# jolibrain/fluidnet_cxx

Measured on AMD Instinct MI355X. Metric: fluid time-step throughput, Mcells/s = cells*steps/s/1e6 (steps/s alongside), higher is better.
Workload: dtype f32; 1 GPU; plume3d_256_jacobi; method=jacobi, jacobi_iters=100, parallelism=1 GPU, launch=hip-graph replay, developed_steps=100, world_size=1, state_finite=True

## Files before the change

fluidnet_cxx_amd/csrc/fluidnet_cpp.cpp:

```cpp
#include <memory>
#include <optional>
#include <torch/extension.h>
#include <c10/hip/HIPStream.h>
#include <c10/hip/HIPGuard.h>

#include "../../include/fluidnet_hip.h"

namespace {

using at::Tensor;

struct Geom {
  bool ref_quirks = false;
  int z_offset = 0, D_global = 0;
  int k_begin = 0, k_end = 0;
};

void check_status(int rc) {
  TORCH_CHECK(rc == FNX_OK, fnx_last_error());
}

void check_field(const Tensor& t, const char* name) {
  TORCH_CHECK(t.is_cuda(), name, " must be on the GPU (libfluidnet_hip has no CPU path)");
  TORCH_CHECK(t.scalar_type() == at::kFloat, name, " must be float32");
// ... 856 lines not shown
  if (grads)
    TORCH_CHECK(upstream->is_cuda() && upstream->scalar_type() == at::kFloat && upstream->numel() == 1 && upstream->get_device() == out_p.get_device(),
                "upstream must be one float32 on the GPU");
  c10::hip::HIPGuard guard(out_p.get_device());
  const float lam[4] = {(float)lambdas[0], (float)lambdas[1], (float)lambdas[2], (float)lambdas[3]};
  Tensor t, gp, gU, ws;
  size_t bytes = 0;
  if (terms) {
    t = at::empty({5}, out_p.options());
    bytes = (is3d ? fnx_train_loss3d_ws_bytes : fnx_train_loss_ws_bytes)(&g);
    ws = at::empty({(int64_t)(bytes ? bytes : 1)}, out_p.options().dtype(at::kByte));
  }
  if (grads) { gp = at::empty_like(out_p); gU = at::empty_like(out_U); }
  check_status((is3d ? fnx_train_loss3d : fnx_train_loss)(
      &g, out_p.data_ptr<float>(), out_U.data_ptr<float>(), flags.data_ptr<float>(), has_t ? target_p->data_ptr<float>() : nullptr, lam,
      grads ? upstream->data_ptr<float>() : nullptr, terms ? t.data_ptr<float>() : nullptr, grads ? gp.data_ptr<float>() : nullptr,
      grads ? gU.data_ptr<float>() : nullptr, terms ? ws.data_ptr() : nullptr, bytes, cur_stream(out_p)));
  return {t, gp, gU};
}

static float* opt_field(const FnxGrid& g, c10::optional<Tensor>& t, bool vel, const char* name) {
  if (!t.has_value() || !t->defined()) return nullptr;
  if (vel) check_vel(*t, g, name); else check_scalar(*t, g, name);
  return t->data_ptr<float>();
}

static FnxState make_state(const FnxGrid& g, Tensor& p, Tensor& U, Tensor& flags, c10::optional<Tensor>& density,
                           c10::optional<Tensor>& UBC, c10::optional<Tensor>& UBCInvMask,
                           c10::optional<Tensor>& densityBC, c10::optional<Tensor>& densityBCInvMask) {
  FnxState st{};
  st.p = p.data_ptr<float>(); st.U = U.data_ptr<float>(); st.flags = flags.data_ptr<float>();
  st.density = opt_field(g, density, false, "density");
  st.UBC = opt_field(g, UBC, true, "UBC"); st.UBCInvMask = opt_field(g, UBCInvMask, true, "UBCInvMask");
  st.densityBC = opt_field(g, densityBC, false, "densityBC"); st.densityBCInvMask = opt_field(g, densityBCInvMask, false, "densityBCInvMask");
  return st;
}

static FnxStepParams step_params(double dt, double buoyancy_scale, const std::vector<double>& gravity_vec, double operating_density) {
  FnxStepParams prm{};
  prm.dt = (float)dt; prm.buoyancy_scale = (float)buoyancy_scale;
  for (int a = 0; a < 3; ++a) prm.gravity_vec[a] = (float)gravity_vec[a];
  prm.operating_density = (float)operating_density;
  return prm;
}

void simulate_step_(Tensor p, Tensor U, Tensor flags, c10::optional<Tensor> density, c10::optional<Tensor> UBC,
                    c10::optional<Tensor> UBCInvMask, c10::optional<Tensor> densityBC,
                    c10::optional<Tensor> densityBCInvMask, c10::optional<Tensor> net, double dt,
                    double maccormack_strength, bool sample_outside_fluid, double buoyancy_scale,
                    std::vector<double> gravity_vec, double operating_density, double p_tol, int jacobi_iter,
                    const std::string method, double normalize_threshold, c10::optional<Tensor> workspace,
                    int static_flags, const Geom* geom, const std::string& precision_mode, double viscosity,
                    double gravity_scale, bool correct_scalar, int periodic, c10::optional<Tensor> flags_stick, double pcg_tol,
                    int pcg_iter, double vorticity_confinement, bool pcg_warm) {
  check_field(U, "U");
  FnxGrid g = grid_of(flags, U.size(1) == 3, geom);
  check_vel(U, g, "U"); check_scalar(p, g, "p");
  TORCH_CHECK(viscosity >= 0, "Viscosity must be positive");
  TORCH_CHECK(method == "jacobi" || method == "convnet" || method == "pcg" || method == "hybrid",
              "Simulation method not supported. Choose convnet, jacobi, pcg or hybrid.");
  TORCH_CHECK(gravity_vec.size() == 3, "gravityVec needs x, y, z");
  FnxStepParams prm = step_params(dt, buoyancy_scale, gravity_vec, operating_density);
  prm.maccormack_strength = (float)maccormack_strength; prm.sample_outside_fluid = sample_outside_fluid;
  prm.p_tol = (float)p_tol; prm.jacobi_iter = jacobi_iter;
  prm.method = method == "convnet" ? 1 : (method == "hybrid" ? 3 : (method == "pcg" ? (pcg_warm ? 4 : 2) : 0)); prm.normalize_threshold = (float)normalize_threshold;
  prm.pcg_tol = (float)pcg_tol; prm.pcg_iter = pcg_iter;
  prm.precision_mode = precision_of(precision_mode);
  prm.viscosity = (float)viscosity; prm.gravity_scale = (float)gravity_scale; prm.correct_scalar = correct_scalar ? 1 : 0;
  prm.periodic = periodic;
  prm.vorticity_confinement = (float)vorticity_confinement;
  FnxState st = make_state(g, p, U, flags, density, UBC, UBCInvMask, densityBC, densityBCInvMask);
  st.net = (net.has_value() && net->defined()) ? net->data_ptr() : nullptr;
  st.flags_stick = opt_field(g, flags_stick, false, "flags_stick");
  c10::hip::HIPGuard guard(flags.get_device());
  const size_t bytes = fnx_workspace_bytes(&g, FNX_OP_STEP);
  Tensor ws;
  const bool given = workspace.has_value() && workspace->defined() && (size_t)workspace->numel() * workspace->element_size() >= bytes;
  if (given) ws = *workspace;
  else ws = at::empty({(int64_t)bytes}, flags.options().dtype(at::kByte));
  prm.static_flags = given ? static_flags : 0;
  check_status(fnx_simulate_step(&g, &prm, &st, ws.data_ptr(), (size_t)ws.numel() * ws.element_size(), cur_stream(U)));
  wrote(p); wrote(U); wrote(density);
}

struct PyLoopbackGroup {
  void* g = nullptr; int nranks;
  explicit PyLoopbackGroup(int n) : nranks(n) { check_status(fnx_slab_loopback_group(&g, n)); }
  ~PyLoopbackGroup() { fnx_slab_loopback_group_free(g); }
};
struct PyPeer {
  void* p = nullptr;
  std::string handle;
  PyPeer(int rank, int nranks, int64_t mailbox_bytes) {
    char h[FNX_PEER_HANDLE_BYTES];
    check_status(fnx_slab_peer_create(&p, rank, nranks, (size_t)mailbox_bytes, h));
    handle.assign(h, FNX_PEER_HANDLE_BYTES);
  }
  ~PyPeer() { fnx_slab_peer_free(p); }
};
struct PySlabComm {
  FnxSlabComm c{};
  std::shared_ptr<PyLoopbackGroup> keep;
  std::shared_ptr<PyPeer> keep_peer;
  ~PySlabComm() { fnx_slab_comm_free(&c); }
};
py::bytes slab_rccl_unique_id() {
  char id[128];
  check_status(fnx_slab_rccl_unique_id(id));
  return py::bytes(id, 128);
}
std::shared_ptr<PySlabComm> slab_comm_rccl(int rank, int nranks, const std::string& unique_id) {
  TORCH_CHECK(unique_id.size() == 128, "the RCCL unique id has 128 bytes");
  auto c = std::make_shared<PySlabComm>();
  py::gil_scoped_release nogil;
  check_status(fnx_slab_comm_rccl(&c->c, rank, nranks, unique_id.data()));
  return c;
}
std::shared_ptr<PySlabComm> slab_comm_loopback(std::shared_ptr<PyLoopbackGroup> group, int rank) {
  auto c = std::make_shared<PySlabComm>();
  check_status(fnx_slab_comm_loopback(&c->c, group->g, rank));
  c->keep = group;
  return c;
}
struct PySlab {
  FnxSlab* s = nullptr;
  FnxSlabConfig cfg{};
  std::shared_ptr<PySlabComm> comm;
  PySlab(int B, int H, int W, int D_global, int rank, int nranks, int halo, int sweeps_per_exchange, bool static_flags,
         int cfl_check_every, std::shared_ptr<PySlabComm> comm_, const std::string& schedule, const std::string& method, const std::string& direct_sends) : comm(comm_) {
    cfg.B = B; cfg.H = H; cfg.W = W; cfg.D_global = D_global; cfg.rank = rank; cfg.nranks = nranks; cfg.halo = halo;
    cfg.sweeps_per_exchange = sweeps_per_exchange; cfg.static_flags = static_flags ? 1 : 0; cfg.cfl_check_every = cfl_check_every;
    TORCH_CHECK(schedule == "deep_first" || schedule == "edge_first" || schedule == "last_pass" || schedule == "deep_beside",
                "unknown z-slab schedule '", schedule, "'");
    cfg.schedule = schedule == "deep_first" ? FNX_SLAB_DEEP_FIRST : (schedule == "edge_first" ? FNX_SLAB_EDGE_FIRST :
                   (schedule == "deep_beside" ? FNX_SLAB_DEEP_BESIDE : FNX_SLAB_LAST_PASS));
    TORCH_CHECK(method == "jacobi" || method == "convnet", "unknown z-slab method '", method, "'");
    cfg.method = method == "convnet" ? 1 : 0;
    TORCH_CHECK(direct_sends == "auto" || direct_sends == "never" || direct_sends == "always", "direct_sends: 'auto', 'never' or 'always'");
    cfg.direct_sends = direct_sends == "auto" ? 0 : (direct_sends == "never" ? 1 : 2);
    check_status(fnx_slab_create(&s, &cfg, comm ? &comm->c : nullptr));
  }
  ~PySlab() { fnx_slab_destroy(s); }
  std::vector<int> layout() const {
    int o, l, h, z;
    check_status(fnx_slab_layout(&cfg, &o, &l, &h, &z));
    return {o, l, h, z};
  }
  int64_t workspace_bytes() const { return (int64_t)fnx_slab_workspace_bytes(&cfg); }
  void stats_enable(bool on) { check_status(fnx_slab_stats_enable(s, on ? 1 : 0)); }
  py::dict stats_read() {
    FnxSlabStats t{};
    check_status(fnx_slab_stats_read(s, &t));
    py::dict d;
    d["bytes_per_neighbour"] = t.bytes_per_neighbour; d["wait_ms"] = t.wait_ms; d["exchanges"] = (int64_t)t.exchanges;
    return d;
  }
  void step(Tensor p, Tensor U, Tensor flags, Tensor density, c10::optional<Tensor> UBC, c10::optional<Tensor> UBCInvMask,
            c10::optional<Tensor> densityBC, c10::optional<Tensor> densityBCInvMask, double dt, double maccormack_strength,
            bool sample_outside_fluid, double buoyancy_scale, std::vector<double> gravity_vec, double operating_density,
            double p_tol, int jacobi_iter, Tensor workspace, c10::optional<Tensor> net, const std::string& precision_mode,
            double normalize_threshold, const std::string& method, double viscosity) {
    check_field(U, "U");
    Geom none;
    FnxGrid g = grid_of(flags, true, &none);
    check_vel(U, g, "U"); check_scalar(p, g, "p"); check_scalar(density, g, "density");
    const std::vector<int> l = layout();
    TORCH_CHECK(g.B == cfg.B && g.H == cfg.H && g.W == cfg.W && g.D == l[0] + l[1] + l[2], "the tensors are not this rank's slab (",
                cfg.B, " x ", l[0] + l[1] + l[2], " x ", cfg.H, " x ", cfg.W, " with ghost planes)");
    TORCH_CHECK(gravity_vec.size() == 3, "gravityVec needs x, y, z");
    TORCH_CHECK(workspace.is_cuda() && workspace.is_contiguous(), "workspace must be a contiguous GPU tensor");
    FnxStepParams prm = step_params(dt, buoyancy_scale, gravity_vec, operating_density);
    prm.maccormack_strength = (float)maccormack_strength; prm.sample_outside_fluid = sample_outside_fluid;
    prm.p_tol = (float)p_tol; prm.jacobi_iter = jacobi_iter; prm.method = 0;
    const bool cnn = net.has_value() && net->defined();
    if (cnn) {
      TORCH_CHECK(net->is_cuda() && net->is_contiguous(), "net: the packed weights (scalenet_pack) on the GPU");
      prm.method = 1; prm.precision_mode = precision_of(precision_mode); prm.normalize_threshold = (float)normalize_threshold;
    }
    TORCH_CHECK(method == "auto" || method == "jacobi" || method == "convnet" || method == "pcg", "unknown z-slab step method '", method, "'");
    if (method == "pcg") prm.method = 2;
    prm.viscosity = (float)viscosity;
    c10::optional<Tensor> rho(density);
    FnxState st = make_state(g, p, U, flags, rho, UBC, UBCInvMask, densityBC, densityBCInvMask);
    if (cnn) st.net = net->data_ptr();
    c10::hip::HIPGuard guard(flags.get_device());
    check_status(fnx_slab_step(s, &prm, &st, workspace.data_ptr(), (size_t)workspace.numel() * workspace.element_size(), cur_stream(U)));
  }
};

void jacobi_sweeps_(Tensor flags, Tensor div, Tensor p, bool is3D, int nsweeps, c10::optional<Tensor> workspace,
                    bool reuse_mask, const Geom* geom, bool from_zero) {
  FnxGrid g = grid_of(flags, is3D, geom);
  check_scalar(div, g, "div"); check_scalar(p, g, "p");
  c10::hip::HIPGuard guard(flags.get_device());
  const size_t bytes = fnx_workspace_bytes(&g, FNX_OP_JACOBI);
  Tensor ws;
  if (workspace.has_value() && workspace->defined() && (size_t)workspace->numel() * workspace->element_size() >= bytes) ws = *workspace;
  else { ws = at::empty({(int64_t)bytes}, flags.options().dtype(at::kByte)); reuse_mask = false; }
  check_status(fnx_jacobi_sweeps_ex(&g, flags.data_ptr<float>(), div.data_ptr<float>(), p.data_ptr<float>(), nsweeps,
                                    ws.data_ptr(), (size_t)ws.numel() * ws.element_size(), (reuse_mask ? 1 : 0) | (from_zero ? 2 : 0),
                                    cur_stream(flags)));
  wrote(p);
}

void jacobi_pass_(Tensor flags, Tensor div, c10::optional<Tensor> p_in_opt, Tensor p_out, int nsweeps, int k_begin,
                  int k_end, Tensor workspace, bool reuse_mask, int k_begin2, const Geom* geom, int layout) {
  FnxGrid g = grid_of(flags, true, geom);
  const bool zero = !(p_in_opt.has_value() && p_in_opt->defined());
  Tensor p_in = zero ? p_out : *p_in_opt;
  check_scalar(div, g, "div"); check_scalar(p_in, g, "p_in"); check_scalar(p_out, g, "p_out");
  c10::hip::HIPGuard guard(flags.get_device());
  check_status(fnx_jacobi_pass_layout(&g, flags.data_ptr<float>(), div.data_ptr<float>(), zero ? nullptr : p_in.data_ptr<float>(),
                                      p_out.data_ptr<float>(), nsweeps, k_begin, k_end, k_begin2, layout, workspace.data_ptr(),
                                      (size_t)workspace.numel() * workspace.element_size(), reuse_mask ? 1 : 0, cur_stream(flags)));
  wrote(p_out);
}

bool jacobi_quad_ok(int B, int D, int H, int W) {
  FnxGrid g{B, D, H, W, 1, 0, 0, 0};
  return fnx_jacobi_quad_ok(&g) != 0;
}

void jacobi_pass_mirror_(Tensor flags, Tensor div, Tensor p_in, Tensor p_out, int k_begin, int k_end, Tensor workspace, bool reuse_mask,
                         Tensor mirror, int k_first, int planes, int k_begin2, c10::optional<Tensor> mirror2, int k_first2, const Geom* geom,
                         int layout) {
  FnxGrid g = grid_of(flags, true, geom);
  check_scalar(div, g, "div"); check_scalar(p_in, g, "p_in"); check_scalar(p_out, g, "p_out");
  const int64_t need = (int64_t)g.B * planes * g.H * g.W;
  auto chk = [&](const Tensor& t) { TORCH_CHECK(t.is_cuda() && t.is_contiguous() && t.scalar_type() == at::kFloat && t.numel() >= need, "mirror: a contiguous fp32 GPU tensor of B * planes * H * W floats"); };
  chk(mirror);
  FnxPlaneMirror m{};
  m.out[0][0] = mirror.data_ptr<float>(); m.k_first[0] = k_first; m.planes = planes; m.sample_stride = (size_t)planes * g.H * g.W;
  if (mirror2.has_value() && mirror2->defined()) { chk(*mirror2); m.out[1][0] = mirror2->data_ptr<float>(); m.k_first[1] = k_first2; }
  c10::hip::HIPGuard guard(flags.get_device());
  check_status(fnx_jacobi_pass_mirror(&g, flags.data_ptr<float>(), div.data_ptr<float>(), p_in.data_ptr<float>(), p_out.data_ptr<float>(),
                                      k_begin, k_end, k_begin2, layout, &m, workspace.data_ptr(),
                                      (size_t)workspace.numel() * workspace.element_size(), reuse_mask ? 1 : 0, cur_stream(flags)));
  wrote(p_out); wrote(mirror); wrote(mirror2);
}

int64_t jacobi_workspace_bytes(int B, int D, int H, int W, bool is3D) {
  FnxGrid g{B, D, H, W, is3D ? 1 : 0, 0, 0, 0};
  return (int64_t)fnx_workspace_bytes(&g, FNX_OP_JACOBI);
}

static const unsigned char* bc_class_ptr(c10::optional<Tensor>& t, const Tensor& flags) {
  if (!t.has_value() || !t->defined()) return nullptr;
  TORCH_CHECK(t->scalar_type() == at::kByte && t->is_contiguous() && t->numel() == flags.numel() && t->device() == flags.device(),
              "bc_class: expected the uint8 tensor bc_classify returned for this grid");
  return t->data_ptr<unsigned char>();
}

Tensor bc_classify(Tensor flags, bool is3D, c10::optional<Tensor> UBC, c10::optional<Tensor> UBCInvMask,
                   c10::optional<Tensor> densityBC, c10::optional<Tensor> densityBCInvMask) {
  FnxGrid g = grid_of(flags, is3D, nullptr);
  Tensor dummy;
  c10::optional<Tensor> none;
  FnxState st{};
  st.UBC = opt_field(g, UBC, true, "UBC"); st.UBCInvMask = opt_field(g, UBCInvMask, true, "UBCInvMask");
  st.densityBC = opt_field(g, densityBC, false, "densityBC"); st.densityBCInvMask = opt_field(g, densityBCInvMask, false, "densityBCInvMask");
  c10::hip::HIPGuard guard(flags.get_device());
  Tensor cls = at::empty(flags.sizes(), flags.options().dtype(at::kByte));
  check_status(fnx_bc_classify(&g, &st, cls.data_ptr<unsigned char>(), cur_stream(flags)));
  return cls;
}

Tensor pre_projection_(Tensor U_adv, c10::optional<Tensor> rho_adv, Tensor p, Tensor U, Tensor flags,
                       c10::optional<Tensor> density, c10::optional<Tensor> UBC, c10::optional<Tensor> UBCInvMask,
                       c10::optional<Tensor> densityBC, c10::optional<Tensor> densityBCInvMask, double dt,
                       double buoyancy_scale, std::vector<double> gravity_vec, double operating_density,
                       bool jacobi_method, c10::optional<Tensor> bc_class, const Geom* geom) {
  check_field(U, "U");
  FnxGrid g = grid_of(flags, U.size(1) == 3, geom);
  check_vel(U, g, "U"); check_vel(U_adv, g, "U_adv"); check_scalar(p, g, "p");
  FnxStepParams prm = step_params(dt, buoyancy_scale, gravity_vec, operating_density);
  prm.method = jacobi_method ? 0 : 1;
  FnxState st = make_state(g, p, U, flags, density, UBC, UBCInvMask, densityBC, densityBCInvMask);
  const float* ra = nullptr;
  if (rho_adv.has_value() && rho_adv->defined()) { check_scalar(*rho_adv, g, "rho_adv"); ra = rho_adv->data_ptr<float>(); }
  st.bc_class = bc_class_ptr(bc_class, flags);
  c10::hip::HIPGuard guard(flags.get_device());
  Tensor div = at::empty_like(flags);
  check_status(fnx_pre_projection(&g, &prm, &st, U_adv.data_ptr<float>(), ra, div.data_ptr<float>(), cur_stream(U)));
  return div;
}

void post_projection_(Tensor p, Tensor U, Tensor flags, c10::optional<Tensor> density, c10::optional<Tensor> UBC,
                      c10::optional<Tensor> UBCInvMask, c10::optional<Tensor> densityBC,
                      c10::optional<Tensor> densityBCInvMask, c10::optional<Tensor> bc_class, const Geom* geom,
                      bool density_bc_applied) {
  check_field(U, "U");
  FnxGrid g = grid_of(flags, U.size(1) == 3, geom);
  check_vel(U, g, "U"); check_scalar(p, g, "p");
  FnxState st = make_state(g, p, U, flags, density, UBC, UBCInvMask, densityBC, densityBCInvMask);
  st.bc_class = bc_class_ptr(bc_class, flags);
  st.density_bc_applied = density_bc_applied ? 1 : 0;
  c10::hip::HIPGuard guard(flags.get_device());
  check_status(fnx_post_projection(&g, &st, cur_stream(U)));
  wrote(U); wrote(density);
}

int64_t step_workspace_bytes(int B, int D, int H, int W, bool is3D) {
  FnxGrid g{B, D, H, W, is3D ? 1 : 0, 0, 0, 0};
  return (int64_t)fnx_workspace_bytes(&g, FNX_OP_STEP);
}

}

template <class T, class R, class... A>
static auto in_dim(T which, R (*body)(T, A...)) {
  return [=](A... a) { return body(which, std::forward<A>(a)...); };
}

PYBIND11_MODULE(TORCH_EXTENSION_NAME, m) {
  using NoGil = py::call_guard<py::gil_scoped_release>;
  const auto GEOM = py::arg("geom") = py::none();
  py::class_<Geom>(m, "Geom", "per-call 3D geometry options: ref_quirks, z-slab view (z_offset, D_global), compute window [k_begin, k_end)")
      .def(py::init([](bool ref_quirks, int z_offset, int D_global, int k_begin, int k_end) {
             Geom g; g.ref_quirks = ref_quirks; g.z_offset = z_offset; g.D_global = D_global; g.k_begin = k_begin; g.k_end = k_end;
             return g;
           }),
           py::arg("ref_quirks") = false, py::arg("z_offset") = 0, py::arg("D_global") = 0, py::arg("k_begin") = 0,
           py::arg("k_end") = 0)
      .def_readwrite("ref_quirks", &Geom::ref_quirks)
      .def_readwrite("z_offset", &Geom::z_offset)
      .def_readwrite("D_global", &Geom::D_global)
      .def_readwrite("k_begin", &Geom::k_begin)
      .def_readwrite("k_end", &Geom::k_end);
  m.def("advect_scalar", &advect_scalar, "Advect Scalar", py::arg("dt"), py::arg("src"), py::arg("U"), py::arg("flags"),
        py::arg("method"), py::arg("boundary_width"), py::arg("sample_outside_fluid"), py::arg("maccormack_strength"),
        py::arg("out") = py::none(), GEOM, py::arg("plan") = "auto", NoGil());
  m.def("advect_scalars", &advect_scalars, "Advect C passive scalars through one pair of line traces", py::arg("dt"), py::arg("src"),
        py::arg("U"), py::arg("flags"), py::arg("method"), py::arg("boundary_width"), py::arg("sample_outside_fluid"),
        py::arg("maccormack_strength"), py::arg("workspace") = py::none(), GEOM, py::arg("out") = py::none(), NoGil());
  m.def("advect_scalars_workspace_bytes", [](int B, int D, int H, int W, bool is3D, int channels) {
          FnxGrid g{}; g.B = B; g.D = D; g.H = H; g.W = W; g.is3D = is3D ? 1 : 0;
          return fnx_advect_scalars_workspace_bytes(&g, channels);
        }, py::arg("B"), py::arg("D"), py::arg("H"), py::arg("W"), py::arg("is3D"), py::arg("channels"));
  m.def("advect_step", &advect_step, py::arg("dt"), py::arg("density"), py::arg("U"), py::arg("flags"),
        py::arg("sample_outside_fluid"), py::arg("maccormack_strength"), py::arg("out_density") = py::none(),
        py::arg("out_U") = py::none(), GEOM, py::arg("plan") = "auto", NoGil());
  m.def("advect_vel", &advect_vel, "Advect Velocity", py::arg("dt"), py::arg("orig"), py::arg("U"), py::arg("flags"),
        py::arg("method"), py::arg("boundary_width"), py::arg("maccormack_strength"), py::arg("out") = py::none(), GEOM,
        py::arg("plan") = "auto", NoGil());
  m.def("solve_linear_system", &solve_linear_system, "Solve Linear System using Jacobi's method", py::arg("flags"),
        py::arg("div"), py::arg("is3D"), py::arg("p_tol"), py::arg("max_iter"), py::arg("verbose"), GEOM, NoGil());
  m.def("solve_linear_system_pcg", &solve_linear_system_pcg, "Converged pressure solve: multigrid-preconditioned CG (fnx_pcg); "
        "returns (p, residual, iterations per sample or None when p_tol <= 0).  p0: a starting guess (fnx_pcg_from; max_iter may then be 0)",
        py::arg("flags"), py::arg("div"), py::arg("is3D"), py::arg("p_tol") = 1e-5,
        py::arg("max_iter") = 50, py::arg("verbose") = false, GEOM, py::arg("p0") = py::none(), NoGil());
  m.def("poisson_apply", &poisson_apply, "A p, the operator of the pressure solve (fnx_poisson_apply)", py::arg("flags"), py::arg("p"),
        py::arg("is3D"), GEOM, NoGil());
  m.def("pcg_precondition", &pcg_precondition, "z = M^-1 r, one V-cycle of the PCG preconditioner (fnx_pcg_precondition)", py::arg("flags"),
        py::arg("r"), py::arg("is3D"), GEOM, NoGil());
  m.def("velocity_divergence", &velocity_divergence, py::arg("U"), py::arg("flags"), GEOM, NoGil());
  m.def("velocity_update_", &velocity_update_, py::arg("pressure"), py::arg("U"), py::arg("flags"), GEOM, NoGil());
  m.def("add_buoyancy_", &add_buoyancy_, py::arg("U"), py::arg("flags"), py::arg("density"), py::arg("gravity"),
        py::arg("rho_star"), py::arg("dt"), GEOM, NoGil());
  m.def("correct_scalar_", &correct_scalar_, py::arg("dt"), py::arg("src"), py::arg("div"), py::arg("flags"), NoGil());
  m.def("add_gravity_", &add_gravity_, py::arg("U"), py::arg("flags"), py::arg("gravity"), py::arg("dt"), GEOM, NoGil());
  m.def("add_viscosity_", &add_viscosity_, NoGil());
  m.def("add_vorticity_confinement", &add_vorticity_confinement, py::arg("U"), py::arg("flags"), py::arg("strength"), GEOM, NoGil());
  m.def("add_vorticity_confinement_", &add_vorticity_confinement_, py::arg("U"), py::arg("flags"), py::arg("strength"), GEOM, NoGil());
  m.def("render_volume", &render_volume, "density + flags -> (B,2,R,Cc) radiance / transmittance image (fnx_render_volume)", py::arg("density"),
        py::arg("flags"), py::arg("view_dir"), py::arg("light_dir"), py::arg("k_view"), py::arg("k_light"), py::arg("ambient") = 0.25,
        py::arg("albedo_smoke") = 1.0, py::arg("albedo_obstacle") = 0.5, py::arg("bnd") = 1, NoGil());
  m.def("set_wall_bcs_", &set_wall_bcs_, py::arg("U"), py::arg("flags"), GEOM, NoGil());
  m.def("set_wall_bcs_stick_", &set_wall_bcs_stick_, NoGil());
  m.def("add_viscosity_out", &add_viscosity_out, "addViscosity of U into `out` (not U), returned (fnx_add_viscosity)", py::arg("dt"), py::arg("U"),
        py::arg("flags"), py::arg("viscosity"), py::arg("out"), NoGil());
  m.def("set_wall_bcs_stick_out", &set_wall_bcs_stick_out, "setWallBcsStick of U into `out` (not U), returned (fnx_set_wall_bcs_stick)",
        py::arg("U"), py::arg("flags"), py::arg("flags_stick"), py::arg("out"), NoGil());
  m.def("set_const_vals_", &set_const_vals_, NoGil());
  m.def("flags_to_occupancy", &flags_to_occupancy, NoGil());
  m.def("max_abs", &max_abs, NoGil());
  m.def("empty_domain_", &empty_domain_, py::arg("flags"), py::arg("boundary_width"), GEOM, NoGil());
  m.def("velocity_divergence_backward", &velocity_divergence_backward, py::arg("grad_div"), py::arg("flags"), py::arg("is3D"), GEOM, NoGil());
  m.def("velocity_update_backward", &velocity_update_backward, py::arg("grad_U_out"), py::arg("flags"), GEOM, NoGil());
  m.def("create_cylinder_", &create_cylinder_, NoGil());
  m.def("create_box2d_", &create_box2d_, NoGil());
  m.def("get_centered", &get_centered, NoGil());
  m.def("scalenet_pack", &scalenet_pack, NoGil());
  m.def("multiscale_forward", &multiscale_forward, py::arg("packed"), py::arg("x"), py::arg("precision_mode") = "fp32",
        py::arg("trim") = std::vector<int64_t>(), NoGil());
  m.def("fluidnet_forward", in_dim((const BankApi*)nullptr, &whole_forward), py::arg("packed"), py::arg("input"),
        py::arg("normalize_threshold"), py::arg("precision_mode") = "fp32", NoGil());
  m.def("banknet_pack", in_dim(&BANK2D, &bank_pack), py::arg("blob"), NoGil());
  m.def("banknet_forward", in_dim(&BANK2D, &bank_forward), py::arg("packed"), py::arg("x"), py::arg("precision_mode") = "fp32", NoGil());
  m.def("fluidnet_bank_forward", in_dim(&BANK2D, &whole_forward), py::arg("packed"), py::arg("input"), py::arg("normalize_threshold"),
        py::arg("precision_mode") = "fp32", NoGil());
  m.def("banknet3d_pack", in_dim(&BANK3D, &bank_pack), py::arg("blob"), NoGil());
  m.def("banknet3d_forward", in_dim(&BANK3D, &bank_forward), py::arg("packed"), py::arg("x"), py::arg("precision_mode") = "fp32", NoGil());
  m.def("fluidnet_bank3d_forward", in_dim(&BANK3D, &whole_forward), py::arg("packed"), py::arg("input"), py::arg("normalize_threshold"),
        py::arg("precision_mode") = "fp32", NoGil());
  m.def("banknet_pack_t", &banknet_pack_t, py::arg("blob"), NoGil());
  m.def("banknet_tape_layout", &banknet_tape_layout, py::arg("B"), py::arg("H"), py::arg("W"));
  m.def("banknet_forward_train", &banknet_forward_train, py::arg("packed"), py::arg("x"), py::arg("precision_mode") = "fp32", NoGil());
  m.def("banknet_backward", &banknet_backward, py::arg("packed_t"), py::arg("x"), py::arg("grad_p"), py::arg("tape"),
        py::arg("precision_mode") = "fp32", NoGil());
  m.def("fluidnet_bank_forward_train", &fluidnet_bank_forward_train, py::arg("packed"), py::arg("input"), py::arg("normalize_threshold"),
        py::arg("precision_mode") = "fp32", NoGil());
  m.def("fluidnet_bank_backward", &fluidnet_bank_backward, py::arg("packed_t"), py::arg("flags"), py::arg("scale"), py::arg("grad_p"),
        py::arg("grad_U"), py::arg("tape"), py::arg("precision_mode") = "fp32", NoGil());
  m.def("simulate_step_", &simulate_step_, py::arg("p"), py::arg("U"), py::arg("flags"), py::arg("density"), py::arg("UBC"),
        py::arg("UBCInvMask"), py::arg("densityBC"), py::arg("densityBCInvMask"), py::arg("net"), py::arg("dt"),
        py::arg("maccormack_strength"), py::arg("sample_outside_fluid"), py::arg("buoyancy_scale"), py::arg("gravity_vec"),
        py::arg("operating_density"), py::arg("p_tol"), py::arg("jacobi_iter"), py::arg("method"),
        py::arg("normalize_threshold"), py::arg("workspace") = py::none(), py::arg("static_flags") = 0, GEOM,
        py::arg("precision_mode") = "fp32", py::arg("viscosity") = 0.0, py::arg("gravity_scale") = 0.0,
        py::arg("correct_scalar") = false, py::arg("periodic") = 0, py::arg("flags_stick") = py::none(), py::arg("pcg_tol") = 1e-5,
        py::arg("pcg_iter") = 50, py::arg("vorticity_confinement") = 0.0, py::arg("pcg_warm") = false, NoGil());
  m.def("step_workspace_bytes", &step_workspace_bytes);
  m.def("jacobi_sweeps_", &jacobi_sweeps_, py::arg("flags"), py::arg("div"), py::arg("p"), py::arg("is3D"), py::arg("nsweeps"),
        py::arg("workspace") = py::none(), py::arg("reuse_mask") = false, GEOM, py::arg("from_zero") = false, NoGil());
  m.def("jacobi_workspace_bytes", &jacobi_workspace_bytes);
  m.def("jacobi_pass_", &jacobi_pass_, py::arg("flags"), py::arg("div"), py::arg("p_in"), py::arg("p_out"), py::arg("nsweeps"),
        py::arg("k_begin"), py::arg("k_end"), py::arg("workspace"), py::arg("reuse_mask"), py::arg("k_begin2") = -1, GEOM,
        py::arg("layout") = 0, NoGil());
  m.def("jacobi_pass_mirror_", &jacobi_pass_mirror_, py::arg("flags"), py::arg("div"), py::arg("p_in"), py::arg("p_out"), py::arg("k_begin"),
        py::arg("k_end"), py::arg("workspace"), py::arg("reuse_mask"), py::arg("mirror"), py::arg("k_first"), py::arg("planes"),
        py::arg("k_begin2") = -1, py::arg("mirror2") = py::none(), py::arg("k_first2") = 0, GEOM, py::arg("layout") = 0, NoGil(),
        "two sweeps on planes [k_begin, k_end) (+ a second range) whose output planes [k_first, k_first + planes) also go to `mirror` (fnx_jacobi_pass_mirror)");
  m.def("jacobi_pass_mirror_ok", [](int B, int D, int H, int W, int planes_per_range, bool two_ranges, int layout) {
    FnxGrid g{}; g.B = B; g.D = D; g.H = H; g.W = W; g.is3D = 1;
    return fnx_jacobi_pass_mirror_ok(&g, planes_per_range, two_ranges ? 1 : 0, layout) != 0;
  });
  m.def("jacobi_quad_ok", &jacobi_quad_ok);
  m.def("pre_projection_", &pre_projection_, py::arg("U_adv"), py::arg("rho_adv"), py::arg("p"), py::arg("U"), py::arg("flags"),
        py::arg("density"), py::arg("UBC"), py::arg("UBCInvMask"), py::arg("densityBC"), py::arg("densityBCInvMask"),
        py::arg("dt"), py::arg("buoyancy_scale"), py::arg("gravity_vec"), py::arg("operating_density"),
        py::arg("jacobi_method"), py::arg("bc_class") = py::none(), GEOM, NoGil());
  m.def("post_projection_", &post_projection_, py::arg("p"), py::arg("U"), py::arg("flags"), py::arg("density"), py::arg("UBC"),
        py::arg("UBCInvMask"), py::arg("densityBC"), py::arg("densityBCInvMask"), py::arg("bc_class") = py::none(), GEOM,
        py::arg("density_bc_applied") = false, NoGil());
  m.def("bc_classify", &bc_classify, "uint8 class map of static BC arrays (FnxState.bc_class)", NoGil());
  py::class_<PyLoopbackGroup, std::shared_ptr<PyLoopbackGroup>>(m, "SlabLoopbackGroup", "in-process communicator group: n slabs driven by n host threads")
      .def(py::init<int>(), py::arg("nranks"))
      .def("set_timeout", [](PyLoopbackGroup& g, double seconds) { check_status(fnx_slab_loopback_group_set_timeout(g.g, seconds)); }, py::arg("seconds"),
           "how long a rank waits for a peer before its call fails (the group stays usable); default 120 s")
      .def("reset", [](PyLoopbackGroup& g) { check_status(fnx_slab_loopback_group_reset(g.g)); },
           "clear an abort (no rank may be inside a call of the group)");
  py::class_<PySlabComm, std::shared_ptr<PySlabComm>>(m, "SlabComm", "ghost-plane communicator of the native z-slab driver (FnxSlabComm)")
      .def("failed", [](PySlabComm& c) { return c.keep_peer ? fnx_slab_peer_failed(c.keep_peer->p) != FNX_OK : false; },
           "peer-store: an exchange of this rank timed out / the group was aborted (ask after synchronising; other transports report through their calls)")
      .def("allreduce_sum_", [](PySlabComm& c, Tensor x) {
             TORCH_CHECK(x.is_cuda() && x.is_contiguous() && x.scalar_type() == at::kFloat, "allreduce: a contiguous fp32 GPU tensor");
             c10::hip::HIPGuard guard(x.get_device());
             py::gil_scoped_release nogil;
             check_status(c.c.allreduce_sum(c.c.ctx, x.data_ptr<float>(), (int)x.numel(), cur_stream(x)));
           }, py::arg("x"))
      .def("allreduce_max_", [](PySlabComm& c, Tensor x) {
             TORCH_CHECK(x.is_cuda() && x.is_contiguous() && x.scalar_type() == at::kFloat, "allreduce: a contiguous fp32 GPU tensor");
             c10::hip::HIPGuard guard(x.get_device());
             py::gil_scoped_release nogil;
             check_status(c.c.allreduce_max(c.c.ctx, x.data_ptr<float>(), (int)x.numel(), cur_stream(x)));
           }, py::arg("x"));
  m.def("slab_rccl_unique_id", &slab_rccl_unique_id);
  m.def("slab_comm_rccl", &slab_comm_rccl, py::arg("rank"), py::arg("nranks"), py::arg("unique_id"));
  m.def("slab_comm_loopback", &slab_comm_loopback, py::arg("group"), py::arg("rank"));
  py::class_<PyPeer, std::shared_ptr<PyPeer>>(m, "SlabPeer", "a rank's peer-store region: flags + mailbox its z-neighbours map (fnx_slab_peer_create)")
      .def(py::init<int, int, int64_t>(), py::arg("rank"), py::arg("nranks"), py::arg("mailbox_bytes"))
      .def_property_readonly("handle", [](PyPeer& p) { return py::bytes(p.handle); }, "the bytes both neighbours need (FNX_PEER_HANDLE_BYTES)")
      .def("set_timeout", [](PyPeer& p, double seconds) { check_status(fnx_slab_peer_set_timeout(p.p, seconds)); }, py::arg("seconds"))
      .def("failed", [](PyPeer& p) { return fnx_slab_peer_failed(p.p) != FNX_OK; },
           "a device-side wait of this rank's exchanges has timed out, or the group was aborted (ask after synchronising the stream)");
  m.def("slab_comm_peer", [](std::shared_ptr<PyPeer> peer, py::object handle_lo, py::object handle_hi) {
    std::string lo = handle_lo.is_none() ? std::string() : handle_lo.cast<std::string>();
    std::string hi = handle_hi.is_none() ? std::string() : handle_hi.cast<std::string>();
    TORCH_CHECK((lo.empty() || lo.size() == FNX_PEER_HANDLE_BYTES) && (hi.empty() || hi.size() == FNX_PEER_HANDLE_BYTES), "a peer handle has ",
                FNX_PEER_HANDLE_BYTES, " bytes");
    auto c = std::make_shared<PySlabComm>();
    check_status(fnx_slab_comm_peer(&c->c, peer->p, lo.empty() ? nullptr : lo.data(), hi.empty() ? nullptr : hi.data()));
    c->keep_peer = peer;
    return c;
  }, py::arg("peer"), py::arg("handle_lo"), py::arg("handle_hi"), "peer-store communicator: device stores into the neighbours' mapped mailboxes + flags");
  m.def("slab_comm_link_model", [](double latency_us, double gbps) {
    auto c = std::make_shared<PySlabComm>();
    check_status(fnx_slab_comm_link_model(&c->c, latency_us, gbps));
    return c;
  }, py::arg("latency_us"), py::arg("gbytes_per_s"), "rehearsal communicator: one process runs a middle rank's step against an assumed link");
  m.def("slab_comm_probe", [](std::shared_ptr<PySlabComm> comm, int64_t bytes, int reps, Tensor scratch) {
    TORCH_CHECK(scratch.is_cuda() && scratch.is_contiguous() && (int64_t)scratch.numel() * scratch.element_size() >= 4 * bytes,
                "slab_comm_probe: scratch must be a contiguous GPU tensor of at least 4 * bytes");
    c10::hip::HIPGuard guard(scratch.get_device());
    float ms = 0.f;
    { py::gil_scoped_release nogil;
      check_status(fnx_slab_comm_probe(&comm->c, scratch.data_ptr(), (size_t)bytes, reps, &ms, cur_stream(scratch))); }
    return (double)ms;
  }, py::arg("comm"), py::arg("bytes"), py::arg("reps"), py::arg("scratch"),
        "average ms of one ghost exchange of `bytes` bytes with each neighbour (every rank must call it)");
  py::class_<PySlab>(m, "SlabDriver", "native z-slab driver of the 3D Jacobi step (fnx_slab_create / fnx_slab_step)")
      .def(py::init<int, int, int, int, int, int, int, int, bool, int, std::shared_ptr<PySlabComm>, const std::string&, const std::string&, const std::string&>(), py::arg("B"), py::arg("H"),
           py::arg("W"), py::arg("D_global"), py::arg("rank"), py::arg("nranks"), py::arg("halo"), py::arg("sweeps_per_exchange"),
           py::arg("static_flags") = false, py::arg("cfl_check_every") = 0, py::arg("comm") = nullptr, py::arg("schedule") = "deep_first",
           py::arg("method") = "jacobi", py::arg("direct_sends") = "auto")
      .def("stats_enable", &PySlab::stats_enable, py::arg("on"))
      .def("stats_read", &PySlab::stats_read, "dict(bytes_per_neighbour, wait_ms, exchanges) since stats_enable(True); synchronises")
      .def("layout", &PySlab::layout, "(owned planes, ghost planes below, above, global plane of local plane 0)")
      .def("workspace_bytes", &PySlab::workspace_bytes)
      .def("step", &PySlab::step, py::arg("p"), py::arg("U"), py::arg("flags"), py::arg("density"), py::arg("UBC"), py::arg("UBCInvMask"),
           py::arg("densityBC"), py::arg("densityBCInvMask"), py::arg("dt"), py::arg("maccormack_strength"),
           py::arg("sample_outside_fluid"), py::arg("buoyancy_scale"), py::arg("gravity_vec"), py::arg("operating_density"),
           py::arg("p_tol"), py::arg("jacobi_iter"), py::arg("workspace"), py::arg("net") = py::none(), py::arg("precision_mode") = "fp32",
           py::arg("normalize_threshold") = 1e-5, py::arg("method") = "auto", py::arg("viscosity") = 0.0, NoGil());
  m.def("device_name", []() { const char* n = fnx_device_name(); return std::string(n ? n : ""); });
  m.def("trilinear_upsample_backward", &trilinear_upsample_backward, py::arg("grad_dst"), py::arg("size"), NoGil());
  m.def("multiscale_tape_layout", [](int64_t B, int64_t H, int64_t W) { return multiscale_tape_layout(false, B, 1, H, W); }, py::arg("B"),
        py::arg("H"), py::arg("W"));
  m.def("multiscale3d_tape_layout", in_dim(true, &multiscale_tape_layout), py::arg("B"), py::arg("D"), py::arg("H"), py::arg("W"));
  m.def("scene_obstacles",
        [](Tensor ids, int64_t H, int64_t W, int64_t seed, int n_min, int n_max, double centre_min, double centre_max, double size_min,
           double size_max, int64_t depth) {
          return scene_obstacles(false, ids, depth, H, W, seed, n_min, n_max, centre_min, centre_max, size_min, size_max);
        },
        py::arg("scene_ids"), py::arg("H"), py::arg("W"), py::arg("seed"), py::arg("n_min"), py::arg("n_max"), py::arg("centre_min"),
        py::arg("centre_max"), py::arg("size_min"), py::arg("size_max"), py::arg("depth") = 1, NoGil());
  m.def("scene_obstacles3d", in_dim(true, &scene_obstacles), py::arg("scene_ids"), py::arg("D"), py::arg("H"), py::arg("W"), py::arg("seed"),
        py::arg("n_min"), py::arg("n_max"), py::arg("centre_min"), py::arg("centre_max"), py::arg("size_min"), py::arg("size_max"), NoGil());
  m.def("scene_turbulence",
        [](Tensor ids, int64_t H, int64_t W, int64_t seed, int octaves, double wavelength, double amplitude, double density_scale,
           bool with_density, int64_t depth) {
          return scene_turbulence(false, ids, depth, H, W, seed, octaves, wavelength, amplitude, density_scale, with_density);
        },
        py::arg("scene_ids"), py::arg("H"), py::arg("W"), py::arg("seed"), py::arg("octaves"), py::arg("wavelength"), py::arg("amplitude"),
        py::arg("density_scale"), py::arg("with_density") = true, py::arg("depth") = 1, NoGil());
  m.def("scene_turbulence3d", in_dim(true, &scene_turbulence), py::arg("scene_ids"), py::arg("D"), py::arg("H"), py::arg("W"), py::arg("seed"),
        py::arg("octaves"), py::arg("wavelength"), py::arg("amplitude"), py::arg("density_scale"), py::arg("with_density") = true, NoGil());
  for (const bool is3d : {false, true}) {
    const std::string d = is3d ? "3d" : "";
    m.def(("scalenet" + d + "_pack_t").c_str(), in_dim(is3d, &scalenet_pack_t), py::arg("blob"), NoGil());
    m.def(("multiscale" + d + "_forward_train").c_str(), in_dim(is3d, &multiscale_forward_train), py::arg("packed"), py::arg("x"),
          py::arg("precision_mode") = "fp32", NoGil());
    m.def(("multiscale" + d + "_backward").c_str(), in_dim(is3d, &multiscale_backward), py::arg("packed_t"), py::arg("grad_p"), py::arg("tape"),
          py::arg("precision_mode") = "fp32", NoGil());
    m.def(("multiscale" + d + "_backward_plain").c_str(), in_dim(is3d, &multiscale_backward_plain), py::arg("packed_t"), py::arg("grad_p"),
          py::arg("tape"), py::arg("precision_mode") = "fp32", NoGil());
    m.def(("fluidnet" + d + "_forward_train").c_str(), in_dim(is3d, &fluidnet_forward_train), py::arg("packed"), py::arg("input"),
          py::arg("normalize_threshold"), py::arg("precision_mode") = "fp32", NoGil());
    m.def(("fluidnet" + d + "_backward").c_str(), in_dim(is3d, &fluidnet_backward), py::arg("packed_t"), py::arg("flags"), py::arg("scale"),
          py::arg("grad_p"), py::arg("grad_U"), py::arg("tape"), py::arg("precision_mode") = "fp32", NoGil());
    m.def(is3d ? "train_loss3d" : "train_loss", in_dim(is3d, &train_loss), py::arg("out_p"), py::arg("out_U"), py::arg("flags"),
          py::arg("target_p"), py::arg("lambdas"), py::arg("upstream") = py::none(), py::arg("terms") = true, NoGil());
  }
  m.def("abi_version", &fnx_abi_version);
  m.def("profile_enable", [](bool on, bool runs) { fnx_profile_enable(on ? (runs ? 2 : 1) : 0); }, py::arg("on"), py::arg("runs") = false);
  m.def("roctx_enable", [](bool on) { check_status(fnx_roctx_enable(on ? 1 : 0)); });
  m.def("profile_read_work", [](int tag) { double w = 0; fnx_profile_read_work(tag, &w); return w; });
  m.def("profile_read", [](int tag) { double ms = 0; int n = 0; fnx_profile_read(tag, &ms, &n); return std::make_pair(ms, n); });
}
```

fluidnet_cxx_amd/csrc/fnx_api.hip:

```cpp
#include <stdarg.h>
#include <stdio.h>
#include <string.h>

#include "../../include/fluidnet_hip.h"
#include "fnx_cnn.h"
#include "fnx_kernels.h"
#include <algorithm>
#include <atomic>
#include <dlfcn.h>

namespace {

thread_local char g_err[512] = "";

int fail(int code, const char* fmt, ...) {
  va_list ap;
  va_start(ap, fmt);
  vsnprintf(g_err, sizeof(g_err), fmt, ap);
  va_end(ap);
  return code;
}

#define HIP_OK(expr)                                                                      \
  do {                                                                                    \
    hipError_t e_ = (expr);                                                               \
    if (e_ != hipSuccess) return fail(FNX_EHIP, "HIP error: %s (%s)", hipGetErrorString(e_), #expr); \
  } while (0)

int check_grid(const FnxGrid* g) {
  if (!g) return fail(FNX_EINVAL, "grid descriptor is NULL");
  if (g->B < 1 || g->D < 1 || g->H < 3 || g->W < 3) return fail(FNX_EINVAL, "Dimension mismatch: B=%d D=%d H=%d W=%d", g->B, g->D, g->H, g->W);
  if (!g->is3D && g->D != 1) return fail(FNX_EINVAL, "2D velocity field but zdepth > 1");
  if (g->is3D && g->D < 3) return fail(FNX_EINVAL, "3D domain needs D >= 3");
  if ((long long)g->D * g->H * g->W >= (1ll << 31)) return fail(FNX_EINVAL, "more than 2^31 cells per sample");
  if ((long long)g->B * g->D > 65535) return fail(FNX_EINVAL, "B*D > 65535 not supported");
  if (!g->is3D && (g->W > 65535 || g->H > 65535)) return fail(FNX_EINVAL, "2D grids wider or taller than 65535 are not supported");
  if (g->k_end != 0 || g->k_begin != 0) {
    if (!g->is3D || g->k_begin < 0 || g->k_end > g->D || g->k_end <= g->k_begin)
      return fail(FNX_EINVAL, "bad compute window [%d, %d) for D=%d", g->k_begin, g->k_end, g->D);
  }
  if (g->D_global != 0 && (!g->is3D || g->z_offset < 0 || g->z_offset + g->D > g->D_global))
    return fail(FNX_EINVAL, "bad z-slab: z_offset=%d D=%d D_global=%d", g->z_offset, g->D, g->D_global);
  return FNX_OK;
}

inline GridDims dims(const FnxGrid* g) {
  GridDims d = make_dims(g->B, g->D, g->H, g->W, g->z_offset, g->D_global);
  if (g->is3D && g->k_end > g->k_begin) { d.K0 = g->k_begin; d.KN = g->k_end - g->k_begin; }
  return d;
}
inline bool quirks(const FnxGrid* g) { return g->is3D && g->ref_quirks; }
inline size_t ncell(const FnxGrid* g) { return (size_t)g->B * g->D * g->H * g->W; }
inline size_t al(size_t x) { return (x + 255) & ~(size_t)255; }

struct Carver {
  char* base; size_t off;
  explicit Carver(void* p) : base((char*)p), off(0) {}
  void* take(size_t bytes) { void* r = base ? base + off : nullptr; off += al(bytes); return r; }
};

size_t ws_advect(const FnxGrid* g, int what) { return fnx::advect_workspace(dims(g), g->is3D, what, nullptr).bytes; }
size_t ws_mask(const FnxGrid* g) { return g->is3D ? fnx::jacobi3d_mask_layout(dims(g), nullptr).bytes : 0; }
struct JacobiWs { float* tmp; double* partials; float* res; fnx::JacobiMaskLayout mask; };
size_t carve_jacobi(const FnxGrid* g, void* ws, JacobiWs* out) {
  Carver c(ws);
  out->tmp = (float*)c.take(ncell(g) * 4);
  out->partials = (double*)c.take(fnx::residual_scratch_bytes(g->B));
  out->res = (float*)c.take(4);
  out->mask = fnx::jacobi3d_mask_layout(dims(g), g->is3D ? c.take(ws_mask(g)) : nullptr);
  return c.off;
}
size_t ws_jacobi(const FnxGrid* g) { JacobiWs W; return carve_jacobi(g, nullptr, &W); }
size_t ws_pcg_kept(const FnxGrid* g) { return al(fnx::pcg_kept_bytes(dims(g), g->is3D)); }
size_t ws_pcg(const FnxGrid* g) { return ws_pcg_kept(g) + al(fnx::pcg_scratch_bytes(dims(g), g->is3D)); }
inline bool is_view(const FnxGrid* g) { return g->k_begin != 0 || g->k_end != 0 || g->z_offset != 0 || g->D_global != 0; }
fnx::StepLayout carve_step(const FnxGrid* g, void* ws) {
  const GridDims d = dims(g);
  const size_t advect = ws_advect(g, fnx::ADVECT_BOTH);
  const size_t jacobi = ws_jacobi(g);
  const size_t net = fnx::fluidnet_ws_bytes(d, g->is3D);
  const size_t pcg = al(fnx::pcg_scratch_bytes(d, g->is3D));
  const size_t periodic = fnx::periodic_save_bytes(d);
  const size_t tail_need = std::max({advect, jacobi, net, pcg, periodic});
  return fnx::step_layout(ncell(g), g->is3D ? 3 : 2, g->is3D != 0, ws_mask(g), ws_pcg_kept(g), tail_need, ws);
}
size_t ws_step(const FnxGrid* g) { return carve_step(g, nullptr).bytes; }

}

namespace fnx {
int set_error(int code, const char* fmt, ...) {
  va_list ap;
  va_start(ap, fmt);
  vsnprintf(g_err, sizeof(g_err), fmt, ap);
  va_end(ap);
  return code;
}
}

namespace fnx {
namespace {
constexpr int PROF_MAX = 16384;
struct Prof {
  bool on = false;
  bool runs = false;
  int n = 0;
  hipEvent_t ev[PROF_MAX][2];
  int tag[PROF_MAX];
  int count[PROF_MAX];
  hipStream_t stream[PROF_MAX];
  int created = 0;
  int open_idx[FNX_PROF_NTAGS];
  double work[FNX_PROF_NTAGS];
} g_prof;
}

namespace {
struct Roctx { int (*push)(const char*) = nullptr; int (*pop)() = nullptr; std::atomic<bool> on{false}; } g_roctx;
const char* const kProfNames[FNX_PROF_NTAGS] = {"fnx:jacobi", "fnx:conv_mfma", "fnx:advect", "fnx:stage", "fnx:conv_direct", "fnx:conv_mfma16", "fnx:conv_bf16"};
}

bool prof_begin(int tag, hipStream_t s) {
  const bool pushed = g_roctx.on.load(std::memory_order_acquire);
  if (pushed) g_roctx.push(kProfNames[tag]);
  if (!g_prof.on || g_prof.n >= PROF_MAX) { if (g_prof.on) g_prof.open_idx[tag] = -1; return pushed; }
  if (g_prof.runs && g_prof.n > 0 && g_prof.tag[g_prof.n - 1] == tag && g_prof.stream[g_prof.n - 1] == s) {
    g_prof.open_idx[tag] = g_prof.n - 1;
    ++g_prof.count[g_prof.n - 1];
    return pushed;
  }
  const int i = g_prof.n++;
  if (i >= g_prof.created) {
    hipEventCreate(&g_prof.ev[i][0]); hipEventCreate(&g_prof.ev[i][1]);
    g_prof.created = i + 1;
  }
  g_prof.tag[i] = tag;
  g_prof.count[i] = 1;
  g_prof.stream[i] = s;
  g_prof.open_idx[tag] = i;
  hipEventRecord(g_prof.ev[i][0], s);
  return pushed;
}

void prof_add_work(int tag, double amount) {
  if (g_prof.on && g_prof.open_idx[tag] >= 0) g_prof.work[tag] += amount;
}

void prof_end(int tag, hipStream_t s, bool pushed) {
  if (pushed) g_roctx.pop();
  if (!g_prof.on) return;
  const int i = g_prof.open_idx[tag];
  if (i >= 0) hipEventRecord(g_prof.ev[i][1], s);
}
}

extern "C" {

int fnx_profile_enable(int on) {
  fnx::g_prof.on = on != 0;
  fnx::g_prof.runs = on == 2;
  if (on) { fnx::g_prof.n = 0; for (int t = 0; t < FNX_PROF_NTAGS; ++t) { fnx::g_prof.open_idx[t] = -1; fnx::g_prof.work[t] = 0.0; } }
  return FNX_OK;
}

int fnx_roctx_enable(int on) {
  if (!on) { fnx::g_roctx.on.store(false, std::memory_order_release); return FNX_OK; }
  if (!fnx::g_roctx.push) {
    void* h = nullptr;
    for (const char* name : {"librocprofiler-sdk-roctx.so.1", "librocprofiler-sdk-roctx.so", "libroctx64.so.4", "libroctx64.so"}) {
      h = dlopen(name, RTLD_NOW | RTLD_GLOBAL);
      if (h) break;
    }
    if (!h) return fail(FNX_EINVAL, "roctx_enable: no roctx library found (librocprofiler-sdk-roctx.so / libroctx64.so)");
    fnx::g_roctx.push = (int (*)(const char*))dlsym(h, "roctxRangePushA");
    fnx::g_roctx.pop = (int (*)())dlsym(h, "roctxRangePop");
    if (!fnx::g_roctx.push || !fnx::g_roctx.pop) { fnx::g_roctx.push = nullptr; return fail(FNX_EINVAL, "roctx_enable: roctxRangePushA / roctxRangePop not found"); }
  }
  fnx::g_roctx.on.store(true, std::memory_order_release);
  return FNX_OK;
}

int fnx_profile_read_work(int tag, double* work) {
  if (tag < 0 || tag >= FNX_PROF_NTAGS || !work) return fail(FNX_EINVAL, "profile_read_work: bad tag");
  *work = fnx::g_prof.work[tag];
  return FNX_OK;
}

int fnx_profile_read(int tag, double* total_ms, int* launches) {
  double tot = 0.0; int cnt = 0;
  for (int i = 0; i < fnx::g_prof.n; ++i) {
    if (fnx::g_prof.tag[i] != tag) continue;
    if (hipEventSynchronize(fnx::g_prof.ev[i][1]) != hipSuccess) continue;
    float ms = 0.f;
    if (hipEventElapsedTime(&ms, fnx::g_prof.ev[i][0], fnx::g_prof.ev[i][1]) == hipSuccess) { tot += ms; cnt += fnx::g_prof.count[i]; }
  }
  if (total_ms) *total_ms = tot;
  if (launches) *launches = cnt;
  return FNX_OK;
}

const char* fnx_last_error(void) { return g_err; }
int fnx_abi_version(void) { return FNX_ABI_VERSION; }

const char* fnx_device_name(void) {
  static thread_local char name[256];
  int dev = 0;
  if (hipGetDevice(&dev) != hipSuccess) { fail(FNX_EHIP, "no HIP device"); return nullptr; }
  hipDeviceProp_t prop;
  if (hipGetDeviceProperties(&prop, dev) != hipSuccess) { fail(FNX_EHIP, "no HIP device"); return nullptr; }
  snprintf(name, sizeof(name), "%s (%s)", prop.name, prop.gcnArchName);
  return name;
}

size_t fnx_workspace_bytes(const FnxGrid* g, int op) {
  if (check_grid(g) != FNX_OK) return 0;
  switch (op) {
    case FNX_OP_ADVECT_SCALAR: return ws_advect(g, fnx::ADVECT_RHO);
    case FNX_OP_ADVECT_VEL: return ws_advect(g, fnx::ADVECT_VEL);
    case FNX_OP_JACOBI: return ws_jacobi(g);
    case FNX_OP_STEP: return ws_step(g);
    case FNX_OP_FLUIDNET: return fnx::fluidnet_ws_bytes(dims(g), g->is3D);
    case FNX_OP_ADVECT_STEP: return ws_advect(g, fnx::ADVECT_BOTH);
  }
  fail(FNX_EINVAL, "unknown op %d", op);
  return 0;
}

static int advect_run(const char* name, const FnxGrid* g, int what, int method, int plan, const fnx::AdvectArgs& a, void* ws,
                      size_t ws_bytes, void* stream) {
  const fnx::AdvectPlan p = fnx::advect_plan(dims(g), g->is3D, quirks(g), what, a.orig == a.U, method, plan);
  fnx::AdvectWs w{};
  if (p.maccormack) {
    w = fnx::advect_workspace(p.g, g->is3D, what, ws);
    if (!ws || w.bytes > ws_bytes) return fail(FNX_EWORKSPACE, "%s: workspace too small (%zu < %zu)", name, ws_bytes, w.bytes);
  }
  hipStream_t s = (hipStream_t)stream;
  fnx::ProfScope ps(FNX_PROF_ADVECT, s);
  fnx::launch_advect(p, a, w, s);
  HIP_OK(hipGetLastError());
  return FNX_OK;
}

int fnx_advect_scalar(const FnxGrid* g, float dt, const float* src, const float* U, const float* flags, float* dst,
                      int method, int bnd, int sample_outside, float strength, void* ws, size_t ws_bytes,
                      void* stream) {
  return fnx_advect_scalar_plan(g, dt, src, U, flags, dst, method, bnd, sample_outside, strength, FNX_ADVECT_PLAN_AUTO, ws, ws_bytes, stream);
}

int fnx_advect_scalar_plan(const FnxGrid* g, float dt, const float* src, const float* U, const float* flags, float* dst,
                           int method, int bnd, int sample_outside, float strength, int plan, void* ws, size_t ws_bytes,
                           void* stream) {
  if (int rc = check_grid(g)) return rc;
  if (plan < FNX_ADVECT_PLAN_AUTO || plan > FNX_ADVECT_PLAN_TILES_SPLIT) return fail(FNX_EINVAL, "advect_scalar: unknown plan %d", plan);
  if (!src || !U || !flags || !dst) return fail(FNX_EINVAL, "advect_scalar: NULL tensor");
  if (dst == src) return fail(FNX_EINVAL, "advect_scalar: dst must not alias src");
  if (method != FNX_ADVECT_EULER && method != FNX_ADVECT_MACCORMACK) return fail(FNX_EMETHOD, "Advection method not supported");
  if (bnd != 1) return fail(FNX_EINVAL, "advect_scalar: only boundary_width == 1 is supported (the reference's MAC sampling strips exactly one border cell)");
  const fnx::AdvectArgs a{dt, strength * 0.5f, sample_outside != 0, src, U, U, flags, dst, nullptr};
  return advect_run("advect_scalar", g, fnx::ADVECT_RHO, method, plan, a, ws, ws_bytes, stream);
}

int fnx_advect_vel(const FnxGrid* g, float dt, const float* orig, const float* U, const float* flags, float* dst,
                   int method, int bnd, float strength, void* ws, size_t ws_bytes, void* stream) {
  return fnx_advect_vel_plan(g, dt, orig, U, flags, dst, method, bnd, strength, FNX_ADVECT_PLAN_AUTO, ws, ws_bytes, stream);
}

int fnx_advect_vel_plan(const FnxGrid* g, float dt, const float* orig, const float* U, const float* flags, float* dst,
                        int method, int bnd, float strength, int plan, void* ws, size_t ws_bytes, void* stream) {
  if (int rc = check_grid(g)) return rc;
  if (plan < FNX_ADVECT_PLAN_AUTO || plan > FNX_ADVECT_PLAN_TILES_SPLIT) return fail(FNX_EINVAL, "advect_vel: unknown plan %d", plan);
  if (!orig || !U || !flags || !dst) return fail(FNX_EINVAL, "advect_vel: NULL tensor");
  if (dst == orig || dst == U) return fail(FNX_EINVAL, "advect_vel: dst must not alias orig or U");
  if (method != FNX_ADVECT_EULER && method != FNX_ADVECT_MACCORMACK) return fail(FNX_EMETHOD, "Advection method not supported");
  if (bnd != 1) return fail(FNX_EINVAL, "advect_vel: only boundary_width == 1 is supported");
  const fnx::AdvectArgs a{dt, strength * 0.5f, false, nullptr, orig, U, flags, nullptr, dst};
  return advect_run("advect_vel", g, fnx::ADVECT_VEL, method, plan, a, ws, ws_bytes, stream);
}

int fnx_advect_step(const FnxGrid* g, float dt, const float* density, const float* U, const float* flags,
                    float* density_dst, float* U_dst, int sample_outside, float strength, void* ws, size_t ws_bytes,
                    void* stream) {
  return fnx_advect_step_plan(g, dt, density, U, flags, density_dst, U_dst, sample_outside, strength, FNX_ADVECT_PLAN_AUTO, ws, ws_bytes, stream);
}

int fnx_advect_step_plan(const FnxGrid* g, float dt, const float* density, const float* U, const float* flags,
                         float* density_dst, float* U_dst, int sample_outside, float strength, int plan, void* ws,
                         size_t ws_bytes, void* stream) {
  if (int rc = check_grid(g)) return rc;
  if (plan < FNX_ADVECT_PLAN_AUTO || plan > FNX_ADVECT_PLAN_TILES_SPLIT) return fail(FNX_EINVAL, "advect_step: unknown plan %d", plan);
  if (!density || !U || !flags || !density_dst || !U_dst) return fail(FNX_EINVAL, "advect_step: NULL tensor");
  if (density_dst == density || U_dst == U) return fail(FNX_EINVAL, "advect_step: dst must not alias the inputs");
  const fnx::AdvectArgs a{dt, strength * 0.5f, sample_outside != 0, density, U, U, flags, density_dst, U_dst};
  return advect_run("advect_step", g, fnx::ADVECT_BOTH, FNX_ADVECT_MACCORMACK, plan, a, ws, ws_bytes, stream);
}

static int check_scalars_grid(const FnxGrid* g, int channels) {
  if (int rc = check_grid(g)) return rc;
  if (channels < 1) return fail(FNX_EINVAL, "advect_scalars: channels < 1 (%d)", channels);
  if (is_view(g)) return fail(FNX_EINVAL, "advect_scalars: no compute window or z-slab view (single-domain only)");
  if ((g->H + 3) / 4 > 65535) return fail(FNX_EINVAL, "advect_scalars: H/4 > 65535 not supported");
  if (g->is3D && (long long)g->B * channels * fnx::advect_scalars_box_chunks(dims(g)) > 65535)
    return fail(FNX_EINVAL, "advect_scalars: B*channels*ceil(D/16) > 65535 not supported");
  return FNX_OK;
}

size_t fnx_advect_scalars_workspace_bytes(const FnxGrid* g, int channels) {
  if (check_scalars_grid(g, channels) != FNX_OK) return 0;
  return fnx::advect_scalars_workspace(dims(g), g->is3D != 0, channels, nullptr).bytes;
}

int fnx_advect_scalars(const FnxGrid* g, float dt, int channels, const float* src, const float* U, const float* flags, float* dst,
                       int method, int bnd, int sample_outside, float strength, void* ws, size_t ws_bytes, void* stream) {
  if (int rc = check_scalars_grid(g, channels)) return rc;
  if (!src || !U || !flags || !dst) return fail(FNX_EINVAL, "advect_scalars: NULL tensor");
  if (dst == src) return fail(FNX_EINVAL, "advect_scalars: dst must not alias src");
  if (method != FNX_ADVECT_EULER && method != FNX_ADVECT_MACCORMACK) return fail(FNX_EMETHOD, "Advection method not supported");
  if (bnd != 1) return fail(FNX_EINVAL, "advect_scalars: only boundary_width == 1 is supported (the reference's MAC sampling strips exactly one border cell)");
  const bool mac = method == FNX_ADVECT_MACCORMACK;
  fnx::AdvectScalarsWs w{};
  if (mac) {
    w = fnx::advect_scalars_workspace(dims(g), g->is3D != 0, channels, ws);
    if (!ws || w.bytes > ws_bytes) return fail(FNX_EWORKSPACE, "advect_scalars: workspace too small (%zu < %zu)", ws ? ws_bytes : (size_t)0, w.bytes);
  }
  hipStream_t s = (hipStream_t)stream;
  fnx::ProfScope ps(FNX_PROF_ADVECT, s);
  fnx::launch_advect_scalars(dims(g), g->is3D != 0, quirks(g), mac, sample_outside != 0, dt, strength * 0.5f, channels, src, U, flags, dst,
                             w, s);
  HIP_OK(hipGetLastError());
  return FNX_OK;
}

int fnx_velocity_divergence(const FnxGrid* g, const float* U, const float* flags, float* div, void* stream) {
  if (int rc = check_grid(g)) return rc;
  if (!U || !flags || !div) return fail(FNX_EINVAL, "velocity_divergence: NULL tensor");
  fnx::launch_divergence(dims(g), g->is3D, U, flags, div, (hipStream_t)stream);
  HIP_OK(hipGetLastError());
  return FNX_OK;
}

static int jacobi_begin(const char* name, const FnxGrid* g, const float* flags, void* ws, size_t ws_bytes, bool reuse_mask,
                        hipStream_t s, JacobiWs* W, unsigned char* kept_mask = nullptr) {
  const size_t need = carve_jacobi(g, ws, W);
  if (!ws || need > ws_bytes) return fail(FNX_EWORKSPACE, "%s: workspace too small (%zu < %zu)", name, ws_bytes, need);
  if (g->is3D && kept_mask) W->mask = fnx::jacobi3d_mask_layout(dims(g), kept_mask);
  if (g->is3D && !reuse_mask) fnx::launch_jacobi3d_mask(dims(g), quirks(g), flags, W->mask, s);
  return FNX_OK;
}

static int check_plane_ranges(const char* name, const FnxGrid* g, int kb, int ke, int kb2, bool whole_ok) {
  if (kb < 0 || ke > g->D || ((ke != 0 || !whole_ok) && ke <= kb)) return fail(FNX_EINVAL, "%s: bad plane range", name);
  const int n = ke - kb;
  if (kb2 >= 0 && (ke == 0 || kb2 + n > g->D || (kb2 < ke && kb < kb2 + n)))
    return fail(FNX_EINVAL, "%s: bad or overlapping second plane range", name);
  return FNX_OK;
}

static const float* run_jacobi_launches(const FnxGrid* g, const fnx::JacobiSchedule& sch, const float* flags, const float* div,
                                        const fnx::JacobiMaskLayout& mask, const float* in, float* const buf[2], int first,
                                        hipStream_t s) {
  const GridDims d = dims(g);
  for (int l = 0; l < sch.n; ++l) {
    const fnx::JacobiLaunch L = sch.at(l);
    float* out = buf[(first + l) & 1];
    fnx::ProfScope ps(FNX_PROF_JACOBI, s);
    if (!g->is3D) fnx::launch_jacobi(d, flags, div, in, out, L.sweeps, in == nullptr, s);
    else if (L.sweeps == 2) fnx::launch_jacobi3d_x2(d, mask, div, in, out, s, 0, 0, in == nullptr, -1, L.lay);
    else fnx::launch_jacobi3d(d, mask, div, in, out, in == nullptr, s);
    in = out;
  }
  return in;
}

static int jacobi_solve(const FnxGrid* g, const float* flags, const float* div, float* p, float* residual, float p_tol,
                        int max_iter, int* iters_done, void* ws, size_t ws_bytes, unsigned char* kept_mask, bool reuse_mask,
                        void* stream, int verbose) {
  if (int rc = check_grid(g)) return rc;
  if (!flags || !div || !p) return fail(FNX_EINVAL, "solve_linear_system: NULL tensor");
  if (max_iter < 1) return fail(FNX_EINVAL, "At least 1 iteration is needed (maxIter < 1)");
  hipStream_t s = (hipStream_t)stream;
  const GridDims d = dims(g);
  JacobiWs W;
  if (int rc = jacobi_begin("solve_linear_system", g, flags, ws, ws_bytes, reuse_mask && kept_mask, s, &W, kept_mask)) return rc;
  float* const buf[2] = {p, W.tmp};
  const int cus = cu_count();
  const fnx::JacobiSchedule one = fnx::jacobi_schedule(d, g->is3D, 1, cus);
  const size_t per = (size_t)g->D * g->H * g->W;
  auto residual_of = [&](const float* a, const float* b, float* out) { fnx::launch_residual(g->B, per, 0, per, a, b, W.partials, nullptr, out, s); };
  const bool per_sweep = p_tol > 0.f || verbose;
  if (!per_sweep) {
    const fnx::JacobiSchedule sch = fnx::jacobi_schedule(d, g->is3D, residual ? max_iter - 1 : max_iter, cus);
    if (sch.n > fnx::JACOBI_MAX_LAUNCHES) return fail(FNX_EINVAL, "solve_linear_system: max_iter too large for one call (%d)", max_iter);
    const float* in = run_jacobi_launches(g, sch, flags, div, W.mask, nullptr, buf, fnx::jacobi_solve_first_buffer(sch, residual != nullptr), s);
    if (residual) {
      run_jacobi_launches(g, one, flags, div, W.mask, in, buf, 0, s);
      residual_of(p, in, residual);
    }
    if (iters_done) *iters_done = max_iter;
  } else {
    const float* in = nullptr;
    int sweeps = 0;
    float r = 0.f;
    for (;;) {
      const float* out = run_jacobi_launches(g, one, flags, div, W.mask, in, buf, sweeps & 1, s);
      residual_of(out, in, W.res);
      HIP_OK(hipMemcpyAsync(&r, W.res, 4, hipMemcpyDeviceToHost, s));
      HIP_OK(hipStreamSynchronize(s));
      in = out;
      ++sweeps;
      if (verbose) printf("Jacobi iteration %d: residual %g\n", sweeps, (double)r);
      if (r < p_tol) {
        if (verbose) printf("Jacobi max residual fell below p_tol (%g) (terminating)\n", (double)p_tol);
        break;
      }
      if (sweeps >= max_iter) {
        if (verbose) printf("Jacobi max iteration count (%d) reached (terminating)\n", max_iter);
        break;
      }
    }
    if (verbose) fflush(stdout);
    if (in != p) HIP_OK(hipMemcpyAsync(p, in, ncell(g) * 4, hipMemcpyDeviceToDevice, s));
    if (residual) HIP_OK(hipMemcpyAsync(residual, W.res, 4, hipMemcpyDeviceToDevice, s));
    if (iters_done) *iters_done = sweeps;
  }
  HIP_OK(hipGetLastError());
  return FNX_OK;
}

int fnx_jacobi(const FnxGrid* g, const float* flags, const float* div, float* p, float* residual, float p_tol,
               int max_iter, int* iters_done, void* ws, size_t ws_bytes, void* stream) {
  return jacobi_solve(g, flags, div, p, residual, p_tol, max_iter, iters_done, ws, ws_bytes, nullptr, false, stream, 0);
}

int fnx_jacobi_verbose(const FnxGrid* g, const float* flags, const float* div, float* p, float* residual, float p_tol,
                       int max_iter, int* iters_done, void* ws, size_t ws_bytes, void* stream) {
  return jacobi_solve(g, flags, div, p, residual, p_tol, max_iter, iters_done, ws, ws_bytes, nullptr, false, stream, 1);
}

int fnx_jacobi_sweeps(const FnxGrid* g, const float* flags, const float* div, float* p, int nsweeps, void* ws,
                      size_t ws_bytes, void* stream) {
  return fnx_jacobi_sweeps_ex(g, flags, div, p, nsweeps, ws, ws_bytes, 0, stream);
}

int fnx_jacobi_sweeps_ex(const FnxGrid* g, const float* flags, const float* div, float* p, int nsweeps, void* ws,
                         size_t ws_bytes, int reuse_mask, void* stream) {
  if (int rc = check_grid(g)) return rc;
  if (!flags || !div || !p) return fail(FNX_EINVAL, "jacobi_sweeps: NULL tensor");
  if (nsweeps < 1) return fail(FNX_EINVAL, "At least 1 iteration is needed (maxIter < 1)");
  hipStream_t s = (hipStream_t)stream;
  JacobiWs W;
  if (int rc = jacobi_begin("jacobi_sweeps", g, flags, ws, ws_bytes, (reuse_mask & 1) != 0, s, &W)) return rc;
  const bool from_zero = (reuse_mask & 2) != 0;
  float* const buf[2] = {p, W.tmp};
  const fnx::JacobiSchedule sch = fnx::jacobi_schedule(dims(g), g->is3D, nsweeps, cu_count());
  const float* in = run_jacobi_launches(g, sch, flags, div, W.mask, from_zero ? nullptr : p, buf, 1, s);
  if (in != p) HIP_OK(hipMemcpyAsync(p, in, ncell(g) * 4, hipMemcpyDeviceToDevice, s));
  HIP_OK(hipGetLastError());
  return FNX_OK;
}

int fnx_jacobi_pass2(const FnxGrid* g, const float* flags, const float* div, const float* p_in, float* p_out,
                     int nsweeps, int k_begin, int k_end, int k_begin2, void* ws, size_t ws_bytes, int reuse_mask,
                     void* stream) {
  return fnx_jacobi_pass_layout(g, flags, div, p_in, p_out, nsweeps, k_begin, k_end, k_begin2, 0, ws, ws_bytes, reuse_mask, stream);
}

int fnx_jacobi_quad_ok(const FnxGrid* g) {
  if (check_grid(g) != FNX_OK || !g->is3D) return 0;
  return fnx::jacobi3d_quad_ok(dims(g)) ? 1 : 0;
}

int fnx_jacobi_pass_layout(const FnxGrid* g, const float* flags, const float* div, const float* p_in, float* p_out,
                           int nsweeps, int k_begin, int k_end, int k_begin2, int layout, void* ws, size_t ws_bytes,
                           int reuse_mask, void* stream) {
  if (int rc = check_grid(g)) return rc;
  if (layout < 0 || layout > 3) return fail(FNX_EINVAL, "jacobi_pass: layout must be 0..3");
  if (layout != 0 && (nsweeps != 2 || !g->is3D || !fnx::jacobi3d_quad_ok(dims(g))))
    return fail(FNX_EINVAL, "jacobi_pass: the row-quad layout needs a two-sweep pass on a grid fnx_jacobi_quad_ok accepts");
  if (!flags || !div || !p_out || p_in == p_out) return fail(FNX_EINVAL, "jacobi_pass: NULL or aliased tensor");
  if (!g->is3D) return fail(FNX_EINVAL, "jacobi_pass: 3D only (2D uses fnx_jacobi_sweeps)");
  const bool from_zero = p_in == nullptr;
  if (nsweeps < 1 || nsweeps > 2) return fail(FNX_EINVAL, "jacobi_pass: nsweeps must be 1 or 2");
  if (int rc = check_plane_ranges("jacobi_pass", g, k_begin, k_end, k_begin2, true)) return rc;
  hipStream_t s = (hipStream_t)stream;
  const GridDims d = dims(g);
  JacobiWs W;
  if (int rc = jacobi_begin("jacobi_pass", g, flags, ws, ws_bytes, reuse_mask != 0, s, &W)) return rc;
  fnx::ProfScope ps(FNX_PROF_JACOBI, s);
  if (nsweeps == 2) fnx::launch_jacobi3d_x2(d, W.mask, div, p_in, p_out, s, k_begin, k_end, from_zero, k_begin2, layout);
  else {
    fnx::launch_jacobi3d(d, W.mask, div, p_in, p_out, from_zero, s, k_begin, k_end);
    if (k_begin2 >= 0) fnx::launch_jacobi3d(d, W.mask, div, p_in, p_out, from_zero, s, k_begin2, k_begin2 + (k_end - k_begin));
  }
  HIP_OK(hipGetLastError());
  return FNX_OK;
}

int fnx_jacobi_pass_mirror_ok(const FnxGrid* g, int planes, int two_ranges, int layout) {
  if (check_grid(g) != FNX_OK || !g->is3D || planes < 1) return 0;
  return fnx::jacobi3d_mirror_ok(dims(g), planes, two_ranges != 0, false, layout, cu_count()) ? 1 : 0;
}

int fnx_jacobi_pass_mirror(const FnxGrid* g, const float* flags, const float* div, const float* p_in, float* p_out, int k_begin,
                           int k_end, int k_begin2, int layout, const FnxPlaneMirror* mirror, void* ws, size_t ws_bytes,
                           int reuse_mask, void* stream) {
  if (int rc = check_grid(g)) return rc;
  if (!g->is3D || !flags || !div || !p_in || !p_out || p_in == p_out || !mirror) return fail(FNX_EINVAL, "jacobi_pass_mirror: NULL or aliased argument");
  if (int rc = check_plane_ranges("jacobi_pass_mirror", g, k_begin, k_end, k_begin2, false)) return rc;
  const GridDims d = dims(g);
  if ((layout == 3 && !fnx::jacobi3d_quad_ok(d)) || !fnx::jacobi3d_mirror_ok(d, k_end - k_begin, k_begin2 >= 0, false, layout, cu_count()))
    return fail(FNX_EINVAL, "jacobi_pass_mirror: this launch cannot mirror its output (fnx_jacobi_pass_mirror_ok)");
  if (mirror->planes < 1 || !mirror->out[0][0] || (mirror->slot_select[0] && !mirror->out[0][1]) ||
      (k_begin2 >= 0 && (!mirror->out[1][0] || (mirror->slot_select[1] && !mirror->out[1][1]))))
    return fail(FNX_EINVAL, "jacobi_pass_mirror: bad mirror");
  hipStream_t s = (hipStream_t)stream;
  JacobiWs W;
  if (int rc = jacobi_begin("jacobi_pass_mirror", g, flags, ws, ws_bytes, reuse_mask != 0, s, &W)) return rc;
  fnx::ProfScope ps(FNX_PROF_JACOBI, s);
  fnx::JacobiMirror m{};
  for (int r = 0; r < 2; ++r) { m.out[r][0] = mirror->out[r][0]; m.out[r][1] = mirror->out[r][1]; m.sel[r] = mirror->slot_select[r]; }
  m.k[0] = mirror->k_first[0]; m.k[1] = mirror->k_first[1]; m.n = mirror->planes;
  m.bstride = mirror->sample_stride; m.clock = mirror->start_clock;
  fnx::launch_jacobi3d_x2(d, W.mask, div, p_in, p_out, s, k_begin, k_end, false, k_begin2, layout, &m);
  HIP_OK(hipGetLastError());
  return FNX_OK;
}

int fnx_jacobi_pass(const FnxGrid* g, const float* flags, const float* div, const float* p_in, float* p_out,
                    int nsweeps, int k_begin, int k_end, void* ws, size_t ws_bytes, int reuse_mask, void* stream) {
  return fnx_jacobi_pass2(g, flags, div, p_in, p_out, nsweeps, k_begin, k_end, -1, ws, ws_bytes, reuse_mask, stream);
}

int fnx_residual(const FnxGrid* g, const float* a, const float* b, float* sumsq, float* residual, void* ws, size_t ws_bytes, void* stream) {
  if (int rc = check_grid(g)) return rc;
  if (!a || (!sumsq && !residual)) return fail(FNX_EINVAL, "residual: NULL tensor");
  if (!ws || ws_bytes < fnx::residual_scratch_bytes(g->B)) return fail(FNX_EWORKSPACE, "residual: workspace too small (%zu < %zu)", ws_bytes, fnx::residual_scratch_bytes(g->B));
  const GridDims d = dims(g);
  const size_t per = (size_t)g->D * g->H * g->W;
  fnx::launch_residual(g->B, per, (size_t)d.K0 * d.HW, (size_t)d.KN * d.HW, a, b, (double*)ws, sumsq, residual, (hipStream_t)stream);
  HIP_OK(hipGetLastError());
  return FNX_OK;
}

size_t fnx_pcg_workspace_bytes(const FnxGrid* g) {
  if (check_grid(g) != FNX_OK) return 0;
  return ws_pcg(g);
}

namespace {
int check_pcg_grid(const FnxGrid* g, const char* who) {
  if (int rc = check_grid(g)) return rc;
  if (is_view(g))
    return fail(FNX_EINVAL, "%s: no compute window or z-slab view (the solve is single-domain)", who);
  return FNX_OK;
}

int pcg_entry(const FnxGrid* g, const float* flags, const float* div, const float* p0, float* p, float* residual, float p_tol, int max_iter,
              int min_iter, int* iters_done, void* ws, size_t ws_bytes, void* stream, bool verbose) {
  if (int rc = check_pcg_grid(g, "pcg")) return rc;
  if (!flags || !div || !p) return fail(FNX_EINVAL, "pcg: NULL tensor");
  if (div == p) return fail(FNX_EINVAL, "pcg: p must not alias div");
  if (min_iter > 0 && max_iter < 1) return fail(FNX_EINVAL, "At least 1 iteration is needed (maxIter < 1)");
  if (max_iter < 0) return fail(FNX_EINVAL, "pcg_from: max_iter must not be negative (maxIter < 0)");
  if (!ws || ws_bytes < ws_pcg(g)) return fail(FNX_EWORKSPACE, "pcg: workspace too small (%zu < %zu)", ws_bytes, ws_pcg(g));
  hipStream_t s = (hipStream_t)stream;
  const GridDims d = dims(g);
  char* kept = (char*)ws;
  fnx::launch_pcg_build(d, g->is3D, quirks(g), flags, kept, s);
  HIP_OK(hipGetLastError());
  if (int rc = fnx::pcg_solve(d, g->is3D, kept, kept + ws_pcg_kept(g), div, p0, p, residual, p_tol, max_iter, iters_done, verbose, s)) return rc;
  HIP_OK(hipGetLastError());
  return FNX_OK;
}
}

int fnx_pcg(const FnxGrid* g, const float* flags, const float* div, float* p, float* residual, float p_tol, int max_iter,
            int* iters_done, void* ws, size_t ws_bytes, void* stream) {
  return pcg_entry(g, flags, div, nullptr, p, residual, p_tol, max_iter, 1, iters_done, ws, ws_bytes, stream, false);
}

int fnx_pcg_verbose(const FnxGrid* g, const float* flags, const float* div, float* p, float* residual, float p_tol, int max_iter,
                    int* iters_done, void* ws, size_t ws_bytes, void* stream) {
  return pcg_entry(g, flags, div, nullptr, p, residual, p_tol, max_iter, 1, iters_done, ws, ws_bytes, stream, true);
}

int fnx_pcg_from(const FnxGrid* g, const float* flags, const float* div, const float* p0, float* p, float* residual, float p_tol,
                 int max_iter, int* iters_done, void* ws, size_t ws_bytes, void* stream) {
  return pcg_entry(g, flags, div, p0, p, residual, p_tol, max_iter, 0, iters_done, ws, ws_bytes, stream, false);
}

int fnx_pcg_from_verbose(const FnxGrid* g, const float* flags, const float* div, const float* p0, float* p, float* residual, float p_tol,
                         int max_iter, int* iters_done, void* ws, size_t ws_bytes, void* stream) {
  return pcg_entry(g, flags, div, p0, p, residual, p_tol, max_iter, 0, iters_done, ws, ws_bytes, stream, true);
}

int fnx_poisson_apply(const FnxGrid* g, const float* flags, const float* p, float* Ap, void* stream) {
  if (int rc = check_pcg_grid(g, "poisson_apply")) return rc;
  if (!flags || !p || !Ap) return fail(FNX_EINVAL, "poisson_apply: NULL tensor");
  if (p == Ap) return fail(FNX_EINVAL, "poisson_apply: Ap must not alias p");
  fnx::launch_poisson_apply(dims(g), g->is3D, quirks(g), flags, p, Ap, (hipStream_t)stream);
  HIP_OK(hipGetLastError());
  return FNX_OK;
}

int fnx_pcg_precondition(const FnxGrid* g, const float* flags, const float* r, float* z, void* ws, size_t ws_bytes, void* stream) {
  if (int rc = check_pcg_grid(g, "pcg_precondition")) return rc;
  if (!flags || !r || !z) return fail(FNX_EINVAL, "pcg_precondition: NULL tensor");
  if (r == z) return fail(FNX_EINVAL, "pcg_precondition: z must not alias r");
  if (!ws || ws_bytes < ws_pcg(g)) return fail(FNX_EWORKSPACE, "pcg_precondition: workspace too small (%zu < %zu)", ws_bytes, ws_pcg(g));
  hipStream_t s = (hipStream_t)stream;
  const GridDims d = dims(g);
  char* kept = (char*)ws;
  fnx::launch_pcg_build(d, g->is3D, quirks(g), flags, kept, s);
  fnx::launch_pcg_precondition(d, g->is3D, kept, kept + ws_pcg_kept(g), r, z, s);
  HIP_OK(hipGetLastError());
  return FNX_OK;
}

int fnx_velocity_update(const FnxGrid* g, const float* p, float* U, const float* flags, void* stream) {
  if (int rc = check_grid(g)) return rc;
  if (!p || !U || !flags) return fail(FNX_EINVAL, "velocity_update: NULL tensor");
  fnx::launch_velocity_update(dims(g), g->is3D, p, U, flags, (hipStream_t)stream);
  HIP_OK(hipGetLastError());
  return FNX_OK;
}

int fnx_add_gravity(const FnxGrid* g, float* U, const float* flags, const float gravity[3], float dt, void* stream) {
  if (int rc = check_grid(g)) return rc;
  if (!U || !flags || !gravity) return fail(FNX_EINVAL, "add_gravity: NULL tensor");
  fnx::launch_add_gravity(dims(g), g->is3D, U, flags, gravity[0] * dt, gravity[1] * dt, gravity[2] * dt,
                          (hipStream_t)stream);
  HIP_OK(hipGetLastError());
  return FNX_OK;
}

int fnx_correct_scalar(const FnxGrid* g, float dt, float* src, const float* div, const float* flags, void* stream) {
  if (int rc = check_grid(g)) return rc;
  if (!src || !div || !flags) return fail(FNX_EINVAL, "correct_scalar: NULL tensor");
  fnx::launch_correct_scalar(dims(g), g->is3D, dt * 0.5f, src, div, flags, (hipStream_t)stream);
  HIP_OK(hipGetLastError());
  return FNX_OK;
}

int fnx_add_viscosity(const FnxGrid* g, float dt, const float* U_in, float* U_out, const float* flags, float viscosity,
                      void* stream) {
  if (int rc = check_grid(g)) return rc;
  if (!U_in || !U_out || !flags) return fail(FNX_EINVAL, "add_viscosity: NULL tensor");
  if (quirks(g))
    return fail(FNX_EINVAL, "add_viscosity: no 3D form with ref_quirks (the reference's 3D branch cannot run, viscosity.py never defines "
                            "mask_fluid_k: there is nothing to reproduce)");
  if (g->is3D && is_view(g)) return fail(FNX_EINVAL, "add_viscosity: no compute window or z-slab view (whole grids only)");
  if (U_in == U_out) return fail(FNX_EINVAL, "add_viscosity: U_out must not alias U_in");
  if (!(viscosity >= 0.f)) return fail(FNX_EINVAL, "add_viscosity: viscosity must be positive");
  const float coef = (float)((double)dt * (double)viscosity);
  if (g->is3D) fnx::launch_add_viscosity3d(dims(g), U_in, U_out, flags, coef, (hipStream_t)stream);
  else fnx::launch_add_viscosity(dims(g), U_in, U_out, flags, coef, (hipStream_t)stream);
  HIP_OK(hipGetLastError());
  return FNX_OK;
}

int fnx_add_vorticity_confinement(const FnxGrid* g, const float* U_in, float* U_out, const float* flags, float amp, void* stream) {
  if (!U_in || !U_out || !flags) return fail(FNX_EINVAL, "add_vorticity_confinement: NULL tensor");
  if (U_in == U_out) return fail(FNX_EINVAL, "add_vorticity_confinement: U_out must not alias U_in (a cell reads U_in three cells around it)");
  if (int rc = check_grid(g)) return rc;
  if (is_view(g))
    return fail(FNX_EINVAL, "add_vorticity_confinement: no compute window or z-slab view (whole grids only)");
  if (!(amp == amp)) return fail(FNX_EINVAL, "add_vorticity_confinement: the amplitude is NaN");
  hipStream_t s = (hipStream_t)stream;
  if (amp == 0.f) HIP_OK(hipMemcpyAsync(U_out, U_in, ncell(g) * 4 * (g->is3D ? 3 : 2), hipMemcpyDeviceToDevice, s));
  else fnx::launch_vorticity_confinement(dims(g), g->is3D, U_in, flags, U_out, amp, s);
  HIP_OK(hipGetLastError());
  return FNX_OK;
}

namespace {
int check_render(const FnxGrid* g, const FnxRenderParams* prm) {
  if (!prm) return fail(FNX_EINVAL, "render_volume: NULL parameters");
  if (int rc = check_grid(g)) return rc;
  if (is_view(g))
    return fail(FNX_EINVAL, "render_volume: no compute window or z-slab view (whole grids only)");
  if (prm->view_dir < 0 || prm->view_dir > 5 || prm->light_dir < 0 || prm->light_dir > 5)
    return fail(FNX_EINVAL, "render_volume: direction outside 0..5 (view_dir=%d light_dir=%d)", prm->view_dir, prm->light_dir);
  if (prm->bnd < 0) return fail(FNX_EINVAL, "render_volume: bnd < 0 (%d)", prm->bnd);
  const float k[2] = {prm->k_view, prm->k_light};
  for (float v : k)
    if (!(v >= 0.f) || !(v - v == 0.f))
      return fail(FNX_EINVAL, "render_volume: absorption must be finite and not negative (k_view=%g k_light=%g)", prm->k_view, prm->k_light);
  return FNX_OK;
}
}

size_t fnx_render_volume_ws_bytes(const FnxGrid* g, const FnxRenderParams* prm) {
  if (check_render(g, prm) != FNX_OK) return 0;
  return prm->view_dir == prm->light_dir ? 0 : al(ncell(g) * 4);
}

int fnx_render_volume(const FnxGrid* g, const float* density, const float* flags, const FnxRenderParams* prm, float* image,
                      void* ws, size_t ws_bytes, void* stream) {
  if (!density || !flags || !image) return fail(FNX_EINVAL, "render_volume: NULL tensor");
  if (int rc = check_render(g, prm)) return rc;
  const size_t need = prm->view_dir == prm->light_dir ? 0 : al(ncell(g) * 4);
  if (need && (!ws || ws_bytes < need)) return fail(FNX_EINVAL, "render_volume: workspace too small (%zu < %zu)", ws ? ws_bytes : (size_t)0, need);
  const fnx::RenderConsts c = {prm->k_view, prm->k_light, prm->ambient, prm->one_minus_ambient, prm->albedo_smoke, prm->albedo_obstacle,
                               prm->bnd};
  fnx::launch_render_volume(dims(g), prm->view_dir, prm->light_dir, c, density, flags, (float*)ws, image, (hipStream_t)stream);
  HIP_OK(hipGetLastError());
  return FNX_OK;
}

int fnx_add_buoyancy(const FnxGrid* g, float* U, const float* flags, const float* density, const float gravity[3],
                     float rho_star, float dt, void* stream) {
  if (int rc = check_grid(g)) return rc;
  if (!U || !flags || !density || !gravity) return fail(FNX_EINVAL, "add_buoyancy: NULL tensor");
  const float sx = gravity[0] * dt, sy = gravity[1] * dt, sz = gravity[2] * dt;
  fnx::launch_add_buoyancy(dims(g), g->is3D, quirks(g), U, flags, density, sx, sy, sz, rho_star, (hipStream_t)stream);
  HIP_OK(hipGetLastError());
  return FNX_OK;
}

int fnx_set_wall_bcs(const FnxGrid* g, float* U, const float* flags, void* stream) {
  if (int rc = check_grid(g)) return rc;
  if (!U || !flags) return fail(FNX_EINVAL, "set_wall_bcs: NULL tensor");
  fnx::launch_set_wall_bcs(dims(g), g->is3D, U, flags, (hipStream_t)stream);
  HIP_OK(hipGetLastError());
  return FNX_OK;
}

int fnx_set_wall_bcs_stick(const FnxGrid* g, const float* U_in, float* U_out, const float* flags, const float* flags_stick,
                           void* stream) {
  if (int rc = check_grid(g)) return rc;
  if (!U_in || !U_out || !flags || !flags_stick) return fail(FNX_EINVAL, "set_wall_bcs_stick: NULL tensor");
  if (quirks(g))
    return fail(FNX_EINVAL, "set_wall_bcs_stick: no 3D form with ref_quirks (the reference's 3D branch cannot run, "
                            "set_wall_bcs_stick.py:85-86: there is nothing to reproduce)");
  if (U_in == U_out) return fail(FNX_EINVAL, "set_wall_bcs_stick: U_out must not alias U_in");
  if (g->is3D) fnx::launch_set_wall_bcs_stick3d(dims(g), U_in, U_out, flags, flags_stick, (hipStream_t)stream);
  else fnx::launch_set_wall_bcs_stick(dims(g), U_in, U_out, flags, flags_stick, (hipStream_t)stream);
  HIP_OK(hipGetLastError());
  return FNX_OK;
}

int fnx_set_const_vals(const FnxGrid* g, float* U, const float* UBC, const float* UBCInvMask, float* density,
                       const float* densityBC, const float* densityBCInvMask, void* stream) {
  if (int rc = check_grid(g)) return rc;
  hipStream_t s = (hipStream_t)stream;
  if (U && UBC && UBCInvMask) fnx::launch_set_const_vals(ncell(g) * (g->is3D ? 3 : 2), U, UBC, UBCInvMask, s);
  if (density && densityBC && densityBCInvMask) fnx::launch_set_const_vals(ncell(g), density, densityBC, densityBCInvMask, s);
  HIP_OK(hipGetLastError());
  return FNX_OK;
}

int fnx_flags_to_occupancy(const FnxGrid* g, const float* flags, float* occupancy, void* stream) {
  if (int rc = check_grid(g)) return rc;
  if (!flags || !occupancy) return fail(FNX_EINVAL, "flags_to_occupancy: NULL tensor");
  fnx::launch_flags_to_occupancy(ncell(g), flags, occupancy, (hipStream_t)stream);
  HIP_OK(hipGetLastError());
  return FNX_OK;
}

int fnx_max_abs(const FnxGrid* g, const float* x, int channels, float* out_max, void* stream) {
  if (int rc = check_grid(g)) return rc;
  if (!x || !out_max || channels < 1) return fail(FNX_EINVAL, "max_abs: NULL tensor or channels < 1");
  if (((size_t)x & 15) != 0) return fail(FNX_EINVAL, "max_abs: the field must be 16-byte aligned");
  hipStream_t s = (hipStream_t)stream;
  HIP_OK(hipMemsetAsync(out_max, 0, 4, s));
  fnx::launch_max_abs(ncell(g) * (size_t)channels, x, out_max, s);
  HIP_OK(hipGetLastError());
  return FNX_OK;
}

int fnx_empty_domain(const FnxGrid* g, float* flags, int boundary_width, void* stream) {
  if (int rc = check_grid(g)) return rc;
  if (!flags) return fail(FNX_EINVAL, "empty_domain: NULL tensor");
  if (boundary_width < 1) return fail(FNX_EINVAL, "Boundary width must be greater than zero!");
  fnx::launch_empty_domain(dims(g), g->is3D, flags, boundary_width, (hipStream_t)stream);
  HIP_OK(hipGetLastError());
  return FNX_OK;
}

int fnx_create_cylinder(const FnxGrid* g, float* flags, double center_x, double center_y, double radius, void* stream) {
  if (int rc = check_grid(g)) return rc;
  if (!flags) return fail(FNX_EINVAL, "create_cylinder: NULL tensor");
  const float r2 = (float)(radius * radius);
  fnx::launch_create_cylinder(dims(g), flags, (float)center_x, (float)center_y, r2, (hipStream_t)stream);
  HIP_OK(hipGetLastError());
  return FNX_OK;
}

int fnx_create_box2d(const FnxGrid* g, float* flags, float x0, float x1, float y0, float y1, void* stream) {
  if (int rc = check_grid(g)) return rc;
  if (!flags) return fail(FNX_EINVAL, "create_box2d: NULL tensor");
  fnx::launch_create_box2d(dims(g), flags, x0, x1, y0, y1, (hipStream_t)stream);
  HIP_OK(hipGetLastError());
  return FNX_OK;
}

int fnx_get_centered(const FnxGrid* g, const float* U, float* centered, void* stream) {
  if (!g) return fail(FNX_EINVAL, "grid descriptor is NULL");
  if (g->B < 1 || g->D < 1 || g->H < 1 || g->W < 1) return fail(FNX_EINVAL, "Dimension mismatch: B=%d D=%d H=%d W=%d", g->B, g->D, g->H, g->W);
  if (!g->is3D && g->D != 1) return fail(FNX_EINVAL, "2D velocity field but zdepth > 1");
  if ((long long)g->D * g->H * g->W >= (1ll << 31)) return fail(FNX_EINVAL, "more than 2^31 cells per sample");
  if ((long long)g->B * g->D > 65535 || (g->H + 3) / 4 > 65535) return fail(FNX_EINVAL, "B*D or H/4 > 65535 not supported");
  if (!U || !centered) return fail(FNX_EINVAL, "get_centered: NULL tensor");
  if ((const float*)centered == U) return fail(FNX_EINVAL, "get_centered: the output must not alias U");
  fnx::launch_get_centered(make_dims(g->B, g->D, g->H, g->W), g->is3D, U, centered, (hipStream_t)stream);
  HIP_OK(hipGetLastError());
  return FNX_OK;
}

int fnx_velocity_divergence_backward(const FnxGrid* g, const float* grad_div, const float* flags, float* grad_U, void* stream) {
  if (int rc = check_grid(g)) return rc;
  if (!grad_div || !flags || !grad_U) return fail(FNX_EINVAL, "velocity_divergence_backward: NULL tensor");
  fnx::launch_divergence_bwd(make_dims(g->B, g->D, g->H, g->W, g->z_offset, g->D_global), g->is3D, grad_div, flags, grad_U, (hipStream_t)stream);
  HIP_OK(hipGetLastError());
  return FNX_OK;
}

int fnx_velocity_update_backward(const FnxGrid* g, const float* grad_U_out, const float* flags, float* grad_U, float* grad_p,
                                 void* stream) {
  if (int rc = check_grid(g)) return rc;
  if (!grad_U_out || !flags || !grad_U || !grad_p) return fail(FNX_EINVAL, "velocity_update_backward: NULL tensor");
  if (grad_U == grad_U_out) return fail(FNX_EINVAL, "velocity_update_backward: grad_U must not alias grad_U_out (a cell reads its +1 neighbours)");
  fnx::launch_velocity_update_bwd(make_dims(g->B, g->D, g->H, g->W, g->z_offset, g->D_global), g->is3D, grad_U_out, flags, grad_U, grad_p, (hipStream_t)stream);
  HIP_OK(hipGetLastError());
  return FNX_OK;
}

static int pre_projection(const FnxGrid* g, const fnx::StagePlan& sp, const FnxState* st, const float* U_adv, const float* rho_adv,
                          float* div, void* stream) {
  if (U_adv == st->U || (rho_adv && rho_adv == st->density)) return fail(FNX_EINVAL, "pre_projection: the advected fields must not alias the state");
  if (sp.confine && is_view(g))
    return fail(FNX_EINVAL, "pre_projection: vorticity confinement takes no compute window or z-slab view (single domain only)");
  hipStream_t s = (hipStream_t)stream;
  fnx::ProfScope ps(FNX_PROF_STAGE, s);
  const GridDims d = dims(g);
  const fnx::BcPtrs bc = fnx::bc_ptrs(st);
  const fnx::StageIO io{U_adv, rho_adv, st->flags, bc, st->U, st->density, sp.periodic ? nullptr : div};
  const fnx::StageOps all{quirks(g), true, sp.buoy, {sp.s[0], sp.s[1], sp.s[2]}, sp.rho_star, sp.grav, {sp.g[0], sp.g[1], sp.g[2]},
                          sp.wall, sp.second_bcs, d.K0 + d.KN};
  if (!sp.confine) {
    GridDims ds = d;
    if (g->is3D && div && ds.K0 + ds.KN < ds.D) ds.KN += 1;
    fnx::launch_pre_projection(ds, g->is3D, io, all, s);
    if (sp.periodic) fnx::launch_periodic_pre(ds, g->is3D, U_adv, bc.UBC, bc.UBCInvMask, st->U, sp.px, sp.py, s, false);
  } else {
    fnx::StageIO io1 = io;
    io1.div = nullptr;
    fnx::StageOps upto_gravity = all;
    upto_gravity.wall = false; upto_gravity.second_bcs = false; upto_gravity.div_k_end = 0;
    fnx::launch_pre_projection(d, g->is3D, io1, upto_gravity, s);
    float* U_scr = const_cast<float*>(U_adv);
    fnx::launch_vorticity_confinement(d, g->is3D, st->U, st->flags, U_scr, sp.amp, s);
    fnx::StageIO io3 = io;
    io3.rho_adv = nullptr; io3.rho = nullptr; io3.bc.rhoBC = nullptr; io3.bc.rhoBCInvMask = nullptr;
    fnx::StageOps from_walls = all;
    from_walls.first_bcs = false; from_walls.buoy = false; from_walls.grav = false;
    fnx::launch_pre_projection(d, g->is3D, io3, from_walls, s);
    if (sp.periodic) fnx::launch_periodic_pre(d, g->is3D, U_scr, bc.UBC, bc.UBCInvMask, st->U, sp.px, sp.py, s, true);
  }
  if (sp.periodic && div) fnx::launch_divergence(d, g->is3D, st->U, st->flags, div, s);
  if (sp.confine && rho_adv && bc.rhoBC && sp.second_bcs) fnx::launch_set_const_vals(ncell(g), st->density, bc.rhoBC, bc.rhoBCInvMask, s);
  HIP_OK(hipGetLastError());
  return FNX_OK;
}

int fnx_pre_projection(const FnxGrid* g, const FnxStepParams* prm, const FnxState* st, const float* U_adv,
                       const float* rho_adv, float* div, void* stream) {
  if (int rc = check_grid(g)) return rc;
  if (!prm || !st || !st->U || !st->flags || !U_adv) return fail(FNX_EINVAL, "pre_projection: NULL state");
  if (rho_adv && !st->density) return fail(FNX_EINVAL, "pre_projection: rho_adv given but state has no density");
  return pre_projection(g, fnx::stage_plan(prm, rho_adv != nullptr, st->flags_stick != nullptr), st, U_adv, rho_adv, div, stream);
}

int fnx_post_projection(const FnxGrid* g, const FnxState* st, void* stream) {
  if (int rc = check_grid(g)) return rc;
  if (!st || !st->U || !st->flags || !st->p) return fail(FNX_EINVAL, "post_projection: NULL state");
  fnx::ProfScope ps(FNX_PROF_STAGE, (hipStream_t)stream);
  fnx::launch_post_projection(dims(g), g->is3D, st->p, st->U, st->density, st->flags, fnx::bc_ptrs(st), (hipStream_t)stream,
                              st->density_bc_applied != 0);
  HIP_OK(hipGetLastError());
  return FNX_OK;
}

int fnx_bc_classify(const FnxGrid* g, const FnxState* st, unsigned char* bc_class, void* stream) {
  if (int rc = check_grid(g)) return rc;
  if (!st || !bc_class) return fail(FNX_EINVAL, "bc_classify: NULL argument");
  fnx::launch_bc_classify(dims(g), g->is3D, fnx::bc_ptrs(st), bc_class, (hipStream_t)stream);
  HIP_OK(hipGetLastError());
  return FNX_OK;
}

int fnx_simulate_step(const FnxGrid* g, const FnxStepParams* prm, const FnxState* st, void* ws, size_t ws_bytes,
                      void* stream) {
  using fnx::StepAdvect; using fnx::StepClassMap; using fnx::StepProjection; using fnx::StepTail;
  if (int rc = check_grid(g)) return rc;
  if (!prm || !st || !st->p || !st->U || !st->flags) return fail(FNX_EINVAL, "simulate_step: NULL state");
  if (prm->method < 0 || prm->method > 4) return fail(FNX_EINVAL, "Simulation method not supported. Choose convnet, jacobi, pcg or hybrid.");
  const bool pcg = prm->method >= 2;
  if (pcg && prm->pcg_iter < 1) return fail(FNX_EINVAL, "At least 1 iteration of the solver is needed (pcg_iter < 1)");
  if (pcg && is_view(g))
    return fail(FNX_EINVAL, "simulate_step: the PCG solve takes no compute window or z-slab view (single domain only)");
  if (prm->vorticity_confinement > 0.f && is_view(g))
    return fail(FNX_EINVAL, "simulate_step: vorticity confinement takes no compute window or z-slab view (single domain only)");
  if (prm->method == 1 && !st->net) return fail(FNX_EINVAL, "simulate_step: convnet method needs packed weights");
  if (prm->method == 3 && !st->net) return fail(FNX_EINVAL, "simulate_step: hybrid method needs packed weights");
  if (prm->method == 3 && fnx::net_mode(prm->precision_mode) < 0) return fail(FNX_EINVAL, "simulate_step: unknown precision_mode %d", prm->precision_mode);
  const fnx::StepLayout L = carve_step(g, ws);
  if (!ws || ws_bytes < L.bytes) return fail(FNX_EWORKSPACE, "simulate_step: workspace too small (%zu < %zu)", ws_bytes, L.bytes);
  const bool has_rho = st->density != nullptr;
  const fnx::StepPlan plan = fnx::step_plan(prm, has_rho, st->flags_stick != nullptr, st->UBC || st->densityBC);
  if (prm->viscosity < 0.f) return fail(FNX_EINVAL, "Viscosity must be positive");
  if (prm->vorticity_confinement != prm->vorticity_confinement) return fail(FNX_EINVAL, "simulate_step: vorticity_confinement is NaN");
  if (plan.viscous && g->is3D) return fail(FNX_EINVAL, "simulate_step: viscosity is 2D only (reference viscosity.py:5)");
  if (plan.projection == StepProjection::NET_STICK && g->is3D) return fail(FNX_EINVAL, "simulate_step: flags_stick is 2D only (set_wall_bcs_stick.py:85-86)");
  hipStream_t s = (hipStream_t)stream;
  const GridDims d = dims(g);
  const size_t nc = g->is3D ? 3 : 2;

  if (plan.viscous) {
    if (int rc = fnx_add_viscosity(g, prm->dt, st->U, L.orig, st->flags, prm->viscosity, stream)) return rc;
  }
  if (plan.advect == StepAdvect::PAIR) {
    if (int rc = fnx_advect_step(g, prm->dt, st->density, st->U, st->flags, L.rho2, L.U2, prm->sample_outside_fluid,
                                 prm->maccormack_strength, L.tail, L.tail_bytes, stream)) return rc;
  } else {
    if (plan.advect == StepAdvect::RHO_THEN_VEL) {
      if (int rc = fnx_advect_scalar(g, prm->dt, st->density, st->U, st->flags, L.rho2, FNX_ADVECT_MACCORMACK, 1,
                                     prm->sample_outside_fluid, prm->maccormack_strength, L.tail, L.tail_bytes, stream)) return rc;
    }
    if (int rc = fnx_advect_vel(g, prm->dt, plan.viscous ? L.orig : st->U, st->U, st->flags, L.U2, FNX_ADVECT_MACCORMACK, 1,
                                prm->maccormack_strength, L.tail, L.tail_bytes, stream)) return rc;
  }
  if (plan.correct_scalar) {
    fnx::launch_divergence(d, g->is3D, st->U, st->flags, L.div, s);
    if (int rc = fnx_correct_scalar(g, prm->dt, L.rho2, L.div, st->flags, stream)) return rc;
  }
  FnxState stc = *st;
  if (plan.class_map == StepClassMap::BUILD) { if (int rc = fnx_bc_classify(g, st, L.cls, stream)) return rc; }
  stc.bc_class = plan.class_map == StepClassMap::NONE ? nullptr : L.cls;
  stc.density_bc_applied = 1;
  st = &stc;
  if (int rc = pre_projection(g, plan.stage, st, L.U2, has_rho ? L.rho2 : nullptr, plan.solve ? L.div : nullptr, stream)) return rc;

  auto stick_then_bcs = [&]() -> int {
    if (int rc = fnx_set_wall_bcs_stick(g, st->U, L.U2, st->flags, st->flags_stick, stream)) return rc;
    HIP_OK(hipMemcpyAsync(st->U, L.U2, ncell(g) * 4 * nc, hipMemcpyDeviceToDevice, s));
    return fnx_set_const_vals(g, st->U, st->UBC, st->UBCInvMask, st->density, st->densityBC, st->densityBCInvMask, stream);
  };
  switch (plan.projection) {
    case StepProjection::JACOBI:
      if (int rc = jacobi_solve(g, st->flags, L.div, st->p, nullptr, prm->p_tol, prm->jacobi_iter, nullptr, L.tail, L.tail_bytes, L.mask,
                                plan.reuse_mask, stream, 0)) return rc;
      break;
    case StepProjection::PCG_COLD: case StepProjection::PCG_FROM_NET: case StepProjection::PCG_FROM_P: {
      if (plan.pcg_rebuild) fnx::launch_pcg_build(d, g->is3D, quirks(g), st->flags, L.pcg_kept, s);
      if (plan.projection == StepProjection::PCG_FROM_NET) {
        if (int rc = fnx::fluidnet_pressure(g, st->net, st->flags, prm->normalize_threshold, fnx::net_mode(prm->precision_mode), st->p, st->U,
                                            L.tail, stream)) return rc;
      }
      const float* p0 = plan.projection == StepProjection::PCG_COLD ? nullptr : st->p;
      if (int rc = fnx::pcg_solve(d, g->is3D, L.pcg_kept, L.tail, L.div, p0, st->p, nullptr, prm->pcg_tol, prm->pcg_iter, nullptr, false, s)) return rc;
      break;
    }
    case StepProjection::NET_STICK:
      if (int rc = stick_then_bcs()) return rc;
      [[fallthrough]];
    case StepProjection::NET_FUSED: {
      const int mode = fnx::net_mode(prm->precision_mode);
      if (mode < 0) return fail(FNX_EINVAL, "simulate_step: unknown precision_mode %d", prm->precision_mode);
      if (int rc = fnx::fluidnet_core(g, st->net, st->flags, prm->normalize_threshold, mode, st->p, st->U, L.tail, stream,
                                      plan.projection == StepProjection::NET_FUSED ? st : nullptr)) return rc;
      break;
    }
  }
  switch (plan.tail) {
    case StepTail::POST:
      if (int rc = fnx_post_projection(g, st, stream)) return rc;
      break;
    case StepTail::POST_PERIODIC: {
      const fnx::BcPtrs bc = fnx::bc_ptrs(st);
      fnx::launch_periodic_post(d, g->is3D, st->U, (float*)L.tail, nullptr, nullptr, plan.stage.px, plan.stage.py, 0, s);
      if (int rc = fnx_post_projection(g, st, stream)) return rc;
      fnx::launch_periodic_post(d, g->is3D, st->U, (float*)L.tail, bc.UBC, bc.UBCInvMask, plan.stage.px, plan.stage.py, 1, s);
      break;
    }
    case StepTail::STICK_BCS:
      if (int rc = stick_then_bcs()) return rc;
      break;
    case StepTail::NONE:
      break;
  }
  HIP_OK(hipGetLastError());
  return FNX_OK;
}

}
```

fluidnet_cxx_amd/csrc/fnx_kernels.h:

```cpp
#pragma once
#include <hip/hip_runtime.h>
#include "fnx_device.h"
#include "fnx_jacobi_plan.h"
#include "fnx_step_plan.h"

namespace fnx {

int set_error(int code, const char* fmt, ...);

bool prof_begin(int tag, hipStream_t s);
void prof_end(int tag, hipStream_t s, bool pushed);
void prof_add_work(int tag, double amount);
struct ProfScope {
  int tag; hipStream_t s; bool pushed;
  ProfScope(int t, hipStream_t st) : tag(t), s(st), pushed(prof_begin(t, st)) {}
  ~ProfScope() { prof_end(tag, s, pushed); }
};

enum { ADVECT_RHO = 1, ADVECT_VEL = 2, ADVECT_BOTH = 3 };
enum class AdvectPath { CELLS, TILES_2D, TILES_3D };
struct AdvectPlan {
  GridDims g, gfwd;
  bool is3d, quirks;
  int what;
  bool maccormack;
  AdvectPath fwd, bwd;
  bool bwd_fused;
  bool cells_pair;
};
AdvectPlan advect_plan(const GridDims& g, bool is3d, bool quirks, int what, bool orig_is_U, int method, int request);
struct AdvectWs { float* rho_fwd; int* cell; float2* box; float* U_fwd; unsigned long long* fix; size_t bytes; };
AdvectWs advect_workspace(const GridDims& g, bool is3d, int what, void* base);
struct AdvectArgs {
  float dt, half_s; bool sample_outside;
  const float *rho, *orig, *U, *flags;
  float *rho_dst, *U_dst;
};
void launch_advect(const AdvectPlan& p, const AdvectArgs& a, const AdvectWs& ws, hipStream_t s);

struct AdvectScalarsWs { float* fwd; int* cell; float2* box; size_t bytes; };
AdvectScalarsWs advect_scalars_workspace(const GridDims& g, bool is3d, int channels, void* base);
inline int advect_scalars_box_chunks(const GridDims& g) { return (g.D + 15) / 16; }
void launch_advect_scalars(const GridDims& g, bool is3d, bool quirks, bool maccormack, bool sample_outside, float dt, float half_s,
                           int channels, const float* src, const float* U, const float* flags, float* dst, const AdvectScalarsWs& w,
                           hipStream_t s);

void launch_divergence(const GridDims& g, bool is3d, const float* U, const float* flags, float* div, hipStream_t s);
void launch_velocity_update(const GridDims& g, bool is3d, const float* p, float* U, const float* flags, hipStream_t s);
void launch_add_gravity(const GridDims& g, bool is3d, float* U, const float* flags, float fx, float fy, float fz,
                        hipStream_t s);
void launch_correct_scalar(const GridDims& g, bool is3d, float half_dt, float* src, const float* div, const float* flags,
                           hipStream_t s);
void launch_add_viscosity(const GridDims& g, const float* Uin, float* Uout, const float* flags, float coef,
                          hipStream_t s);
void launch_add_buoyancy(const GridDims& g, bool is3d, bool quirks, float* U, const float* flags, const float* rho,
                         float sx, float sy, float sz, float rho_star, hipStream_t s);
void launch_set_wall_bcs(const GridDims& g, bool is3d, float* U, const float* flags, hipStream_t s);
void launch_set_wall_bcs_stick(const GridDims& g, const float* Uin, float* Uout, const float* flags, const float* stick,
                               hipStream_t s);
void launch_set_const_vals(size_t n, float* x, const float* bc, const float* inv_mask, hipStream_t s);
void launch_flags_to_occupancy(size_t n, const float* flags, float* occ, hipStream_t s);
void launch_max_abs(size_t n, const float* x, float* out, hipStream_t s);
void launch_empty_domain(const GridDims& g, bool is3d, float* flags, int bnd, hipStream_t s);
void launch_create_cylinder(const GridDims& g, float* flags, float cx, float cy, float r2, hipStream_t s);
void launch_create_box2d(const GridDims& g, float* flags, float x0, float x1, float y0, float y1, hipStream_t s);
void launch_get_centered(const GridDims& g, bool is3d, const float* U, float* out, hipStream_t s);
void launch_divergence_bwd(const GridDims& g, bool is3d, const float* gdiv, const float* flags, float* gU, hipStream_t s);
void launch_velocity_update_bwd(const GridDims& g, bool is3d, const float* gout, const float* flags, float* gU, float* gp,
                                hipStream_t s);

void launch_add_viscosity3d(const GridDims& g, const float* Uin, float* Uout, const float* flags, float coef, hipStream_t s);
void launch_set_wall_bcs_stick3d(const GridDims& g, const float* Uin, float* Uout, const float* flags, const float* stick,
                                 hipStream_t s);

struct BcPtrs { const float *UBC, *UBCInvMask, *rhoBC, *rhoBCInvMask; const unsigned char* cls; };
inline BcPtrs bc_ptrs(const FnxState* st) {
  const bool ubc = st->UBC && st->UBCInvMask, rbc = st->densityBC && st->densityBCInvMask;
  return BcPtrs{ubc ? st->UBC : nullptr, ubc ? st->UBCInvMask : nullptr, rbc ? st->densityBC : nullptr, rbc ? st->densityBCInvMask : nullptr,
                st->bc_class};
}
struct StageIO {
  const float *U_adv, *rho_adv, *flags;
  BcPtrs bc;
  float *U, *rho, *div;
};
struct StageOps {
  bool quirks;
  bool first_bcs;
  bool buoy; float s[3];
  float rho_star;
  bool grav; float g[3];
  bool wall;
  bool second_bcs;
  int div_k_end;
};
void launch_pre_projection(const GridDims& g, bool is3d, const StageIO& io, const StageOps& ops, hipStream_t s);
void launch_periodic_pre(const GridDims& g, bool is3d, const float* U_adv, const float* UBC, const float* UBCInvMask, float* U,
                         bool px, bool py, hipStream_t s, bool staged = false);
size_t periodic_save_bytes(const GridDims& g);
void launch_periodic_post(const GridDims& g, bool is3d, float* U, float* save, const float* UBC, const float* UBCInvMask,
                          bool px, bool py, int mode, hipStream_t s);
void launch_post_projection(const GridDims& g, bool is3d, const float* p, float* U, float* rho, const float* flags, const BcPtrs& bc,
                            hipStream_t s, bool rho_bc_applied = false, const float* scale = nullptr, float* p_scaled = nullptr);
void launch_bc_classify(const GridDims& g, bool is3d, const BcPtrs& bc, unsigned char* cls, hipStream_t s);

void launch_vorticity_confinement(const GridDims& g, bool is3d, const float* U_in, const float* flags, float* U_out, float amp,
                                  hipStream_t s);

struct RenderConsts { float k_view, k_light, ambient, one_minus_ambient, albedo_smoke, albedo_obstacle; int bnd; };
void launch_render_volume(const GridDims& g, int view_dir, int light_dir, const RenderConsts& c, const float* density, const float* flags,
                          float* Lws, float* image, hipStream_t s);

void launch_jacobi(const GridDims& g, const float* flags, const float* div, const float* p_in, float* p_out, int nsweeps,
                   bool from_zero, hipStream_t s);
void launch_jacobi3d_mask(const GridDims& g, bool quirks, const float* flags, const JacobiMaskLayout& mask, hipStream_t s);
void launch_jacobi3d(const GridDims& g, const JacobiMaskLayout& mask, const float* div, const float* p_in, float* p_out,
                     bool from_zero, hipStream_t s, int kb = 0, int ke = 0);
struct JacobiMirror { float* out[2][2]; const unsigned* sel[2]; int k[2]; int n; unsigned long long bstride; unsigned long long* clock; };
void launch_jacobi3d_x2(const GridDims& g, const JacobiMaskLayout& mask, const float* div, const float* p_in, float* p_out,
                        hipStream_t s, int kb = 0, int ke = 0, bool from_zero = false, int kb2 = -1, int lay = 0,
                        const JacobiMirror* mirror = nullptr);
size_t residual_scratch_bytes(int B);
void launch_residual(int B, size_t per_sample, size_t first, size_t count, const float* a, const float* b, double* partials,
                     float* sumsq, float* res, hipStream_t s);
void launch_residual_root(int B, const float* sumsq, float* res, hipStream_t s);

size_t pcg_kept_bytes(const GridDims& g, bool is3d);
size_t pcg_scratch_bytes(const GridDims& g, bool is3d);
void launch_pcg_build(const GridDims& g, bool is3d, bool quirks, const float* flags, void* kept, hipStream_t s);
void launch_poisson_apply(const GridDims& g, bool is3d, bool quirks, const float* flags, const float* x, float* y, hipStream_t s);
void launch_pcg_precondition(const GridDims& g, bool is3d, const void* kept, void* scratch, const float* r, float* z, hipStream_t s);
int pcg_solve(const GridDims& g, bool is3d, const void* kept, void* scratch, const float* div, const float* p0, float* p, float* residual,
              float tol, int max_iter, int* iters_done, bool verbose, hipStream_t s);

}
```

fluidnet_cxx_amd/csrc/fnx_step.hip:

```cpp
#include "fnx_device.h"
#include "fnx_kernels.h"

namespace {

constexpr int BX = 64, BY = 4;

struct StepPtrs {
  const float* U_adv; const float* rho_adv;
  const float* flags;
  const float* UBC; const float* UBCInvMask;
  const float* rhoBC; const float* rhoBCInvMask;
  float* U; float* rho; float* div;
  const unsigned char* cls;
  int grav; float gx, gy, gz;
  int bc2;
};

__device__ __forceinline__ bool gravity_applies(float fc, float fm) {
  return (fc == FNX_FLUID || fc == FNX_EMPTY) && (fm == FNX_FLUID || (fm == FNX_EMPTY && fc == FNX_FLUID));
}

template <bool QUIRKS, bool WALL, bool BC1 = true>
__device__ __forceinline__ float stage_eval3d(int a, float v, bool ubc, float um, float uc, float fc, float fm, bool border, bool buoy,
                                              float r0, float r1, bool rbc, float rm0, float rc0, float rm1, float rc1, float s_a,
                                              float rho_star, bool grav, float g_a, bool bc2, int kg, int k) {
  if (ubc && BC1) { const float t = v * um; v = t + uc; }
  if (buoy && !border && fc == FNX_FLUID && fm == FNX_FLUID) {
    float q0 = r0, q1 = r1;
    if (rbc) { float t = q0 * rm0; q0 = t + rc0; t = q1 * rm1; q1 = t + rc1; }
    if (a == 2 && QUIRKS) v = v + s_a * (0.5f * (q0 + (kg <= 1 ? 0.f : q1)));
    else v = v + s_a * ((0.5f * (q0 + q1)) - rho_star);
  }
  if (grav && !border && gravity_applies(fc, fm)) v = v + g_a;
  if (WALL && (fc == FNX_FLUID || fc == FNX_OBST)) {
    if (!(a == 2 && (kg == 0 || k == 0))) {
      if (fm == FNX_OBST || (fc == FNX_OBST && fm == FNX_FLUID)) v = 0.f;
    }
  }
  if (ubc && bc2) { const float t = v * um; v = t + uc; }
  return v;
}

template <bool QUIRKS, bool WALL, bool DIV, bool BC1 = true>
__global__ __launch_bounds__(BX* BY) void stage3d_kernel(GridDims g, StepPtrs P, int buoy, float sx, float sy, float sz,
                                                         float rho_star, int kdiv) {
  const int i = blockIdx.x * BX + threadIdx.x, j = blockIdx.y * BY + threadIdx.y;
  const int bk = blockIdx.z;
  const int b = bk / g.KN, k = g.K0 + (bk - b * g.KN);
  if (i >= g.W || j >= g.H) return;
  const size_t o = (size_t)k * g.HW + j * g.W + i, os = (size_t)b * g.DHW + o;
  const int off[3] = { i > 0 ? 1 : 0, j > 0 ? g.W : 0, k > 0 ? g.HW : 0 };
  const bool want_div = DIV && k < kdiv;
  const int offp[3] = { i + 1 < g.W ? 1 : 0, j + 1 < g.H ? g.W : 0, k + 1 < g.D ? g.HW : 0 };
  const bool has_rho = P.rho_adv != nullptr, ubc = P.UBC != nullptr, rbc = P.rhoBC != nullptr;
  bool ident = false;
  if (P.cls) {
    bool mine = P.cls[os] == 3;
#pragma unroll
    for (int a = 0; a < 3; ++a) mine = mine & ((P.cls[os - off[a]] & 2) != 0);
    if (want_div) {
#pragma unroll
      for (int a = 0; a < 3; ++a) mine = mine & (P.cls[os + offp[a]] == 3);
    }
    ident = __builtin_amdgcn_ballot_w64(!mine) == 0;
  }
  const float fc = P.flags[os];
  float fm[3], u[3], r1[3] = { 0.f, 0.f, 0.f }, r0 = 0.f;
#pragma unroll
  for (int a = 0; a < 3; ++a) { fm[a] = P.flags[os - off[a]]; u[a] = P.U_adv[((size_t)b * 3 + a) * g.DHW + o]; }
  if (has_rho) {
    r0 = P.rho_adv[os];
#pragma unroll
    for (int a = 0; a < 3; ++a) r1[a] = P.rho_adv[os - off[a]];
  }
  float fp[3] = { 0.f, 0.f, 0.f }, up[3] = { 0.f, 0.f, 0.f }, rp[3] = { 0.f, 0.f, 0.f };
  if (want_div) {
#pragma unroll
    for (int a = 0; a < 3; ++a) { fp[a] = P.flags[os + offp[a]]; up[a] = P.U_adv[((size_t)b * 3 + a) * g.DHW + o + offp[a]]; }
    if (has_rho) {
#pragma unroll
      for (int a = 0; a < 3; ++a) rp[a] = P.rho_adv[os + offp[a]];
    }
  }
  float um[3] = { 1.f, 1.f, 1.f }, uc[3] = { 0.f, 0.f, 0.f }, rm0 = 1.f, rc0 = 0.f, rm1[3] = { 1.f, 1.f, 1.f }, rc1[3] = { 0.f, 0.f, 0.f };
  float ump[3] = { 1.f, 1.f, 1.f }, ucp[3] = { 0.f, 0.f, 0.f }, rmp[3] = { 1.f, 1.f, 1.f }, rcp[3] = { 0.f, 0.f, 0.f };
  if (!ident) {
    if (ubc) {
#pragma unroll
      for (int a = 0; a < 3; ++a) { um[a] = P.UBCInvMask[((size_t)b * 3 + a) * g.DHW + o]; uc[a] = P.UBC[((size_t)b * 3 + a) * g.DHW + o]; }
      if (want_div) {
#pragma unroll
        for (int a = 0; a < 3; ++a) { ump[a] = P.UBCInvMask[((size_t)b * 3 + a) * g.DHW + o + offp[a]]; ucp[a] = P.UBC[((size_t)b * 3 + a) * g.DHW + o + offp[a]]; }
      }
    }
    if (rbc && has_rho) {
      rm0 = P.rhoBCInvMask[os]; rc0 = P.rhoBC[os];
#pragma unroll
      for (int a = 0; a < 3; ++a) { rm1[a] = P.rhoBCInvMask[os - off[a]]; rc1[a] = P.rhoBC[os - off[a]]; }
      if (want_div) {
#pragma unroll
        for (int a = 0; a < 3; ++a) { rmp[a] = P.rhoBCInvMask[os + offp[a]]; rcp[a] = P.rhoBC[os + offp[a]]; }
      }
    }
  }
  const bool border = is_border<true>(g, i, j, k);
  const float sa[3] = { sx, sy, sz };
  const float ga[3] = { P.gx, P.gy, P.gz };
  const bool by = buoy && has_rho, gr = P.grav && has_rho, rb = rbc && has_rho;
  float un[3];
#pragma unroll
  for (int a = 0; a < 3; ++a)
    un[a] = stage_eval3d<QUIRKS, WALL, BC1>(a, u[a], ubc, um[a], uc[a], fc, fm[a], border, by, r0, r1[a], rb, rm0, rc0, rm1[a], rc1[a], sa[a],
                                       rho_star, gr, ga[a], P.bc2 != 0, k + g.zoff, k);
  float rnew = r0;
  if (has_rho && rbc) {
    float t = rnew * rm0; rnew = t + rc0;
    if (P.bc2) { t = rnew * rm0; rnew = t + rc0; }
  }
#pragma unroll
  for (int a = 0; a < 3; ++a) P.U[((size_t)b * 3 + a) * g.DHW + o] = un[a];
  if (has_rho) P.rho[os] = rnew;
  if (want_div) {
    float d = 0.f;
    if (!border) {
      float vp[3];
#pragma unroll
      for (int a = 0; a < 3; ++a) {
        const bool bp = is_border<true>(g, i + (a == 0), j + (a == 1), k + (a == 2));
        vp[a] = stage_eval3d<QUIRKS, WALL, BC1>(a, up[a], ubc, ump[a], ucp[a], fp[a], fc, bp, by, rp[a], r0, rb, rmp[a], rcp[a], rm0, rc0, sa[a],
                                           rho_star, gr, ga[a], P.bc2 != 0, k + (a == 2) + g.zoff, k + (a == 2));
      }
      d = ((un[0] - vp[0]) + un[1]) - vp[1];
      d = d + (un[2] - vp[2]);
    }
    if (fc == FNX_OBST) d = 0.f;
    P.div[os] = d;
  }
}

template <bool WALL, bool BC1 = true>
__device__ __forceinline__ float stage_eval2d(int a, float u, bool ubc, float um, float uc, float fc, float fm, bool border,
                                              bool buoy, float r0, float r1, bool rbc, float rm0, float rc0, float rm1,
                                              float rc1, float s_a, float rho_star, bool grav, float g_a, bool bc2) {
  if (ubc && BC1) { const float t = u * um; u = t + uc; }
  if (buoy && !border && fc == FNX_FLUID && fm == FNX_FLUID) {
    if (rbc) { float t = r0 * rm0; r0 = t + rc0; t = r1 * rm1; r1 = t + rc1; }
    u = u + s_a * ((0.5f * (r0 + r1)) - rho_star);
  }
  if (grav && !border && gravity_applies(fc, fm)) u = u + g_a;
  if (WALL && (fc == FNX_FLUID || fc == FNX_OBST)) {
    if (fm == FNX_OBST || (fc == FNX_OBST && fm == FNX_FLUID)) u = 0.f;
  }
  if (ubc && bc2) { const float t = u * um; u = t + uc; }
  (void)a;
  return u;
}

template <bool WALL, bool BC1 = true>
__global__ __launch_bounds__(BX* BY) void stage2d_div_kernel(GridDims g, StepPtrs P, int buoy_, float sx, float sy,
                                                             float rho_star) {
  const int i = blockIdx.x * BX + threadIdx.x, j = blockIdx.y * BY + threadIdx.y;
  const int b = blockIdx.z;
  if (i >= g.W || j >= g.H) return;
  const size_t o = (size_t)j * g.W + i, os = (size_t)b * g.DHW + o;
  const bool has_rho = P.rho_adv != nullptr, ubc = P.UBC != nullptr, rbc = P.rhoBC != nullptr && has_rho;
  const bool buoy = buoy_ != 0 && has_rho;
  const bool grav = P.grav != 0 && has_rho, bc2 = P.bc2 != 0;
  const int xm = i > 0 ? 1 : 0, ym = j > 0 ? g.W : 0, xp = i < g.W - 1 ? 1 : 0, yp = j < g.H - 1 ? g.W : 0;
  bool ident = false;
  if (P.cls) {
    const bool mine = (P.cls[os] == 3) & ((P.cls[os - xm] & 2) != 0) & ((P.cls[os - ym] & 2) != 0) & (P.cls[os + xp] == 3) &
                      (P.cls[os + yp] == 3);
    ident = __builtin_amdgcn_ballot_w64(!mine) == 0;
  }
  const float F00 = P.flags[os], Fm0 = P.flags[os - xm], F0m = P.flags[os - ym], Fp0 = P.flags[os + xp], F0p = P.flags[os + yp];
  const size_t o0 = ((size_t)b * 2 + 0) * g.DHW + o, o1 = ((size_t)b * 2 + 1) * g.DHW + o;
  const float u0 = P.U_adv[o0], u1 = P.U_adv[o1], u0p = P.U_adv[o0 + xp], u1p = P.U_adv[o1 + yp];
  float R00 = 0.f, Rm0 = 0.f, R0m = 0.f, Rp0 = 0.f, R0p = 0.f;
  if (has_rho) { R00 = P.rho_adv[os]; Rm0 = P.rho_adv[os - xm]; R0m = P.rho_adv[os - ym]; Rp0 = P.rho_adv[os + xp]; R0p = P.rho_adv[os + yp]; }
  float m0 = 1.f, c0 = 0.f, m1 = 1.f, c1 = 0.f, m0p = 1.f, c0p = 0.f, m1p = 1.f, c1p = 0.f;
  float rm00 = 1.f, rc00 = 0.f, rmm0 = 1.f, rcm0 = 0.f, rm0m = 1.f, rc0m = 0.f, rmp0 = 1.f, rcp0 = 0.f, rm0p = 1.f, rc0p = 0.f;
  if (!ident) {
    if (ubc) {
      m0 = P.UBCInvMask[o0]; c0 = P.UBC[o0]; m1 = P.UBCInvMask[o1]; c1 = P.UBC[o1];
      m0p = P.UBCInvMask[o0 + xp]; c0p = P.UBC[o0 + xp]; m1p = P.UBCInvMask[o1 + yp]; c1p = P.UBC[o1 + yp];
    }
    if (rbc) {
      rm00 = P.rhoBCInvMask[os]; rc00 = P.rhoBC[os]; rmm0 = P.rhoBCInvMask[os - xm]; rcm0 = P.rhoBC[os - xm];
      rm0m = P.rhoBCInvMask[os - ym]; rc0m = P.rhoBC[os - ym]; rmp0 = P.rhoBCInvMask[os + xp]; rcp0 = P.rhoBC[os + xp];
      rm0p = P.rhoBCInvMask[os + yp]; rc0p = P.rhoBC[os + yp];
    }
  }
  const bool border = is_border<false>(g, i, j, 0);
  const float v0 = stage_eval2d<WALL, BC1>(0, u0, ubc, m0, c0, F00, Fm0, border, buoy, R00, Rm0, rbc, rm00, rc00, rmm0, rcm0, sx, rho_star, grav, P.gx, bc2);
  const float v1 = stage_eval2d<WALL, BC1>(1, u1, ubc, m1, c1, F00, F0m, border, buoy, R00, R0m, rbc, rm00, rc00, rm0m, rc0m, sy, rho_star, grav, P.gy, bc2);
  float rnew = R00;
  if (rbc) { float t = rnew * rm00; rnew = t + rc00; if (bc2) { t = rnew * rm00; rnew = t + rc00; } }
  float d = 0.f;
  if (P.div) {
    if (!border) {
      const float v0p = stage_eval2d<WALL, BC1>(0, u0p, ubc, m0p, c0p, Fp0, F00, is_border<false>(g, i + 1, j, 0), buoy, Rp0, R00, rbc,
                                           rmp0, rcp0, rm00, rc00, sx, rho_star, grav, P.gx, bc2);
      const float v1p = stage_eval2d<WALL, BC1>(1, u1p, ubc, m1p, c1p, F0p, F00, is_border<false>(g, i, j + 1, 0), buoy, R0p, R00, rbc,
                                           rm0p, rc0p, rm00, rc00, sy, rho_star, grav, P.gy, bc2);
      d = ((v0 - v0p) + v1) - v1p;
    }
    if (F00 == FNX_OBST) d = 0.f;
  }
  P.U[o0] = v0;
  P.U[o1] = v1;
  if (has_rho) P.rho[os] = rnew;
  if (P.div) P.div[os] = d;
}

template <bool IS3D, bool SCALE>
__global__ __launch_bounds__(BX* BY) void post_projection_kernel(GridDims g, const float* __restrict__ p,
                                                                 float* __restrict__ U, float* __restrict__ rho,
                                                                 const float* __restrict__ flags,
                                                                 const float* __restrict__ UBC,
                                                                 const float* __restrict__ UBCInvMask,
                                                                 const float* __restrict__ rhoBC,
                                                                 const float* __restrict__ rhoBCInvMask,
                                                                 const unsigned char* __restrict__ cls, int rho_done,
                                                                 const float* __restrict__ scale, float* __restrict__ p_scaled) {
  const int i = blockIdx.x * BX + threadIdx.x, j = blockIdx.y * BY + threadIdx.y;
  const int bk = blockIdx.z;
  const int b = IS3D ? bk / g.KN : bk, k = IS3D ? g.K0 + (bk - b * g.KN) : 0;
  if (i >= g.W || j >= g.H) return;
  constexpr int NC = IS3D ? 3 : 2;
  const size_t o = (size_t)k * g.HW + j * g.W + i, os = (size_t)b * g.DHW + o;
  const float fc = flags[os], P = p[os];
  const unsigned cl = cls ? cls[os] : 0u;
  const bool border = is_border<IS3D>(g, i, j, k);
  const float sc = SCALE ? scale[b] : 1.f;
  float fm[NC], Pm[NC], u[NC], bm[NC], bc[NC];
  size_t ou[NC];
  const bool need_u = UBC != nullptr && !(cl & 1);
  const bool load_u = __builtin_amdgcn_ballot_w64(need_u) != 0;
  const bool do_rho = rho != nullptr && rhoBC != nullptr && !(rho_done && (cl & 2));
  const bool need_r = do_rho && !(cl & 2);
  const bool load_rho = __builtin_amdgcn_ballot_w64(do_rho) != 0, load_r = __builtin_amdgcn_ballot_w64(need_r) != 0;
#pragma unroll
  for (int a = 0; a < NC; ++a) {
    ou[a] = ((size_t)b * NC + a) * g.DHW + o;
    const int off = a == 0 ? 1 : (a == 1 ? g.W : g.HW);
    const int idx = a == 0 ? i : (a == 1 ? j : k);
    const int offs = idx > 0 ? off : 0;
    fm[a] = flags[os - offs];
    Pm[a] = p[os - offs];
    u[a] = U[ou[a]];
    bm[a] = 1.f; bc[a] = 0.f;
  }
  if (load_u) {
#pragma unroll
    for (int a = 0; a < NC; ++a) { bm[a] = UBCInvMask[ou[a]]; bc[a] = UBC[ou[a]]; }
  }
  float r0 = 0.f, rm = 1.f, rc = 0.f;
  if (load_rho) r0 = rho[os];
  if (load_r) { rm = rhoBCInvMask[os]; rc = rhoBC[os]; }
  if (SCALE) p_scaled[os] = P * sc;
#pragma unroll
  for (int a = 0; a < NC; ++a) {
    float v = u[a];
    if (SCALE) v = v / sc;
    {
      const float m_ff = (fc == FNX_FLUID && fm[a] == FNX_FLUID) ? 1.f : 0.f;
      float w;
      if (!IS3D) {
        const float m_fe = (fc == FNX_FLUID && fm[a] == FNX_EMPTY) ? 1.f : 0.f;
        const float m_ef = (fc == FNX_EMPTY && fm[a] == FNX_FLUID) ? 1.f : 0.f;
        const float m_nf = (fc == FNX_EMPTY && fm[a] == FNX_EMPTY) ? 1.f : 0.f;
        w = ((m_ff * (v - (P - Pm[a])) + m_fe * (v - P)) + m_ef * (v + Pm[a])) + m_nf * 0.f;
      } else {
        w = m_ff * (v - (P - Pm[a]));
      }
      v = border ? v : w;
    }
    if (SCALE) v = v * sc;
    {
      const bool zface = a == 2 && (k + g.zoff == 0 || k == 0);
      const bool wall = (fc == FNX_FLUID || fc == FNX_OBST) && !zface && (fm[a] == FNX_OBST || (fc == FNX_OBST && fm[a] == FNX_FLUID));
      v = wall ? 0.f : v;
    }
    if (UBC) {
      const float m = need_u ? bm[a] : 1.f, c = need_u ? bc[a] : 0.f;
      const float t = v * m; v = t + c;
    }
    U[ou[a]] = v;
  }
  if (do_rho) {
    const float m = need_r ? rm : 1.f, c = need_r ? rc : 0.f;
    const float t = r0 * m; rho[os] = t + c;
  }
}

__global__ __launch_bounds__(256) void bc_classify_kernel(size_t n, size_t dhw, int nc, const float* __restrict__ UBC,
                                                          const float* __restrict__ UBCInvMask,
                                                          const float* __restrict__ rhoBC,
                                                          const float* __restrict__ rhoBCInvMask,
                                                          unsigned char* __restrict__ cls) {
  for (size_t q = (size_t)blockIdx.x * 256 + threadIdx.x; q < n; q += (size_t)gridDim.x * 256) {
    const size_t b = q / dhw, o = q - b * dhw;
    unsigned c = 0;
    if (UBC && UBCInvMask) {
      bool id = true;
      for (int a = 0; a < nc; ++a) {
        const size_t ou = (b * nc + a) * dhw + o;
        id = id & (UBCInvMask[ou] == 1.f) & (__float_as_uint(UBC[ou]) == 0u);
      }
      c |= id ? 1u : 0u;
    }
    if (rhoBC && rhoBCInvMask) c |= ((rhoBCInvMask[q] == 1.f) & (__float_as_uint(rhoBC[q]) == 0u)) ? 2u : 0u;
    cls[q] = (unsigned char)c;
  }
}

__global__ __launch_bounds__(256) void periodic_pre_kernel(GridDims g, int nc, const float* __restrict__ U_adv,
                                                           const float* __restrict__ UBC, const float* __restrict__ UBCInvMask,
                                                           float* __restrict__ U, int px, int py, int staged) {
  const int t = blockIdx.x * 256 + threadIdx.x;
  const int bk = blockIdx.y, b = bk / g.KN, k = g.K0 + (bk - b * g.KN);
  if (t >= g.H + g.W) return;
  const bool xp = t < g.H;
  if (xp ? !px : !py) return;
  const int a = xp ? 1 : 0;
  const size_t base = ((size_t)b * nc + a) * g.DHW + (size_t)k * g.HW;
  const size_t src = base + (xp ? (size_t)t * g.W + (g.W - 1) : (size_t)(g.H - 1) * g.W + (t - g.H));
  const size_t dst = base + (xp ? (size_t)t * g.W + 1 : (size_t)g.W + (t - g.H));
  float v = U_adv[src];
  if (UBC) {
    float q;
    if (!staged) { q = v * UBCInvMask[src]; v = q + UBC[src]; }
    q = v * UBCInvMask[dst]; v = q + UBC[dst];
  }
  U[dst] = v;
}

__global__ __launch_bounds__(256) void periodic_post_kernel(GridDims g, int nc, float* __restrict__ U, float* __restrict__ save,
                                                            const float* __restrict__ UBC, const float* __restrict__ UBCInvMask,
                                                            int px, int py, int mode) {
  const int t = blockIdx.x * 256 + threadIdx.x;
  const int bk = blockIdx.y, b = bk / g.KN, k = g.K0 + (bk - b * g.KN);
  if (t >= g.H + g.W) return;
  const bool xp = t < g.H;
  if (xp ? !px : !py) return;
  const int a = xp ? 1 : 0;
  const size_t base = ((size_t)b * nc + a) * g.DHW + (size_t)k * g.HW;
  const size_t src = base + (xp ? (size_t)t * g.W + (g.W - 1) : (size_t)(g.H - 1) * g.W + (t - g.H));
  const size_t dst = base + (xp ? (size_t)t * g.W + 1 : (size_t)g.W + (t - g.H));
  float* sv = save + (size_t)bk * (g.H + g.W) + t;
  if (mode == 0) { *sv = U[src]; return; }
  float v = *sv;
  if (UBC) { const float q = v * UBCInvMask[dst]; v = q + UBC[dst]; }
  U[dst] = v;
}

inline dim3 cell_grid(const GridDims& g) { return dim3((g.W + BX - 1) / BX, (g.H + BY - 1) / BY, g.B * g.KN); }

}

namespace fnx {

namespace {
using Stage2d = void (*)(GridDims, StepPtrs, int, float, float, float);
using Stage3d = void (*)(GridDims, StepPtrs, int, float, float, float, float, int);
struct StageKernel { Stage2d k2; Stage3d k3; };
template <bool Q, bool BC1> Stage3d stage3d_of(bool wall, bool div) {
  return wall ? (div ? stage3d_kernel<Q, true, true, BC1> : stage3d_kernel<Q, true, false, BC1>)
              : (div ? stage3d_kernel<Q, false, true, BC1> : stage3d_kernel<Q, false, false, BC1>);
}
StageKernel stage_kernel(bool is3d, const StageOps& o, bool div) {
  if (!is3d) {
    return {o.first_bcs ? (o.wall ? stage2d_div_kernel<true, true> : stage2d_div_kernel<false, true>)
                        : (o.wall ? stage2d_div_kernel<true, false> : stage2d_div_kernel<false, false>), nullptr};
  }
  return {nullptr, !o.first_bcs ? stage3d_of<false, false>(o.wall, div) : o.quirks ? stage3d_of<true, true>(o.wall, div) : stage3d_of<false, true>(o.wall, div)};
}
}

void launch_pre_projection(const GridDims& g, bool is3d, const StageIO& io, const StageOps& o, hipStream_t s) {
  const StepPtrs P{io.U_adv, io.rho_adv, io.flags, io.bc.UBC, io.bc.UBCInvMask, io.bc.rhoBC, io.bc.rhoBCInvMask, io.U, io.rho, io.div, io.bc.cls,
                   o.grav ? 1 : 0, o.g[0], o.g[1], o.g[2], o.second_bcs ? 1 : 0};
  const dim3 grid = cell_grid(g), block(BX, BY);
  const StageKernel k = stage_kernel(is3d, o, io.div != nullptr);
  auto launch = [&](auto kernel, auto... rest) { kernel<<<grid, block, 0, s>>>(g, P, o.buoy ? 1 : 0, o.s[0], o.s[1], rest...); };
  if (is3d) launch(k.k3, o.s[2], o.rho_star, io.div ? o.div_k_end : 0);
  else launch(k.k2, o.rho_star);
}

void launch_post_projection(const GridDims& g, bool is3d, const float* p, float* U, float* rho, const float* flags, const BcPtrs& bc,
                            hipStream_t s, bool rho_bc_applied, const float* scale, float* p_scaled) {
  const dim3 grid = cell_grid(g), block(BX, BY);
  const int rd = (bc.cls && rho_bc_applied) ? 1 : 0;
  const bool scaled = scale && p_scaled;
  auto k = scaled ? (is3d ? post_projection_kernel<true, true> : post_projection_kernel<false, true>)
                  : (is3d ? post_projection_kernel<true, false> : post_projection_kernel<false, false>);
  k<<<grid, block, 0, s>>>(g, p, U, rho, flags, bc.UBC, bc.UBCInvMask, bc.rhoBC, bc.rhoBCInvMask, bc.cls, rd, scaled ? scale : nullptr,
                           scaled ? p_scaled : nullptr);
}

void launch_periodic_pre(const GridDims& g, bool is3d, const float* U_adv, const float* UBC, const float* UBCInvMask, float* U,
                         bool px, bool py, hipStream_t s, bool staged) {
  const dim3 grid((g.H + g.W + 255) / 256, g.B * g.KN);
  periodic_pre_kernel<<<grid, 256, 0, s>>>(g, is3d ? 3 : 2, U_adv, UBC, UBCInvMask, U, px, py, staged ? 1 : 0);
}

size_t periodic_save_bytes(const GridDims& g) { return (size_t)g.B * g.KN * (g.H + g.W) * sizeof(float); }

void launch_periodic_post(const GridDims& g, bool is3d, float* U, float* save, const float* UBC, const float* UBCInvMask,
                          bool px, bool py, int mode, hipStream_t s) {
  const dim3 grid((g.H + g.W + 255) / 256, g.B * g.KN);
  periodic_post_kernel<<<grid, 256, 0, s>>>(g, is3d ? 3 : 2, U, save, UBC, UBCInvMask, px, py, mode);
}

void launch_bc_classify(const GridDims& g, bool is3d, const BcPtrs& bc, unsigned char* cls, hipStream_t s) {
  const size_t n = (size_t)g.B * g.DHW;
  size_t blocks = (n + 255) / 256;
  if (blocks > 8192) blocks = 8192;
  bc_classify_kernel<<<(unsigned)blocks, 256, 0, s>>>(n, (size_t)g.DHW, is3d ? 3 : 2, bc.UBC, bc.UBCInvMask, bc.rhoBC, bc.rhoBCInvMask, cls);
}

}
```

fluidnet_cxx_amd/csrc/fnx_step_plan.h:

```cpp
#pragma once
#include <stddef.h>

#include "../../include/fluidnet_hip.h"

namespace fnx {

struct StepLayout {
  float *rho2, *U2, *div;
  unsigned char *mask, *cls;
  void* pcg_kept;
  float* orig;
  void* tail;
  size_t tail_bytes, bytes;
};
inline StepLayout step_layout(size_t cells, size_t nc, bool is3d, size_t mask_bytes, size_t pcg_kept_bytes, size_t tail_need, void* base) {
  size_t off = 0;
  auto take = [&](size_t bytes) { void* r = base ? (char*)base + off : nullptr; off += (bytes + 255) & ~(size_t)255; return r; };
  StepLayout L{};
  L.rho2 = (float*)take(cells * 4);
  L.U2 = (float*)take(cells * 4 * nc);
  L.div = (float*)take(cells * 4);
  if (is3d) L.mask = (unsigned char*)take(mask_bytes);
  L.cls = (unsigned char*)take(cells);
  L.pcg_kept = take(pcg_kept_bytes);
  if (!is3d) L.orig = (float*)take(cells * 4 * nc);
  L.tail = take(0);
  L.tail_bytes = tail_need;
  L.bytes = off + tail_need;
  return L;
}

struct StagePlan {
  bool buoy; float s[3];
  float rho_star;
  bool grav; float g[3];
  bool wall;
  bool periodic, px, py;
  bool second_bcs;
  bool confine; float amp;
};
inline StagePlan stage_plan(const FnxStepParams* prm, bool has_rho, bool has_stick) {
  StagePlan p{};
  p.buoy = has_rho && prm->buoyancy_scale > 0.f;
  p.rho_star = prm->operating_density;
  if (p.buoy) {
    const float ns = -prm->buoyancy_scale;
    const float gx = prm->gravity_vec[0] * ns, gy = prm->gravity_vec[1] * ns, gz = prm->gravity_vec[2] * ns;
    p.s[0] = gx * prm->dt; p.s[1] = gy * prm->dt; p.s[2] = gz * prm->dt;
  }
  p.grav = has_rho && prm->gravity_scale > 0.f;
  if (p.grav) {
    const float ns = -prm->gravity_scale;
    for (int a = 0; a < 3; ++a) p.g[a] = (prm->gravity_vec[a] * ns) * prm->dt;
  }
  p.wall = prm->method != 1;
  p.periodic = p.wall && (prm->periodic & 1);
  p.px = (prm->periodic & 2) != 0;
  p.py = (prm->periodic & 4) != 0;
  p.second_bcs = !(prm->method == 1 && has_stick);
  p.confine = prm->vorticity_confinement > 0.f;
  p.amp = prm->vorticity_confinement;
  return p;
}

enum class StepAdvect { PAIR, RHO_THEN_VEL, VEL_ONLY };
enum class StepClassMap { NONE, BUILD, REUSE };
enum class StepProjection { JACOBI, PCG_COLD, PCG_FROM_NET, PCG_FROM_P, NET_FUSED, NET_STICK };
enum class StepTail { POST, POST_PERIODIC, STICK_BCS, NONE };
struct StepPlan {
  bool viscous;
  StepAdvect advect;
  bool correct_scalar;
  StepClassMap class_map;
  StagePlan stage;
  StepProjection projection;
  bool solve;
  bool pcg_rebuild;
  bool reuse_mask;
  StepTail tail;
};
inline StepPlan step_plan(const FnxStepParams* prm, bool has_rho, bool has_stick, bool has_bc) {
  StepPlan p{};
  p.viscous = prm->viscosity > 0.f;
  p.advect = !has_rho ? StepAdvect::VEL_ONLY : p.viscous ? StepAdvect::RHO_THEN_VEL : StepAdvect::PAIR;
  p.correct_scalar = has_rho && prm->correct_scalar;
  p.class_map = !((prm->static_flags & 2) && has_bc) ? StepClassMap::NONE : (prm->static_flags & 4) ? StepClassMap::REUSE : StepClassMap::BUILD;
  p.stage = stage_plan(prm, has_rho, has_stick);
  switch (prm->method) {
    case 0: p.projection = StepProjection::JACOBI; break;
    case 1: p.projection = has_stick ? StepProjection::NET_STICK : StepProjection::NET_FUSED; break;
    case 2: p.projection = StepProjection::PCG_COLD; break;
    case 3: p.projection = StepProjection::PCG_FROM_NET; break;
    default: p.projection = StepProjection::PCG_FROM_P; break;
  }
  p.solve = prm->method != 1;
  p.pcg_rebuild = (prm->static_flags & 9) != 9;
  p.reuse_mask = (prm->static_flags & 1) != 0;
  p.tail = p.projection == StepProjection::NET_FUSED ? StepTail::NONE
         : p.projection == StepProjection::NET_STICK ? StepTail::STICK_BCS
         : p.stage.periodic ? StepTail::POST_PERIODIC : StepTail::POST;
  return p;
}

}
```

include/fluidnet_hip.h:

```cpp
#ifndef FLUIDNET_HIP_H
#define FLUIDNET_HIP_H

#include <stddef.h>
#include <stdint.h>

#ifdef __cplusplus
extern "C" {
#endif

#define FNX_ABI_VERSION 32

enum {
  FNX_OK = 0,
  FNX_EINVAL = 1,
  FNX_EMETHOD = 2,
  FNX_EWORKSPACE = 3,
  FNX_EHIP = 4,
  FNX_ECFL = 5,
  FNX_ECOMM = 6
};

enum { FNX_TYPE_NONE = 0, FNX_TYPE_FLUID = 1, FNX_TYPE_OBSTACLE = 2, FNX_TYPE_EMPTY = 4,
       FNX_TYPE_INFLOW = 8, FNX_TYPE_OUTFLOW = 16, FNX_TYPE_OPEN = 32, FNX_TYPE_STICK = 128 };

enum { FNX_ADVECT_EULER = 0, FNX_ADVECT_MACCORMACK = 1 };

typedef struct FnxGrid {
  int B, D, H, W;
  int is3D;
  int ref_quirks;
  int z_offset, D_global;
  int k_begin, k_end;
} FnxGrid;

enum { FNX_OP_ADVECT_SCALAR = 0, FNX_OP_ADVECT_VEL = 1, FNX_OP_JACOBI = 2, FNX_OP_STEP = 3, FNX_OP_FLUIDNET = 4,
       FNX_OP_ADVECT_STEP = 5 };
size_t fnx_workspace_bytes(const FnxGrid* g, int op);

const char* fnx_last_error(void);
int fnx_abi_version(void);
const char* fnx_device_name(void);

int fnx_advect_scalar(const FnxGrid* g, float dt, const float* src, const float* U, const float* flags,
                      float* dst, int method, int bnd, int sample_outside_fluid, float maccormack_strength,
                      void* ws, size_t ws_bytes, void* stream);

int fnx_advect_vel(const FnxGrid* g, float dt, const float* orig, const float* U, const float* flags,
                   float* dst, int method, int bnd, float maccormack_strength,
                   void* ws, size_t ws_bytes, void* stream);

int fnx_advect_step(const FnxGrid* g, float dt, const float* density, const float* U, const float* flags,
                    float* density_dst, float* U_dst, int sample_outside, float strength, void* ws, size_t ws_bytes,
                    void* stream);
enum { FNX_ADVECT_PLAN_AUTO = 0,
       FNX_ADVECT_PLAN_TILES = 1,
       FNX_ADVECT_PLAN_CELLS = 2,
       FNX_ADVECT_PLAN_TILES_SPLIT = 3 };
int fnx_advect_step_plan(const FnxGrid* g, float dt, const float* density, const float* U, const float* flags,
                         float* density_dst, float* U_dst, int sample_outside, float strength, int plan, void* ws,
                         size_t ws_bytes, void* stream);
int fnx_advect_scalar_plan(const FnxGrid* g, float dt, const float* src, const float* U, const float* flags,
                           float* dst, int method, int bnd, int sample_outside_fluid, float maccormack_strength, int plan,
                           void* ws, size_t ws_bytes, void* stream);
int fnx_advect_vel_plan(const FnxGrid* g, float dt, const float* orig, const float* U, const float* flags,
                        float* dst, int method, int bnd, float maccormack_strength, int plan,
                        void* ws, size_t ws_bytes, void* stream);

size_t fnx_advect_scalars_workspace_bytes(const FnxGrid* g, int channels);
int fnx_advect_scalars(const FnxGrid* g, float dt, int channels, const float* src, const float* U, const float* flags,
                       float* dst, int method, int bnd, int sample_outside_fluid, float maccormack_strength,
                       void* ws, size_t ws_bytes, void* stream);

int fnx_velocity_divergence(const FnxGrid* g, const float* U, const float* flags, float* div, void* stream);

int fnx_jacobi(const FnxGrid* g, const float* flags, const float* div, float* p, float* residual,
               float p_tol, int max_iter, int* iters_done, void* ws, size_t ws_bytes, void* stream);
int fnx_jacobi_verbose(const FnxGrid* g, const float* flags, const float* div, float* p, float* residual,
                       float p_tol, int max_iter, int* iters_done, void* ws, size_t ws_bytes, void* stream);
int fnx_residual(const FnxGrid* g, const float* a, const float* b, float* sumsq, float* residual, void* ws, size_t ws_bytes, void* stream);

int fnx_jacobi_sweeps(const FnxGrid* g, const float* flags, const float* div, float* p, int nsweeps,
                      void* ws, size_t ws_bytes, void* stream);
int fnx_jacobi_sweeps_ex(const FnxGrid* g, const float* flags, const float* div, float* p, int nsweeps,
                         void* ws, size_t ws_bytes, int reuse_mask, void* stream);

int fnx_jacobi_pass(const FnxGrid* g, const float* flags, const float* div, const float* p_in, float* p_out,
                    int nsweeps, int k_begin, int k_end, void* ws, size_t ws_bytes, int reuse_mask, void* stream);
int fnx_jacobi_pass2(const FnxGrid* g, const float* flags, const float* div, const float* p_in, float* p_out,
                     int nsweeps, int k_begin, int k_end, int k_begin2, void* ws, size_t ws_bytes, int reuse_mask,
                     void* stream);
int fnx_jacobi_quad_ok(const FnxGrid* g);
int fnx_jacobi_pass_layout(const FnxGrid* g, const float* flags, const float* div, const float* p_in, float* p_out,
                           int nsweeps, int k_begin, int k_end, int k_begin2, int layout, void* ws, size_t ws_bytes,
                           int reuse_mask, void* stream);

typedef struct FnxPlaneMirror {
  float* out[2][2]; const unsigned* slot_select[2]; int k_first[2]; int planes; size_t sample_stride;
  unsigned long long* start_clock;
} FnxPlaneMirror;
int fnx_jacobi_pass_mirror_ok(const FnxGrid* g, int planes_per_range, int two_ranges, int layout);
int fnx_jacobi_pass_mirror(const FnxGrid* g, const float* flags, const float* div, const float* p_in, float* p_out, int k_begin,
                           int k_end, int k_begin2, int layout, const FnxPlaneMirror* mirror, void* ws, size_t ws_bytes,
                           int reuse_mask, void* stream);

size_t fnx_pcg_workspace_bytes(const FnxGrid* g);
int fnx_pcg(const FnxGrid* g, const float* flags, const float* div, float* p, float* residual, float p_tol, int max_iter,
            int* iters_done, void* ws, size_t ws_bytes, void* stream);
int fnx_pcg_verbose(const FnxGrid* g, const float* flags, const float* div, float* p, float* residual, float p_tol, int max_iter,
                    int* iters_done, void* ws, size_t ws_bytes, void* stream);
int fnx_pcg_from(const FnxGrid* g, const float* flags, const float* div, const float* p0, float* p, float* residual, float p_tol,
                 int max_iter, int* iters_done, void* ws, size_t ws_bytes, void* stream);
int fnx_pcg_from_verbose(const FnxGrid* g, const float* flags, const float* div, const float* p0, float* p, float* residual, float p_tol,
                         int max_iter, int* iters_done, void* ws, size_t ws_bytes, void* stream);
int fnx_poisson_apply(const FnxGrid* g, const float* flags, const float* p, float* Ap, void* stream);
int fnx_pcg_precondition(const FnxGrid* g, const float* flags, const float* r, float* z, void* ws, size_t ws_bytes, void* stream);

int fnx_velocity_update(const FnxGrid* g, const float* p, float* U, const float* flags, void* stream);

int fnx_add_buoyancy(const FnxGrid* g, float* U, const float* flags, const float* density,
                     const float gravity[3], float rho_star, float dt, void* stream);

int fnx_add_gravity(const FnxGrid* g, float* U, const float* flags, const float gravity[3], float dt, void* stream);

int fnx_correct_scalar(const FnxGrid* g, float dt, float* src, const float* div, const float* flags, void* stream);

int fnx_add_viscosity(const FnxGrid* g, float dt, const float* U_in, float* U_out, const float* flags,
                      float viscosity, void* stream);

int fnx_add_vorticity_confinement(const FnxGrid* g, const float* U_in, float* U_out, const float* flags, float amp,
                                  void* stream);

typedef struct FnxRenderParams {
  int view_dir, light_dir;
  float k_view, k_light;
  float ambient, one_minus_ambient, albedo_smoke, albedo_obstacle;
  int bnd;
} FnxRenderParams;
size_t fnx_render_volume_ws_bytes(const FnxGrid* g, const FnxRenderParams* prm);
int fnx_render_volume(const FnxGrid* g, const float* density, const float* flags, const FnxRenderParams* prm, float* image,
                      void* ws, size_t ws_bytes, void* stream);

int fnx_set_wall_bcs(const FnxGrid* g, float* U, const float* flags, void* stream);

int fnx_set_wall_bcs_stick(const FnxGrid* g, const float* U_in, float* U_out, const float* flags,
                           const float* flags_stick, void* stream);

int fnx_set_const_vals(const FnxGrid* g, float* U, const float* UBC, const float* UBCInvMask,
                       float* density, const float* densityBC, const float* densityBCInvMask, void* stream);

int fnx_flags_to_occupancy(const FnxGrid* g, const float* flags, float* occupancy, void* stream);

int fnx_max_abs(const FnxGrid* g, const float* x, int channels, float* out_max, void* stream);

int fnx_empty_domain(const FnxGrid* g, float* flags, int boundary_width, void* stream);

int fnx_create_cylinder(const FnxGrid* g, float* flags, double center_x, double center_y, double radius, void* stream);
int fnx_create_box2d(const FnxGrid* g, float* flags, float x0, float x1, float y0, float y1, void* stream);
int fnx_get_centered(const FnxGrid* g, const float* U, float* centered, void* stream);

typedef struct FnxStepParams {
  float dt;
  float maccormack_strength;
  int   sample_outside_fluid;
  float buoyancy_scale;
  float gravity_vec[3];
  float operating_density;
  float p_tol;
  int   jacobi_iter;
  int   method;
  float normalize_threshold;
  int   precision_mode;
  int   static_flags;
  float viscosity;
  float gravity_scale;
  int   correct_scalar;
  int   periodic;
  float pcg_tol;
  int   pcg_iter;
  float vorticity_confinement;
} FnxStepParams;

typedef struct FnxState {
  float* p;
  float* U;
  float* density;
  const float* flags;
  const float* UBC; const float* UBCInvMask;
  const float* densityBC; const float* densityBCInvMask;
  const void*  net;
  const unsigned char* bc_class;
  const float* flags_stick;
  int density_bc_applied;
} FnxState;

int fnx_bc_classify(const FnxGrid* g, const FnxState* st, unsigned char* bc_class, void* stream);

int fnx_simulate_step(const FnxGrid* g, const FnxStepParams* prm, const FnxState* st,
                      void* ws, size_t ws_bytes, void* stream);

int fnx_pre_projection(const FnxGrid* g, const FnxStepParams* prm, const FnxState* st, const float* U_adv,
                       const float* rho_adv, float* div, void* stream);
int fnx_post_projection(const FnxGrid* g, const FnxState* st, void* stream);

int fnx_velocity_divergence_backward(const FnxGrid* g, const float* grad_div, const float* flags, float* grad_U, void* stream);
int fnx_velocity_update_backward(const FnxGrid* g, const float* grad_U_out, const float* flags, float* grad_U, float* grad_p,
                                 void* stream);

typedef struct FnxSlabSeg {
  const void* send_lo; void* recv_lo;
  const void* send_hi; void* recv_hi;
  size_t bytes;
} FnxSlabSeg;
typedef struct FnxSlabComm {
  void* ctx;
  int (*exchange)(void* ctx, const FnxSlabSeg* segs, int nsegs, void* stream);
  int (*allreduce_max)(void* ctx, float* x, int n, void* stream);
  int (*allreduce_sum)(void* ctx, float* x, int n, void* stream);
  void (*destroy)(void* ctx);
  void (*abort)(void* ctx);
  int (*direct_begin)(void* ctx, size_t bytes, int nsegs, void* dst[2][2], const unsigned* select[2], size_t* seg_stride,
                      void** start_clock, void* stream);
  int (*direct_exchange)(void* ctx, const FnxSlabSeg* segs, int nsegs, void* stream);
} FnxSlabComm;
int fnx_slab_rccl_unique_id(void* out128);
int fnx_slab_comm_rccl(FnxSlabComm* out, int rank, int nranks, const void* unique_id128);
int fnx_slab_loopback_group(void** group, int nranks);
int fnx_slab_loopback_group_set_timeout(void* group, double seconds);
int fnx_slab_loopback_group_reset(void* group);
int fnx_slab_comm_loopback(FnxSlabComm* out, void* group, int rank);
void fnx_slab_loopback_group_free(void* group);
int fnx_slab_comm_link_model(FnxSlabComm* out, double latency_us, double gbytes_per_s);
#define FNX_PEER_HANDLE_BYTES 128
int fnx_slab_peer_create(void** peer, int rank, int nranks, size_t mailbox_bytes, void* handle_out);
int fnx_slab_peer_set_timeout(void* peer, double seconds);
int fnx_slab_peer_failed(void* peer);
int fnx_slab_comm_peer(FnxSlabComm* out, void* peer, const void* handle_lo, const void* handle_hi);
void fnx_slab_peer_free(void* peer);
void fnx_slab_comm_free(FnxSlabComm* comm);

#define FNX_SLAB_MAX_HALO 64
enum { FNX_SLAB_DEEP_FIRST = 0, FNX_SLAB_EDGE_FIRST = 1, FNX_SLAB_LAST_PASS = 2, FNX_SLAB_DEEP_BESIDE = 3 };
typedef struct FnxSlabConfig {
  int B, H, W, D_global;
  int rank, nranks;
  int halo;
  int sweeps_per_exchange;
  int static_flags;
  int cfl_check_every;
  int schedule;
  int method;
  int direct_sends;
} FnxSlabConfig;
#define FNX_SLAB_NET_MARGIN 48
#define FNX_SLAB_NET_MARGIN_FULL 8
#define FNX_SLAB_NET_MARGIN_HALF 24
typedef struct FnxSlab FnxSlab;
int fnx_slab_layout(const FnxSlabConfig* cfg, int* owned, int* ghost_lo, int* ghost_hi, int* z_offset);
size_t fnx_slab_workspace_bytes(const FnxSlabConfig* cfg);
int fnx_slab_create(FnxSlab** out, const FnxSlabConfig* cfg, const FnxSlabComm* comm);
void fnx_slab_destroy(FnxSlab* s);
int fnx_slab_step(FnxSlab* s, const FnxStepParams* prm, const FnxState* st, void* ws, size_t ws_bytes, void* stream);

typedef struct FnxSlabStats {
  double bytes_per_neighbour;
  double wait_ms;
  long long exchanges;
} FnxSlabStats;
int fnx_slab_stats_enable(FnxSlab* s, int on);
int fnx_slab_stats_read(FnxSlab* s, FnxSlabStats* out);
int fnx_slab_comm_probe(const FnxSlabComm* comm, void* scratch, size_t bytes, int reps, float* ms_per_exchange, void* stream);

size_t fnx_scalenet_weight_floats(int is3D);
size_t fnx_scalenet_packed_bytes(int is3D);
int fnx_scalenet_pack(int is3D, const float* weights_blob, void* packed, void* stream);
enum { FNX_PRECISION_FP32 = 0, FNX_PRECISION_FP32_DIRECT = 1, FNX_PRECISION_BF16X6 = 2, FNX_PRECISION_BF16X3 = 3, FNX_PRECISION_FP32_F4 = 4,
       FNX_PRECISION_FP32_F2 = 5 };
int fnx_multiscale_forward(const FnxGrid* g, const void* packed, const float* x, float* p, int precision_mode,
                           void* ws, size_t ws_bytes, void* stream);
int fnx_multiscale_forward_crop(const FnxGrid* g, const void* packed, const float* x, float* p, int precision_mode,
                                const int trim[4], void* ws, size_t ws_bytes, void* stream);
int fnx_fluidnet_forward(const FnxGrid* g, const void* packed, const float* input, float normalize_threshold,
                         float* p_out, float* U_out, int precision_mode, void* ws, size_t ws_bytes, void* stream);

size_t fnx_banknet_weight_floats(void);
size_t fnx_banknet_packed_bytes(void);
int fnx_banknet_pack(const float* weights_blob, void* packed, void* stream);
size_t fnx_banknet_ws_bytes(const FnxGrid* g, int whole_forward);
int fnx_banknet_forward(const FnxGrid* g, const void* packed, const float* x, float* p, int precision_mode, void* ws, size_t ws_bytes,
                        void* stream);
int fnx_fluidnet_bank_forward(const FnxGrid* g, const void* packed, const float* input, float normalize_threshold, float* p_out,
                              float* U_out, int precision_mode, void* ws, size_t ws_bytes, void* stream);

size_t fnx_banknet3d_weight_floats(void);
size_t fnx_banknet3d_packed_bytes(void);
int fnx_banknet3d_pack(const float* weights_blob, void* packed, void* stream);
size_t fnx_banknet3d_ws_bytes(const FnxGrid* g, int whole_forward);
int fnx_banknet3d_launch_plan(const FnxGrid* g, int level, int plan[6]);
int fnx_banknet3d_forward(const FnxGrid* g, const void* packed, const float* x, float* p, int precision_mode, void* ws, size_t ws_bytes,
                          void* stream);
int fnx_fluidnet_bank3d_forward(const FnxGrid* g, const void* packed, const float* input, float normalize_threshold, float* p_out,
                                float* U_out, int precision_mode, void* ws, size_t ws_bytes, void* stream);

typedef struct FnxTapeEntry {
  char name[8];
  size_t offset;
  int C, H, W;
} FnxTapeEntry;
int fnx_multiscale_tape_entries(void);
size_t fnx_multiscale_tape_layout(const FnxGrid* g, FnxTapeEntry* entries);
size_t fnx_scalenet_packed_t_bytes(void);
int fnx_scalenet_pack_t(const float* weights_blob, void* packed_t, void* stream);
size_t fnx_multiscale_backward_ws_bytes(const FnxGrid* g);
int fnx_multiscale_forward_train(const FnxGrid* g, const void* packed, const float* x, float* p, float* tape, int precision_mode,
                                 void* stream);
int fnx_multiscale_backward(const FnxGrid* g, const void* packed_t, const float* grad_p, const float* tape, float* grad_blob,
                            int precision_mode, void* ws, size_t ws_bytes, void* stream);
int fnx_multiscale_backward_plain(const FnxGrid* g, const void* packed_t, const float* grad_p, const float* tape, float* grad_blob,
                                  int precision_mode, void* ws, size_t ws_bytes, void* stream);
size_t fnx_fluidnet_train_ws_bytes(const FnxGrid* g);
int fnx_fluidnet_forward_train(const FnxGrid* g, const void* packed, const float* input, float normalize_threshold, float* p_out,
                               float* U_out, float* flags_out, float* scale_out, float* tape, int precision_mode, void* ws, size_t ws_bytes,
                               void* stream);
int fnx_fluidnet_backward(const FnxGrid* g, const void* packed_t, const float* flags, const float* scale, const float* grad_p,
                          const float* grad_U, const float* tape, float* grad_blob, int precision_mode, void* ws, size_t ws_bytes,
                          void* stream);

int fnx_banknet_tape_entries(void);
size_t fnx_banknet_tape_layout(const FnxGrid* g, FnxTapeEntry* entries);
size_t fnx_banknet_packed_t_bytes(void);
int fnx_banknet_pack_t(const float* weights_blob, void* packed_t, void* stream);
size_t fnx_banknet_backward_ws_bytes(const FnxGrid* g);
int fnx_banknet_forward_train(const FnxGrid* g, const void* packed, const float* x, float* p, float* tape, int precision_mode, void* stream);
int fnx_banknet_backward(const FnxGrid* g, const void* packed_t, const float* x, const float* grad_p, const float* tape, float* grad_blob,
                         int precision_mode, void* ws, size_t ws_bytes, void* stream);
size_t fnx_fluidnet_bank_train_ws_bytes(const FnxGrid* g);
int fnx_fluidnet_bank_forward_train(const FnxGrid* g, const void* packed, const float* input, float normalize_threshold, float* p_out,
                                    float* U_out, float* flags_out, float* scale_out, float* tape, int precision_mode, void* ws,
                                    size_t ws_bytes, void* stream);
int fnx_fluidnet_bank_backward(const FnxGrid* g, const void* packed_t, const float* flags, const float* scale, const float* grad_p,
// ... 65 lines not shown
```

Baseline: 5482 Mcells/s.

## Pack per-cell neighbour flags and BC class into a cached 32-bit stage word

Adds a precomputed per-cell 32-bit word that encodes the cell's flag code, the six neighbour flag codes and the BC class bits. The 3D stage and post-projection kernels read this one word instead of seven float flag loads and several class-byte loads. When static flags permit, the word is reused across steps; otherwise a build kernel regenerates it each step. This cuts memory traffic in the bandwidth-bound stage kernels, at the cost of extra workspace and, when not reused, an extra kernel pass.

```diff
diff --git a/fluidnet_cxx_amd/csrc/fluidnet_cpp.cpp b/fluidnet_cxx_amd/csrc/fluidnet_cpp.cpp
--- a/fluidnet_cxx_amd/csrc/fluidnet_cpp.cpp
+++ b/fluidnet_cxx_amd/csrc/fluidnet_cpp.cpp
@@ -1182,7 +1182,7 @@
 
 int64_t step_workspace_bytes(int B, int D, int H, int W, bool is3D) {
   FnxGrid g{B, D, H, W, is3D ? 1 : 0, 0, 0, 0};
-  return (int64_t)fnx_workspace_bytes(&g, FNX_OP_STEP);
+  return (int64_t)fnx_workspace_bytes(&g, FNX_OP_STEP_STATIC);
 }
 
 }
diff --git a/fluidnet_cxx_amd/csrc/fnx_api.hip b/fluidnet_cxx_amd/csrc/fnx_api.hip
--- a/fluidnet_cxx_amd/csrc/fnx_api.hip
+++ b/fluidnet_cxx_amd/csrc/fnx_api.hip
@@ -85,6 +85,10 @@
   return fnx::step_layout(ncell(g), g->is3D ? 3 : 2, g->is3D != 0, ws_mask(g), ws_pcg_kept(g), tail_need, ws);
 }
 size_t ws_step(const FnxGrid* g) { return carve_step(g, nullptr).bytes; }
+size_t ws_step_static(const FnxGrid* g) {
+  const fnx::StepLayout L = carve_step(g, nullptr);
+  return g->is3D ? fnx::stage_word_offset(L) + al(fnx::stage_word_bytes(ncell(g), true)) : L.bytes;
+}
 
 }
 
@@ -221,6 +225,7 @@
     case FNX_OP_STEP: return ws_step(g);
     case FNX_OP_FLUIDNET: return fnx::fluidnet_ws_bytes(dims(g), g->is3D);
     case FNX_OP_ADVECT_STEP: return ws_advect(g, fnx::ADVECT_BOTH);
+    case FNX_OP_STEP_STATIC: return ws_step_static(g);
   }
   fail(FNX_EINVAL, "unknown op %d", op);
   return 0;
@@ -826,14 +831,14 @@
 }
 
 static int pre_projection(const FnxGrid* g, const fnx::StagePlan& sp, const FnxState* st, const float* U_adv, const float* rho_adv,
-                          float* div, void* stream) {
+                          float* div, void* stream, const unsigned* word = nullptr) {
   if (U_adv == st->U || (rho_adv && rho_adv == st->density)) return fail(FNX_EINVAL, "pre_projection: the advected fields must not alias the state");
   if (sp.confine && is_view(g))
     return fail(FNX_EINVAL, "pre_projection: vorticity confinement takes no compute window or z-slab view (single domain only)");
   hipStream_t s = (hipStream_t)stream;
   fnx::ProfScope ps(FNX_PROF_STAGE, s);
   const GridDims d = dims(g);
-  const fnx::BcPtrs bc = fnx::bc_ptrs(st);
+  const fnx::BcPtrs bc = fnx::bc_ptrs(st, word);
   const fnx::StageIO io{U_adv, rho_adv, st->flags, bc, st->U, st->density, sp.periodic ? nullptr : div};
   const fnx::StageOps all{quirks(g), true, sp.buoy, {sp.s[0], sp.s[1], sp.s[2]}, sp.rho_star, sp.grav, {sp.g[0], sp.g[1], sp.g[2]},
                           sp.wall, sp.second_bcs, d.K0 + d.KN};
@@ -871,15 +876,17 @@
   return pre_projection(g, fnx::stage_plan(prm, rho_adv != nullptr, st->flags_stick != nullptr), st, U_adv, rho_adv, div, stream);
 }
 
-int fnx_post_projection(const FnxGrid* g, const FnxState* st, void* stream) {
+static int post_projection(const FnxGrid* g, const FnxState* st, void* stream, const unsigned* word) {
   if (int rc = check_grid(g)) return rc;
   if (!st || !st->U || !st->flags || !st->p) return fail(FNX_EINVAL, "post_projection: NULL state");
   fnx::ProfScope ps(FNX_PROF_STAGE, (hipStream_t)stream);
-  fnx::launch_post_projection(dims(g), g->is3D, st->p, st->U, st->density, st->flags, fnx::bc_ptrs(st), (hipStream_t)stream,
+  fnx::launch_post_projection(dims(g), g->is3D, st->p, st->U, st->density, st->flags, fnx::bc_ptrs(st, word), (hipStream_t)stream,
                               st->density_bc_applied != 0);
   HIP_OK(hipGetLastError());
   return FNX_OK;
 }
+
+int fnx_post_projection(const FnxGrid* g, const FnxState* st, void* stream) { return post_projection(g, st, stream, nullptr); }
 
 int fnx_bc_classify(const FnxGrid* g, const FnxState* st, unsigned char* bc_class, void* stream) {
   if (int rc = check_grid(g)) return rc;
@@ -891,7 +898,7 @@
 
 int fnx_simulate_step(const FnxGrid* g, const FnxStepParams* prm, const FnxState* st, void* ws, size_t ws_bytes,
                       void* stream) {
-  using fnx::StepAdvect; using fnx::StepClassMap; using fnx::StepProjection; using fnx::StepTail;
+  using fnx::StepAdvect; using fnx::StepClassMap; using fnx::StepProjection; using fnx::StepStageWord; using fnx::StepTail;
   if (int rc = check_grid(g)) return rc;
   if (!prm || !st || !st->p || !st->U || !st->flags) return fail(FNX_EINVAL, "simulate_step: NULL state");
   if (prm->method < 0 || prm->method > 4) return fail(FNX_EINVAL, "Simulation method not supported. Choose convnet, jacobi, pcg or hybrid.");
@@ -939,7 +946,13 @@
   stc.bc_class = plan.class_map == StepClassMap::NONE ? nullptr : L.cls;
   stc.density_bc_applied = 1;
   st = &stc;
-  if (int rc = pre_projection(g, plan.stage, st, L.U2, has_rho ? L.rho2 : nullptr, plan.solve ? L.div : nullptr, stream)) return rc;
+  const StepStageWord sw = fnx::stage_word_plan(prm, g->is3D != 0, plan.class_map, L, ncell(g), ws_bytes);
+  unsigned* word = sw == StepStageWord::NONE ? nullptr : (unsigned*)((char*)ws + fnx::stage_word_offset(L));
+  if (sw == StepStageWord::BUILD) {
+    fnx::ProfScope ps(FNX_PROF_STAGE, s);
+    fnx::launch_stage_word(d, st->flags, L.cls, word, s);
+  }
+  if (int rc = pre_projection(g, plan.stage, st, L.U2, has_rho ? L.rho2 : nullptr, plan.solve ? L.div : nullptr, stream, word)) return rc;
 
   auto stick_then_bcs = [&]() -> int {
     if (int rc = fnx_set_wall_bcs_stick(g, st->U, L.U2, st->flags, st->flags_stick, stream)) return rc;
@@ -974,12 +987,12 @@
   }
   switch (plan.tail) {
     case StepTail::POST:
-      if (int rc = fnx_post_projection(g, st, stream)) return rc;
+      if (int rc = post_projection(g, st, stream, word)) return rc;
       break;
     case StepTail::POST_PERIODIC: {
       const fnx::BcPtrs bc = fnx::bc_ptrs(st);
       fnx::launch_periodic_post(d, g->is3D, st->U, (float*)L.tail, nullptr, nullptr, plan.stage.px, plan.stage.py, 0, s);
-      if (int rc = fnx_post_projection(g, st, stream)) return rc;
+      if (int rc = post_projection(g, st, stream, word)) return rc;
       fnx::launch_periodic_post(d, g->is3D, st->U, (float*)L.tail, bc.UBC, bc.UBCInvMask, plan.stage.px, plan.stage.py, 1, s);
       break;
     }
diff --git a/fluidnet_cxx_amd/csrc/fnx_kernels.h b/fluidnet_cxx_amd/csrc/fnx_kernels.h
--- a/fluidnet_cxx_amd/csrc/fnx_kernels.h
+++ b/fluidnet_cxx_amd/csrc/fnx_kernels.h
@@ -73,11 +73,11 @@
 void launch_set_wall_bcs_stick3d(const GridDims& g, const float* Uin, float* Uout, const float* flags, const float* stick,
                                  hipStream_t s);
 
-struct BcPtrs { const float *UBC, *UBCInvMask, *rhoBC, *rhoBCInvMask; const unsigned char* cls; };
-inline BcPtrs bc_ptrs(const FnxState* st) {
+struct BcPtrs { const float *UBC, *UBCInvMask, *rhoBC, *rhoBCInvMask; const unsigned char* cls; const unsigned* word; };
+inline BcPtrs bc_ptrs(const FnxState* st, const unsigned* word = nullptr) {
   const bool ubc = st->UBC && st->UBCInvMask, rbc = st->densityBC && st->densityBCInvMask;
   return BcPtrs{ubc ? st->UBC : nullptr, ubc ? st->UBCInvMask : nullptr, rbc ? st->densityBC : nullptr, rbc ? st->densityBCInvMask : nullptr,
-                st->bc_class};
+                st->bc_class, st->bc_class ? word : nullptr};
 }
 struct StageIO {
   const float *U_adv, *rho_adv, *flags;
@@ -103,6 +103,7 @@
 void launch_post_projection(const GridDims& g, bool is3d, const float* p, float* U, float* rho, const float* flags, const BcPtrs& bc,
                             hipStream_t s, bool rho_bc_applied = false, const float* scale = nullptr, float* p_scaled = nullptr);
 void launch_bc_classify(const GridDims& g, bool is3d, const BcPtrs& bc, unsigned char* cls, hipStream_t s);
+void launch_stage_word(const GridDims& g, const float* flags, const unsigned char* cls, unsigned* word, hipStream_t s);
 
 void launch_vorticity_confinement(const GridDims& g, bool is3d, const float* U_in, const float* flags, float* U_out, float amp,
                                   hipStream_t s);
diff --git a/fluidnet_cxx_amd/csrc/fnx_stage_word.h b/fluidnet_cxx_amd/csrc/fnx_stage_word.h
--- /dev/null
+++ b/fluidnet_cxx_amd/csrc/fnx_stage_word.h
@@ -0,0 +1,60 @@
+#pragma once
+#include <stddef.h>
+
+#include "../../include/fluidnet_hip.h"
+
+#if defined(__HIPCC__)
+#define FNX_WORD_FN __host__ __device__ inline
+#else
+#define FNX_WORD_FN inline
+#endif
+
+namespace fnx {
+
+enum : unsigned { FLAG_CODE_OTHER = 0, FLAG_CODE_FLUID = 1, FLAG_CODE_OBST = 2, FLAG_CODE_EMPTY = 3 };
+
+FNX_WORD_FN unsigned stage_flag_code(float f) {
+  return f == (float)FNX_TYPE_FLUID ? FLAG_CODE_FLUID : f == (float)FNX_TYPE_OBSTACLE ? FLAG_CODE_OBST : f == (float)FNX_TYPE_EMPTY ? FLAG_CODE_EMPTY : FLAG_CODE_OTHER;
+}
+
+template <class F> struct FlagConst;
+template <> struct FlagConst<float> { static constexpr float fluid = (float)FNX_TYPE_FLUID, obst = (float)FNX_TYPE_OBSTACLE, empty = (float)FNX_TYPE_EMPTY; };
+template <> struct FlagConst<unsigned> { static constexpr unsigned fluid = FLAG_CODE_FLUID, obst = FLAG_CODE_OBST, empty = FLAG_CODE_EMPTY; };
+
+FNX_WORD_FN void stage_word_offsets(int i, int j, int k, int W, int H, int D, int* minus, int* plus) {
+  const int HW = H * W;
+  minus[0] = i > 0 ? 1 : 0; minus[1] = j > 0 ? W : 0; minus[2] = k > 0 ? HW : 0;
+  plus[0] = i + 1 < W ? 1 : 0; plus[1] = j + 1 < H ? W : 0; plus[2] = k + 1 < D ? HW : 0;
+}
+
+FNX_WORD_FN unsigned stage_word_encode(float fc, const float* fm, const float* fp, unsigned cc, const unsigned* cm, const unsigned* cp) {
+  unsigned w = stage_flag_code(fc) | ((cc & 3u) << 14);
+  for (int a = 0; a < 3; ++a) {
+    w |= stage_flag_code(fm[a]) << (2 + 2 * a);
+    w |= stage_flag_code(fp[a]) << (8 + 2 * a);
+    w |= ((cm[a] >> 1) & 1u) << (16 + a);
+    w |= (cp[a] == 3u ? 1u : 0u) << (19 + a);
+  }
+  return w;
+}
+
+FNX_WORD_FN unsigned stage_word_at(const float* flags, const unsigned char* cls, int W, int H, int D, int i, int j, int k) {
+  int om[3], op[3];
+  stage_word_offsets(i, j, k, W, H, D, om, op);
+  const size_t o = ((size_t)k * H + j) * W + i;
+  float fm[3], fp[3];
+  unsigned cm[3], cp[3];
+  for (int a = 0; a < 3; ++a) { fm[a] = flags[o - om[a]]; fp[a] = flags[o + op[a]]; cm[a] = cls[o - om[a]]; cp[a] = cls[o + op[a]]; }
+  return stage_word_encode(flags[o], fm, fp, cls[o], cm, cp);
+}
+
+FNX_WORD_FN unsigned stage_word_cell(unsigned w) { return w & 3u; }
+FNX_WORD_FN unsigned stage_word_minus(unsigned w, int a) { return (w >> (2 + 2 * a)) & 3u; }
+FNX_WORD_FN unsigned stage_word_plus(unsigned w, int a) { return (w >> (8 + 2 * a)) & 3u; }
+FNX_WORD_FN unsigned stage_word_class(unsigned w) { return (w >> 14) & 3u; }
+FNX_WORD_FN bool stage_word_ident(unsigned w, bool with_plus) {
+  const unsigned need = (3u << 14) | (7u << 16) | (with_plus ? 7u << 19 : 0u);
+  return (w & need) == need;
+}
+
+}
diff --git a/fluidnet_cxx_amd/csrc/fnx_step.hip b/fluidnet_cxx_amd/csrc/fnx_step.hip
--- a/fluidnet_cxx_amd/csrc/fnx_step.hip
+++ b/fluidnet_cxx_amd/csrc/fnx_step.hip
@@ -1,7 +1,12 @@
 #include "fnx_device.h"
 #include "fnx_kernels.h"
+#include "fnx_stage_word.h"
+
+#include <type_traits>
 
 namespace {
+
+using fnx::FlagConst;
 
 constexpr int BX = 64, BY = 4;
 
@@ -12,38 +17,44 @@
   const float* rhoBC; const float* rhoBCInvMask;
   float* U; float* rho; float* div;
   const unsigned char* cls;
+  const unsigned* word;
   int grav; float gx, gy, gz;
   int bc2;
 };
 
-__device__ __forceinline__ bool gravity_applies(float fc, float fm) {
-  return (fc == FNX_FLUID || fc == FNX_EMPTY) && (fm == FNX_FLUID || (fm == FNX_EMPTY && fc == FNX_FLUID));
-}
-
-template <bool QUIRKS, bool WALL, bool BC1 = true>
-__device__ __forceinline__ float stage_eval3d(int a, float v, bool ubc, float um, float uc, float fc, float fm, bool border, bool buoy,
+template <class F>
+__device__ __forceinline__ bool gravity_applies(F fc, F fm) {
+  using K = FlagConst<F>;
+  return (fc == K::fluid || fc == K::empty) && (fm == K::fluid || (fm == K::empty && fc == K::fluid));
+}
+
+template <bool QUIRKS, bool WALL, bool BC1 = true, class F>
+__device__ __forceinline__ float stage_eval3d(int a, float v, bool ubc, float um, float uc, F fc, F fm, bool border, bool buoy,
                                               float r0, float r1, bool rbc, float rm0, float rc0, float rm1, float rc1, float s_a,
                                               float rho_star, bool grav, float g_a, bool bc2, int kg, int k) {
+  using K = FlagConst<F>;
   if (ubc && BC1) { const float t = v * um; v = t + uc; }
-  if (buoy && !border && fc == FNX_FLUID && fm == FNX_FLUID) {
+  if (buoy && !border && fc == K::fluid && fm == K::fluid) {
     float q0 = r0, q1 = r1;
     if (rbc) { float t = q0 * rm0; q0 = t + rc0; t = q1 * rm1; q1 = t + rc1; }
     if (a == 2 && QUIRKS) v = v + s_a * (0.5f * (q0 + (kg <= 1 ? 0.f : q1)));
     else v = v + s_a * ((0.5f * (q0 + q1)) - rho_star);
   }
   if (grav && !border && gravity_applies(fc, fm)) v = v + g_a;
-  if (WALL && (fc == FNX_FLUID || fc == FNX_OBST)) {
+  if (WALL && (fc == K::fluid || fc == K::obst)) {
     if (!(a == 2 && (kg == 0 || k == 0))) {
-      if (fm == FNX_OBST || (fc == FNX_OBST && fm == FNX_FLUID)) v = 0.f;
+      if (fm == K::obst || (fc == K::obst && fm == K::fluid)) v = 0.f;
     }
   }
   if (ubc && bc2) { const float t = v * um; v = t + uc; }
   return v;
 }
 
-template <bool QUIRKS, bool WALL, bool DIV, bool BC1 = true>
+template <bool QUIRKS, bool WALL, bool DIV, bool BC1 = true, bool WORD = false>
 __global__ __launch_bounds__(BX* BY) void stage3d_kernel(GridDims g, StepPtrs P, int buoy, float sx, float sy, float sz,
                                                          float rho_star, int kdiv) {
+  using F = std::conditional_t<WORD, unsigned, float>;
+  using K = FlagConst<F>;
   const int i = blockIdx.x * BX + threadIdx.x, j = blockIdx.y * BY + threadIdx.y;
   const int bk = blockIdx.z;
   const int b = bk / g.KN, k = g.K0 + (bk - b * g.KN);
@@ -54,7 +65,11 @@
   const int offp[3] = { i + 1 < g.W ? 1 : 0, j + 1 < g.H ? g.W : 0, k + 1 < g.D ? g.HW : 0 };
   const bool has_rho = P.rho_adv != nullptr, ubc = P.UBC != nullptr, rbc = P.rhoBC != nullptr;
   bool ident = false;
-  if (P.cls) {
+  unsigned w = 0u;
+  if constexpr (WORD) {
+    w = P.word[os];
+    ident = __builtin_amdgcn_ballot_w64(!fnx::stage_word_ident(w, want_div)) == 0;
+  } else if (P.cls) {
     bool mine = P.cls[os] == 3;
 #pragma unroll
     for (int a = 0; a < 3; ++a) mine = mine & ((P.cls[os - off[a]] & 2) != 0);
@@ -64,19 +79,26 @@
     }
     ident = __builtin_amdgcn_ballot_w64(!mine) == 0;
   }
-  const float fc = P.flags[os];
-  float fm[3], u[3], r1[3] = { 0.f, 0.f, 0.f }, r0 = 0.f;
-#pragma unroll
-  for (int a = 0; a < 3; ++a) { fm[a] = P.flags[os - off[a]]; u[a] = P.U_adv[((size_t)b * 3 + a) * g.DHW + o]; }
+  F fc, fm[3], fp[3] = { F(0), F(0), F(0) };
+  if constexpr (WORD) fc = fnx::stage_word_cell(w); else fc = P.flags[os];
+  float u[3], r1[3] = { 0.f, 0.f, 0.f }, r0 = 0.f;
+#pragma unroll
+  for (int a = 0; a < 3; ++a) {
+    if constexpr (WORD) fm[a] = fnx::stage_word_minus(w, a); else fm[a] = P.flags[os - off[a]];
+    u[a] = P.U_adv[((size_t)b * 3 + a) * g.DHW + o];
+  }
   if (has_rho) {
     r0 = P.rho_adv[os];
 #pragma unroll
     for (int a = 0; a < 3; ++a) r1[a] = P.rho_adv[os - off[a]];
   }
-  float fp[3] = { 0.f, 0.f, 0.f }, up[3] = { 0.f, 0.f, 0.f }, rp[3] = { 0.f, 0.f, 0.f };
+  float up[3] = { 0.f, 0.f, 0.f }, rp[3] = { 0.f, 0.f, 0.f };
   if (want_div) {
 #pragma unroll
-    for (int a = 0; a < 3; ++a) { fp[a] = P.flags[os + offp[a]]; up[a] = P.U_adv[((size_t)b * 3 + a) * g.DHW + o + offp[a]]; }
+    for (int a = 0; a < 3; ++a) {
+      if constexpr (WORD) fp[a] = fnx::stage_word_plus(w, a); else fp[a] = P.flags[os + offp[a]];
+      up[a] = P.U_adv[((size_t)b * 3 + a) * g.DHW + o + offp[a]];
+    }
     if (has_rho) {
 #pragma unroll
       for (int a = 0; a < 3; ++a) rp[a] = P.rho_adv[os + offp[a]];
@@ -133,7 +155,7 @@
       d = ((un[0] - vp[0]) + un[1]) - vp[1];
       d = d + (un[2] - vp[2]);
     }
-    if (fc == FNX_OBST) d = 0.f;
+    if (fc == K::obst) d = 0.f;
     P.div[os] = d;
   }
 }
@@ -213,7 +235,7 @@
   if (P.div) P.div[os] = d;
 }
 
-template <bool IS3D, bool SCALE>
+template <bool IS3D, bool SCALE, bool WORD = false>
 __global__ __launch_bounds__(BX* BY) void post_projection_kernel(GridDims g, const float* __restrict__ p,
                                                                  float* __restrict__ U, float* __restrict__ rho,
                                                                  const float* __restrict__ flags,
@@ -222,18 +244,28 @@
                                                                  const float* __restrict__ rhoBC,
                                                                  const float* __restrict__ rhoBCInvMask,
                                                                  const unsigned char* __restrict__ cls, int rho_done,
-                                                                 const float* __restrict__ scale, float* __restrict__ p_scaled) {
+                                                                 const float* __restrict__ scale, float* __restrict__ p_scaled,
+                                                                 const unsigned* __restrict__ word) {
+  static_assert(IS3D || !WORD, "the stage word is 3D only");
+  using F = std::conditional_t<WORD, unsigned, float>;
+  using K = FlagConst<F>;
   const int i = blockIdx.x * BX + threadIdx.x, j = blockIdx.y * BY + threadIdx.y;
   const int bk = blockIdx.z;
   const int b = IS3D ? bk / g.KN : bk, k = IS3D ? g.K0 + (bk - b * g.KN) : 0;
   if (i >= g.W || j >= g.H) return;
   constexpr int NC = IS3D ? 3 : 2;
   const size_t o = (size_t)k * g.HW + j * g.W + i, os = (size_t)b * g.DHW + o;
-  const float fc = flags[os], P = p[os];
-  const unsigned cl = cls ? cls[os] : 0u;
+  const float P = p[os];
+  unsigned sw = 0u;
+  if constexpr (WORD) sw = word[os];
+  F fc;
+  unsigned cl;
+  if constexpr (WORD) { fc = fnx::stage_word_cell(sw); cl = fnx::stage_word_class(sw); }
+  else { fc = flags[os]; cl = cls ? cls[os] : 0u; }
   const bool border = is_border<IS3D>(g, i, j, k);
   const float sc = SCALE ? scale[b] : 1.f;
-  float fm[NC], Pm[NC], u[NC], bm[NC], bc[NC];
+  F fm[NC];
+  float Pm[NC], u[NC], bm[NC], bc[NC];
   size_t ou[NC];
   const bool need_u = UBC != nullptr && !(cl & 1);
   const bool load_u = __builtin_amdgcn_ballot_w64(need_u) != 0;
@@ -246,7 +278,8 @@
     const int off = a == 0 ? 1 : (a == 1 ? g.W : g.HW);
     const int idx = a == 0 ? i : (a == 1 ? j : k);
     const int offs = idx > 0 ? off : 0;
-    fm[a] = flags[os - offs];
+    if constexpr (WORD) fm[a] = fnx::stage_word_minus(sw, a);
+    else fm[a] = flags[os - offs];
     Pm[a] = p[os - offs];
     u[a] = U[ou[a]];
     bm[a] = 1.f; bc[a] = 0.f;
@@ -264,12 +297,12 @@
     float v = u[a];
     if (SCALE) v = v / sc;
     {
-      const float m_ff = (fc == FNX_FLUID && fm[a] == FNX_FLUID) ? 1.f : 0.f;
+      const float m_ff = (fc == K::fluid && fm[a] == K::fluid) ? 1.f : 0.f;
       float w;
       if (!IS3D) {
-        const float m_fe = (fc == FNX_FLUID && fm[a] == FNX_EMPTY) ? 1.f : 0.f;
-        const float m_ef = (fc == FNX_EMPTY && fm[a] == FNX_FLUID) ? 1.f : 0.f;
-        const float m_nf = (fc == FNX_EMPTY && fm[a] == FNX_EMPTY) ? 1.f : 0.f;
+        const float m_fe = (fc == K::fluid && fm[a] == K::empty) ? 1.f : 0.f;
+        const float m_ef = (fc == K::empty && fm[a] == K::fluid) ? 1.f : 0.f;
+        const float m_nf = (fc == K::empty && fm[a] == K::empty) ? 1.f : 0.f;
         w = ((m_ff * (v - (P - Pm[a])) + m_fe * (v - P)) + m_ef * (v + Pm[a])) + m_nf * 0.f;
       } else {
         w = m_ff * (v - (P - Pm[a]));
@@ -279,7 +312,7 @@
     if (SCALE) v = v * sc;
     {
       const bool zface = a == 2 && (k + g.zoff == 0 || k == 0);
-      const bool wall = (fc == FNX_FLUID || fc == FNX_OBST) && !zface && (fm[a] == FNX_OBST || (fc == FNX_OBST && fm[a] == FNX_FLUID));
+      const bool wall = (fc == K::fluid || fc == K::obst) && !zface && (fm[a] == K::obst || (fc == K::obst && fm[a] == K::fluid));
       v = wall ? 0.f : v;
     }
     if (UBC) {
@@ -313,6 +346,15 @@
     if (rhoBC && rhoBCInvMask) c |= ((rhoBCInvMask[q] == 1.f) & (__float_as_uint(rhoBC[q]) == 0u)) ? 2u : 0u;
     cls[q] = (unsigned char)c;
   }
+}
+
+__global__ __launch_bounds__(BX* BY) void stage_word_kernel(GridDims g, const float* __restrict__ flags,
+                                                            const unsigned char* __restrict__ cls, unsigned* __restrict__ word) {
+  const int i = blockIdx.x * BX + threadIdx.x, j = blockIdx.y * BY + threadIdx.y;
+  const int bk = blockIdx.z, b = bk / g.D, k = bk - b * g.D;
+  if (i >= g.W || j >= g.H) return;
+  const size_t base = (size_t)b * g.DHW;
+  word[base + (size_t)k * g.HW + j * g.W + i] = fnx::stage_word_at(flags + base, cls + base, g.W, g.H, g.D, i, j, k);
 }
 
 __global__ __launch_bounds__(256) void periodic_pre_kernel(GridDims g, int nc, const float* __restrict__ U_adv,
@@ -365,24 +407,30 @@
 using Stage2d = void (*)(GridDims, StepPtrs, int, float, float, float);
 using Stage3d = void (*)(GridDims, StepPtrs, int, float, float, float, float, int);
 struct StageKernel { Stage2d k2; Stage3d k3; };
-template <bool Q, bool BC1> Stage3d stage3d_of(bool wall, bool div) {
-  return wall ? (div ? stage3d_kernel<Q, true, true, BC1> : stage3d_kernel<Q, true, false, BC1>)
-              : (div ? stage3d_kernel<Q, false, true, BC1> : stage3d_kernel<Q, false, false, BC1>);
-}
-StageKernel stage_kernel(bool is3d, const StageOps& o, bool div) {
+template <bool Q, bool BC1, bool WORD> Stage3d stage3d_of(bool wall, bool div) {
+  return wall ? (div ? stage3d_kernel<Q, true, true, BC1, WORD> : stage3d_kernel<Q, true, false, BC1, WORD>)
+              : (div ? stage3d_kernel<Q, false, true, BC1, WORD> : stage3d_kernel<Q, false, false, BC1, WORD>);
+}
+template <bool WORD> Stage3d stage3d_of(const StageOps& o, bool div) {
+  return !o.first_bcs ? stage3d_of<false, false, WORD>(o.wall, div)
+         : o.quirks   ? stage3d_of<true, true, WORD>(o.wall, div)
+                      : stage3d_of<false, true, WORD>(o.wall, div);
+}
+StageKernel stage_kernel(bool is3d, const StageOps& o, bool div, bool word) {
   if (!is3d) {
     return {o.first_bcs ? (o.wall ? stage2d_div_kernel<true, true> : stage2d_div_kernel<false, true>)
                         : (o.wall ? stage2d_div_kernel<true, false> : stage2d_div_kernel<false, false>), nullptr};
   }
-  return {nullptr, !o.first_bcs ? stage3d_of<false, false>(o.wall, div) : o.quirks ? stage3d_of<true, true>(o.wall, div) : stage3d_of<false, true>(o.wall, div)};
+  return {nullptr, word ? stage3d_of<true>(o, div) : stage3d_of<false>(o, div)};
 }
 }
 
 void launch_pre_projection(const GridDims& g, bool is3d, const StageIO& io, const StageOps& o, hipStream_t s) {
+  const unsigned* word = is3d ? io.bc.word : nullptr;
   const StepPtrs P{io.U_adv, io.rho_adv, io.flags, io.bc.UBC, io.bc.UBCInvMask, io.bc.rhoBC, io.bc.rhoBCInvMask, io.U, io.rho, io.div, io.bc.cls,
-                   o.grav ? 1 : 0, o.g[0], o.g[1], o.g[2], o.second_bcs ? 1 : 0};
+                   word, o.grav ? 1 : 0, o.g[0], o.g[1], o.g[2], o.second_bcs ? 1 : 0};
   const dim3 grid = cell_grid(g), block(BX, BY);
-  const StageKernel k = stage_kernel(is3d, o, io.div != nullptr);
+  const StageKernel k = stage_kernel(is3d, o, io.div != nullptr, word != nullptr);
   auto launch = [&](auto kernel, auto... rest) { kernel<<<grid, block, 0, s>>>(g, P, o.buoy ? 1 : 0, o.s[0], o.s[1], rest...); };
   if (is3d) launch(k.k3, o.s[2], o.rho_star, io.div ? o.div_k_end : 0);
   else launch(k.k2, o.rho_star);
@@ -393,10 +441,12 @@
   const dim3 grid = cell_grid(g), block(BX, BY);
   const int rd = (bc.cls && rho_bc_applied) ? 1 : 0;
   const bool scaled = scale && p_scaled;
+  const unsigned* word = is3d && !scaled ? bc.word : nullptr;
   auto k = scaled ? (is3d ? post_projection_kernel<true, true> : post_projection_kernel<false, true>)
-                  : (is3d ? post_projection_kernel<true, false> : post_projection_kernel<false, false>);
+                  : (is3d ? (word ? post_projection_kernel<true, false, true> : post_projection_kernel<true, false>)
+                          : post_projection_kernel<false, false>);
   k<<<grid, block, 0, s>>>(g, p, U, rho, flags, bc.UBC, bc.UBCInvMask, bc.rhoBC, bc.rhoBCInvMask, bc.cls, rd, scaled ? scale : nullptr,
-                           scaled ? p_scaled : nullptr);
+                           scaled ? p_scaled : nullptr, word);
 }
 
 void launch_periodic_pre(const GridDims& g, bool is3d, const float* U_adv, const float* UBC, const float* UBCInvMask, float* U,
@@ -420,4 +470,9 @@
   bc_classify_kernel<<<(unsigned)blocks, 256, 0, s>>>(n, (size_t)g.DHW, is3d ? 3 : 2, bc.UBC, bc.UBCInvMask, bc.rhoBC, bc.rhoBCInvMask, cls);
 }
 
-}
+void launch_stage_word(const GridDims& g, const float* flags, const unsigned char* cls, unsigned* word, hipStream_t s) {
+  const dim3 grid((g.W + BX - 1) / BX, (g.H + BY - 1) / BY, g.B * g.D);
+  stage_word_kernel<<<grid, dim3(BX, BY), 0, s>>>(g, flags, cls, word);
+}
+
+}
diff --git a/fluidnet_cxx_amd/csrc/fnx_step_plan.h b/fluidnet_cxx_amd/csrc/fnx_step_plan.h
--- a/fluidnet_cxx_amd/csrc/fnx_step_plan.h
+++ b/fluidnet_cxx_amd/csrc/fnx_step_plan.h
@@ -102,4 +102,13 @@
   return p;
 }
 
+enum class StepStageWord { NONE, BUILD, REUSE };
+inline size_t stage_word_offset(const StepLayout& L) { return (L.bytes + 255) & ~(size_t)255; }
+inline size_t stage_word_bytes(size_t cells, bool is3d) { return is3d ? cells * 4 : 0; }
+inline StepStageWord stage_word_plan(const FnxStepParams* prm, bool is3d, StepClassMap class_map, const StepLayout& L, size_t cells,
+                                     size_t ws_bytes) {
+  if (!is3d || class_map == StepClassMap::NONE || ws_bytes < stage_word_offset(L) + stage_word_bytes(cells, true)) return StepStageWord::NONE;
+  return (prm->static_flags & 5) == 5 ? StepStageWord::REUSE : StepStageWord::BUILD;
 }
+
+}
diff --git a/include/fluidnet_hip.h b/include/fluidnet_hip.h
--- a/include/fluidnet_hip.h
+++ b/include/fluidnet_hip.h
@@ -8,7 +8,7 @@
 extern "C" {
 #endif
 
-#define FNX_ABI_VERSION 32
+#define FNX_ABI_VERSION 33
 
 enum {
   FNX_OK = 0,
@@ -34,7 +34,9 @@
 } FnxGrid;
 
 enum { FNX_OP_ADVECT_SCALAR = 0, FNX_OP_ADVECT_VEL = 1, FNX_OP_JACOBI = 2, FNX_OP_STEP = 3, FNX_OP_FLUIDNET = 4,
-       FNX_OP_ADVECT_STEP = 5 };
+       FNX_OP_ADVECT_STEP = 5,
+       FNX_OP_STEP_STATIC = 6
+};
 size_t fnx_workspace_bytes(const FnxGrid* g, int op);
 
 const char* fnx_last_error(void);
```

Result: faster. 5580 Mcells/s (median of 6 runs) (+1.8%).
